# mmacklin/tinsel

Measured on AMD Instinct MI355X. Metric: Msamples/s (cornell.tin 1024x1024 maxDepth=4 spp=2126, wavefront path; Mrays/s alongside), higher is better.
Workload: dtype f32; 1 GPU; cornell.tin 1024x1024 maxDepth=4, 1 pass(es) per step, pipeline=auto; scene_pack=tests/golden/cornell.pack, parallelism=1 GPU

## Files before the change

### include/tinsel_hip.h

```cpp
#ifndef TINSEL_HIP_H
#define TINSEL_HIP_H

#include <stddef.h>
#include <stdint.h>

#ifdef __cplusplus
extern "C" {
#endif


typedef struct tinsel_vec3 { float x, y, z; } tinsel_vec3;
typedef struct tinsel_vec4 { float x, y, z, w; } tinsel_vec4;

typedef struct tinsel_transform {
    tinsel_vec3 p;
    tinsel_vec4 r;
    float s;
} tinsel_transform;

typedef struct tinsel_bvh_node {
    tinsel_vec3 lower;
    tinsel_vec3 upper;
    uint32_t left_index;
    uint32_t right_index_leaf;
// ... 295 lines not shown
typedef struct tinsel_ray     { float ox, oy, oz, time;  float dx, dy, dz, tmax; } tinsel_ray;
typedef struct tinsel_ray_hit { float t; int32_t primitive; float nx, ny, nz; uint32_t reserved[3]; } tinsel_ray_hit;

#define TINSEL_QUERY_CLOSEST  0
#define TINSEL_QUERY_OCCLUDED 1

int tinsel_hip_trace_rays(tinsel_hip* r, int mode, long long n, const tinsel_ray* rays_host, void* out_host);
int tinsel_hip_trace_rays_device(tinsel_hip* r, int mode, long long n, const tinsel_ray* rays_dev, void* out_dev, void* stream);
int tinsel_hip_trace_camera(tinsel_hip* r, const tinsel_camera* camera, int width, int height, float time, tinsel_ray_hit* out_host);

typedef struct tinsel_path_start { float ox, oy, oz, time;  float dx, dy, dz, reserved0;  uint32_t rng1, rng2, reserved1, reserved2; } tinsel_path_start;

int tinsel_hip_trace_radiance(tinsel_hip* r, long long n, const tinsel_path_start* starts_host, int max_depth, float* out_rgbx_host);
int tinsel_hip_trace_radiance_device(tinsel_hip* r, long long n, const tinsel_path_start* starts_dev, int max_depth, float* out_rgbx_dev, void* stream);

typedef struct tinsel_gather_point { float px, py, pz, time;  float nx, ny, nz;  uint32_t seed; } tinsel_gather_point;

#define TINSEL_GATHER_COSINE 0
#define TINSEL_GATHER_SPHERE 1

int tinsel_hip_gather_radiance(tinsel_hip* r, int mode, long long n, const tinsel_gather_point* points_host, int samples, int max_depth,
                               float* out_rgbx_host, tinsel_path_start* starts_out_host );
int tinsel_hip_gather_radiance_device(tinsel_hip* r, int mode, long long n, const tinsel_gather_point* points_dev, int samples, int max_depth,
                                      float* out_rgbx_dev, tinsel_path_start* starts_out_dev , void* stream);

#define TINSEL_GATHER_SH_MAX_ORDER 2

int tinsel_hip_gather_sh(tinsel_hip* r, int mode, int order, long long n, const tinsel_gather_point* points_host,
                         int samples, int max_depth, float* out_host, tinsel_path_start* starts_out_host );
int tinsel_hip_gather_sh_device(tinsel_hip* r, int mode, int order, long long n, const tinsel_gather_point* points_dev,
                                int samples, int max_depth, float* out_dev, tinsel_path_start* starts_out_dev , void* stream);

int tinsel_hip_reserve(tinsel_hip* r, int passes, int max_depth);

int tinsel_hip_set_batch_paths(tinsel_hip* r, unsigned long long max_paths);

long long tinsel_hip_read_batch_radiance(tinsel_hip* r, float* out_rgbx, unsigned long long max_paths);

int tinsel_hip_leaf(tinsel_hip* r, int op, int index, int n, const float* in, int in_stride, const uint32_t* seeds,
                    float* out, int out_stride, const tinsel_camera* camera, int width, int height);

int tinsel_hip_mesh_tree(tinsel_hip* r, int primitive, void* out_nodes, int capacity, int* out_meta);

int tinsel_hip_stack_entries(tinsel_hip* r);
int tinsel_hip_nee_per_path(tinsel_hip* r);
int tinsel_hip_walked_prims(tinsel_hip* r);
int tinsel_hip_walk_tops(tinsel_hip* r, int* out_counts, int capacity);
int tinsel_hip_queue_counts(tinsel_hip* r, uint32_t* out, int max_bounces);
int tinsel_hip_bounce_plan(tinsel_hip* r, uint32_t* out2);
unsigned int tinsel_hip_scene_features(const tinsel_scene_desc* scene);
int tinsel_hip_scene_plane_pairs(const tinsel_scene_desc* scene, int32_t* out_pairs, int capacity, int* out_singles);
int tinsel_hip_plane_table(tinsel_hip* r, int* out2);
int tinsel_hip_scene_slim(const tinsel_scene_desc* scene);
enum { TINSEL_BOUNCE_MEDIA = 1, TINSEL_BOUNCE_PROBE = 2, TINSEL_BOUNCE_MOTION = 4, TINSEL_BOUNCE_MESH_WALK = 8, TINSEL_BOUNCE_SPHERE = 16,
       TINSEL_BOUNCE_TRANSMISSION = 32, TINSEL_BOUNCE_POOLS = 64, TINSEL_BOUNCE_SHARE = 128, TINSEL_BOUNCE_SORT = 256, TINSEL_BOUNCE_ROULETTE = 512 };

const char* tinsel_hip_last_error(void);


typedef struct tinsel_hip_group tinsel_hip_group;

tinsel_hip_group* tinsel_hip_group_create(const tinsel_scene_desc* scene, int num_gpus, int tile);
tinsel_hip_group* tinsel_hip_group_create_tuned(const tinsel_scene_desc* scene, int num_gpus, int tile, const tinsel_hip_tuning* tuning);
void tinsel_hip_group_destroy(tinsel_hip_group* g);
int tinsel_hip_group_init(tinsel_hip_group* g, int width, int height);
int tinsel_hip_group_render(tinsel_hip_group* g, const tinsel_camera* camera, const tinsel_options* options, float* out_rgba, int passes);
int tinsel_hip_group_set_lookahead(tinsel_hip_group* g, int enable);
int tinsel_hip_group_present(tinsel_hip_group* g, const tinsel_options* options, int nlm_width, float nlm_falloff, float* out_rgba);
int tinsel_hip_group_size(tinsel_hip_group* g);
tinsel_hip* tinsel_hip_group_member(tinsel_hip_group* g, int rank);

#define TINSEL_HIP_COMM_ID_BYTES 128
int tinsel_hip_comm_unique_id(unsigned char* id_bytes, int capacity);
int tinsel_hip_comm_init(tinsel_hip* r, const unsigned char* id_bytes, int rank, int world);
int tinsel_hip_comm_size(tinsel_hip* r);
int tinsel_hip_comm_reduce_accum(tinsel_hip* r, float* out_device, int root, void* stream);

int tinsel_hip_plan_regions(unsigned long long slots, int num_cus, int nee_per_path, int fused, unsigned int* out);

int tinsel_hip_selftest_arith(int device_index, int op, int variant, unsigned long long* out_counts, unsigned int* out_first_bad);
int tinsel_hip_selftest_sort(int device_index, unsigned long long* keys, unsigned long long n, int begin_bit, int end_bit);
int tinsel_hip_selftest_scan(int device_index, const int* in, int* out, unsigned long long n);
int tinsel_hip_accumulate_support(int filter_type, float filter_width, float filter_falloff, float filter_offset, float* out_arg_zero);
int tinsel_hip_selftest_accumulate(int device_index, int width, int height, int filter_type, float filter_width, float filter_falloff, float filter_offset,
                                   float clamp, const unsigned int* pass_seeds, int passes, const float* radiance, float* accum, int choice, int form,
                                   int* out_form);

int tinsel_hip_ubench(int device_index, int kind, unsigned long long bytes, int steps, double* out_ms, double* out_units);


#define TINSEL_PACK_MAGIC "TINPACK1"

typedef struct tinsel_pack_header {
    char magic[8];
    uint32_t version;
    uint32_t num_primitives;
    uint32_t num_bvh_nodes;
    uint32_t num_meshes;
    uint64_t total_bytes;
    uint64_t off_primitives;
    uint64_t off_bvh_nodes;
    uint64_t off_probe_data;
    uint64_t off_probe_pdf_x;
    uint64_t off_probe_cdf_x;
    uint64_t off_probe_pdf_y;
    uint64_t off_probe_cdf_y;
// ... 47 lines not shown
```

### tinsel_amd/abi.py

```python
import ctypes as C


class Vec3(C.Structure):
    _fields_ = [("x", C.c_float), ("y", C.c_float), ("z", C.c_float)]

    def __iter__(self):
        return iter((self.x, self.y, self.z))


class Vec4(C.Structure):
    _fields_ = [("x", C.c_float), ("y", C.c_float), ("z", C.c_float), ("w", C.c_float)]

    def __iter__(self):
        return iter((self.x, self.y, self.z, self.w))


class Transform(C.Structure):
    _fields_ = [("p", Vec3), ("r", Vec4), ("s", C.c_float)]


class BVHNode(C.Structure):
    _fields_ = [("lower", Vec3), ("upper", Vec3), ("left_index", C.c_uint32), ("right_index_leaf", C.c_uint32)]


# ... 102 lines not shown
RAY_HIT_DTYPE = [("t", "<f4"), ("primitive", "<i4"), ("nx", "<f4"), ("ny", "<f4"), ("nz", "<f4"), ("reserved", "<u4", (3,))]
QUERY_CLOSEST, QUERY_OCCLUDED = 0, 1


class PathStart(C.Structure):
    _fields_ = [("ox", C.c_float), ("oy", C.c_float), ("oz", C.c_float), ("time", C.c_float),
                ("dx", C.c_float), ("dy", C.c_float), ("dz", C.c_float), ("reserved0", C.c_float),
                ("rng1", C.c_uint32), ("rng2", C.c_uint32), ("reserved1", C.c_uint32), ("reserved2", C.c_uint32)]


PATH_START_DTYPE = [("ox", "<f4"), ("oy", "<f4"), ("oz", "<f4"), ("time", "<f4"), ("dx", "<f4"), ("dy", "<f4"), ("dz", "<f4"), ("reserved0", "<f4"),
                    ("rng1", "<u4"), ("rng2", "<u4"), ("reserved1", "<u4"), ("reserved2", "<u4")]


class GatherPoint(C.Structure):
    _fields_ = [("px", C.c_float), ("py", C.c_float), ("pz", C.c_float), ("time", C.c_float),
                ("nx", C.c_float), ("ny", C.c_float), ("nz", C.c_float), ("seed", C.c_uint32)]


GATHER_POINT_DTYPE = [("px", "<f4"), ("py", "<f4"), ("pz", "<f4"), ("time", "<f4"), ("nx", "<f4"), ("ny", "<f4"), ("nz", "<f4"), ("seed", "<u4")]
GATHER_COSINE, GATHER_SPHERE = 0, 1
GATHER_SH_MAX_ORDER = 2
FEATURE_ALBEDO, FEATURE_NORMAL, FEATURE_DEPTH = 1, 2, 4
FEATURE_NAMES = ("albedo", "normal", "depth")
ID_MISS, ID_EMPTY, ID_MAX_SLOTS = -1, -2, 8
MAX_LIGHT_GROUPS = 8
MAX_VIEWS = 4096
VIEWS_ADD, VIEWS_ACCUMULATE_SINGLY = 1, 2
SAMPLE_MAP_MAX = 65535
SAMPLES_ADD = 1
RENDER_SAMPLE_MAP_ARGTYPES = [C.c_void_p, C.POINTER(Camera), C.POINTER(Options), C.c_uint32, C.c_void_p, C.c_uint, C.c_void_p]
RENDER_SAMPLE_MAP_DEVICE_ARGTYPES = RENDER_SAMPLE_MAP_ARGTYPES + [C.c_void_p]
PLAN_SAMPLE_MAP_ARGTYPES = [C.c_ulonglong, C.c_int, C.c_int, C.c_void_p, C.POINTER(C.c_ulonglong)]


class DenoiseParams(C.Structure):
    _fields_ = [("radius", C.c_int32), ("patch_radius", C.c_int32),
                ("k_color", C.c_float), ("k_albedo", C.c_float), ("k_normal", C.c_float), ("k_depth", C.c_float),
                ("demodulate", C.c_int32), ("albedo_floor", C.c_float)]

    def as_dict(self):
        return {k: getattr(self, k) for k, _ in self._fields_}


class KernelTimeV1(C.Structure):
    _fields_ = [("name", C.c_char * 32), ("launches", C.c_uint32), ("total_ms", C.c_float)]


BOUNCE_GENERAL, BOUNCE_COUNT, BOUNCE_FIT_CLOSED, BOUNCE_FIT_DEFERRED = 0, 1, 2, 3
BOUNCE_MEDIA, BOUNCE_PROBE, BOUNCE_MOTION, BOUNCE_MESH_WALK, BOUNCE_SPHERE = 1, 2, 4, 8, 16
BOUNCE_TRANSMISSION, BOUNCE_POOLS, BOUNCE_SHARE, BOUNCE_SORT, BOUNCE_ROULETTE = 32, 64, 128, 256, 512


class Tuning(C.Structure):
    _fields_ = [("struct_bytes", C.c_uint32),
                ("flat_scan", C.c_int32), ("lds_scene", C.c_int32), ("walk", C.c_int32), ("inline_max_tris", C.c_int32), ("walk_min_tris", C.c_int32),
                ("small_mesh_bytes", C.c_int64), ("arena_lds_limit", C.c_int64),
                ("batch_paths", C.c_int64), ("grid_mult", C.c_int32), ("bounce_share", C.c_int32), ("repack", C.c_int32),
                ("tail_split", C.c_int32), ("tail_share", C.c_float), ("tail_divide", C.c_int32),
                ("shade_sorted", C.c_int32), ("overlap", C.c_int32), ("scene_walk", C.c_int32), ("swalk_lds", C.c_int32), ("accumulate", C.c_int32),
                ("walk_block", C.c_int32), ("walk_single", C.c_int32), ("walk_lds_stack", C.c_int32), ("walk_refill_min", C.c_int32), ("walk_leaf_min", C.c_int32),
                ("walk_grid_mult", C.c_int32), ("quads_in_scan", C.c_int32), ("bounce_fit", C.c_int32), ("plane_pairs", C.c_int32)]
    CREATE_FIELDS = ("flat_scan", "lds_scene", "walk", "inline_max_tris", "walk_min_tris", "small_mesh_bytes", "arena_lds_limit")
    _DEFAULTS = dict(flat_scan=-1, lds_scene=-1, walk=-1, inline_max_tris=-1, walk_min_tris=-1, small_mesh_bytes=-1, arena_lds_limit=-1,
                     batch_paths=0, grid_mult=0, bounce_share=-1, repack=-1, tail_split=-1, tail_share=0.0, tail_divide=4,
                     shade_sorted=-1, overlap=-1, scene_walk=-1, swalk_lds=-1, accumulate=0,
                     walk_block=0, walk_single=-1, walk_lds_stack=-1, walk_refill_min=0, walk_leaf_min=0, walk_grid_mult=0, quads_in_scan=-1, bounce_fit=-1, plane_pairs=-1)

    def __init__(self, **over):
        super().__init__()
        self.struct_bytes = C.sizeof(Tuning)
        for k, v in self._DEFAULTS.items():
            setattr(self, k, v)
        for k, v in over.items():
            if k not in self._DEFAULTS:
                raise TypeError("tinsel_hip_tuning has no field %r" % k)
            setattr(self, k, v)

    def replace(self, **over):
        t = Tuning(**{k: getattr(self, k) for k in self._DEFAULTS})
        for k, v in over.items():
            if k not in self._DEFAULTS:
                raise TypeError("tinsel_hip_tuning has no field %r" % k)
            setattr(t, k, v)
        return t

    def as_dict(self):
        return {k: getattr(self, k) for k in self._DEFAULTS}


ACCUMULATE_AUTO, ACCUMULATE_TILED, ACCUMULATE_WIDE, ACCUMULATE_PIPED, ACCUMULATE_FULL_WINDOW = 0, 1, 2, 3, 4
ACCUMULATE_FORM_AUTO, ACCUMULATE_FORM_FULL_WINDOW, ACCUMULATE_FORM_SUPPORT = 0, 1, 2
ACCUMULATE_RAN_UNTILED, ACCUMULATE_RAN_TILED, ACCUMULATE_RAN_WIDE, ACCUMULATE_RAN_PIPED, ACCUMULATE_RAN_SUPPORT_TILED, ACCUMULATE_RAN_SUPPORT_WIDE = 0, 1, 2, 3, 4, 5
SELFTEST_ACCUMULATE_ARGTYPES = [C.c_int, C.c_int, C.c_int, C.c_int, C.c_float, C.c_float, C.c_float, C.c_float, C.c_void_p, C.c_int, C.c_void_p, C.c_void_p,
                                C.c_int, C.c_int, C.POINTER(C.c_int)]


def accumulate_arg_zero(offset):
    import math
    import numpy as np
    z = math.log(float(np.float32(offset))) - 1e-6
    f = np.float32(z)
    if float(f) > z:
        f = np.nextafter(f, np.float32(-np.inf))
    return f


def accumulate_takes_support_form(filter_type, width, falloff, offset):
    import numpy as np
    width, falloff, offset = np.float32(width), np.float32(falloff), np.float32(offset)
    if filter_type == FILTER_BOX or not (offset > 0 and np.isfinite(offset)) or not (falloff > 0 and np.isfinite(falloff)) or not (0 < width <= 1):
        return False
    return bool(-falloff <= accumulate_arg_zero(offset))
COMM_ID_BYTES = 128
MODE_NORMALS, MODE_COMPLEXITY, MODE_PATHTRACE = 0, 1, 2
BVH_REFERENCE, BVH_LBVH, BVH_PLOC = 0, 1, 2
SCENE_BVH_NODES, SCENE_BVH_DEVICE = 0, 1
ARITH_EXACT, ARITH_FAST = 0, 1
PROBE_CDF, PROBE_ALIAS = 0, 1
LOOKAHEAD_OFF, LOOKAHEAD_ON, LOOKAHEAD_PIN_OUTPUT = 0, 1, 2
# ... 10 lines not shown
```

### tinsel_amd/build.py

```python
import hashlib
import json
import os
import shutil
import subprocess
import sys
import tempfile
import time

HERE = os.path.dirname(os.path.abspath(__file__))
ROOT = os.path.dirname(HERE)
SRC = os.path.join(HERE, "csrc", "tinsel_hip.hip")
SRC_FAST = os.path.join(HERE, "csrc", "tinsel_fast.hip")
OUT = os.path.join(HERE, "libtinsel_hip.so")
OBJ_DIR = os.path.join(HERE, "csrc", "_obj")
DEPS = [os.path.join(HERE, "csrc", f) for f in sorted(os.listdir(os.path.join(HERE, "csrc"))) if not f.startswith("_")] + \
       [os.path.join(ROOT, "include", "tinsel_hip.h")]

COMMON_FLAGS = [
    "--offload-arch=gfx950", "-O3", "-std=c++17", "-fPIC", "-fno-slp-vectorize",
    "-Wall", "-Wno-unused-function", "-Wno-unused-variable",
]
HIPCC_FLAGS = COMMON_FLAGS + ["-ffp-contract=off", "-fno-fast-math"]
FAST_FLAGS = COMMON_FLAGS + ["-DTN_FAST=1", "-ffp-contract=fast", "-fno-hip-fp32-correctly-rounded-divide-sqrt", "-freciprocal-math",
                             "-fgpu-flush-denormals-to-zero"]


def hipcc():
    for cand in (os.environ.get("HIPCC"), shutil.which("hipcc"), "/opt/rocm/bin/hipcc"):
        if cand and os.path.exists(cand):
            return cand
    raise RuntimeError("hipcc not found: the HIP library cannot be built (there is no CPU fallback)")


def up_to_date():
    if not os.path.exists(OUT):
        return False
    t = os.path.getmtime(OUT)
    return all(os.path.getmtime(d) <= t for d in DEPS)


def _compile(obj_dir, extra=(), verbose=True):
    os.makedirs(obj_dir, exist_ok=True)
    cc = hipcc()
    jobs = [
        [cc] + HIPCC_FLAGS + list(extra) + ["-c", SRC, "-o", "tinsel_hip.o"],
        [cc] + FAST_FLAGS + list(extra) + ["-c", SRC_FAST, "-o", "tinsel_fast.o"],
    ]
    procs = []
    for cmd in jobs:
        if verbose:
            print("[tinsel_amd.build] (in %s)" % obj_dir, " ".join(cmd), flush=True)
        procs.append(subprocess.Popen(cmd, cwd=obj_dir))
    for p, cmd in zip(procs, jobs):
        if p.wait() != 0:
            raise subprocess.CalledProcessError(p.returncode, cmd)


def _resource_job(tmp):
    cmd = [hipcc()] + HIPCC_FLAGS + ["--cuda-device-only", "-Rpass-analysis=kernel-resource-usage", "-c", SRC, "-o", "resources_only.o"]
    return subprocess.Popen(cmd, cwd=tmp, stdout=subprocess.DEVNULL, stderr=subprocess.PIPE, text=True)


def _kernel_name(mangled):
    import re
    m = re.match(r"_ZN2tn(\d+)", mangled)
    if not m:
        return mangled
    n = int(m.group(1))
    name, rest = mangled[m.end():m.end() + n], mangled[m.end() + n:]
    if len(name) != n or not name.startswith("k_"):
        return mangled
    t = re.match(r"I((?:L[bij]n?\d+E)+)E", rest)
    args = re.findall(r"L[bij](n?\d+)E", t.group(1)) if t else []
    return name + ("<" + ",".join(a.replace("n", "-") for a in args) + ">" if args else "")


def _parse_resources(text):
    import re
    out, cur = {}, None
    for line in text.splitlines():
        m = re.search(r"remark:\s+(.*?)\s*\[-Rpass-analysis", line)
        if not m:
            continue
        body = m.group(1)
        if body.startswith("Function Name:"):
            cur = out.setdefault(_kernel_name(body.split(":", 1)[1].strip()), {})
        elif cur is not None and ":" in body:
            k, v = body.split(":", 1)
            key = {"VGPRs": "vgprs", "AGPRs": "agprs", "TotalSGPRs": "sgprs", "ScratchSize [bytes/lane]": "scratch_bytes",
                   "Occupancy [waves/SIMD]": "waves_per_simd", "LDS Size [bytes/block]": "static_lds_bytes",
                   "SGPRs Spill": "sgpr_spills", "VGPRs Spill": "vgpr_spills"}.get(k.strip())
            if key:
                cur[key] = int(v.strip())
    return out


def _code_bytes(device_obj):
    import struct
    with open(device_obj, "rb") as f:
        b = f.read()
    magic = b"__CLANG_OFFLOAD_BUNDLE__"
    if b.startswith(magic):
        count, = struct.unpack_from("<Q", b, len(magic))
        pos = len(magic) + 8
        for _ in range(count):
            off, size, tlen = struct.unpack_from("<QQQ", b, pos)
            triple = b[pos + 24:pos + 24 + tlen]
            pos += 24 + tlen
# ... 83 lines not shown
```

### tinsel_amd/csrc/tinsel_hip.hip

```cpp

#include "../../include/tinsel_hip.h"

#include "tn_launch.h"
#include "tn_denoise.h"
#include "tn_lbvh.h"
#include "tn_ubench.h"
#include "tn_selftest.h"

#include "tn_sort.h"

#include <hip/hip_runtime.h>
#include <rccl/rccl.h>

#include <dlfcn.h>

#include <cmath>
#include <condition_variable>
#include <deque>
#include <mutex>
#include <thread>
#include <cstdio>
#include <cstdlib>
#include <cstring>
#include <map>
#include <memory>
#include <string>
#include <vector>

using namespace tn;

namespace {

thread_local std::string g_error;

int fail(const std::string& msg)
{
    g_error = msg;
    fprintf(stderr, "tinsel_hip: %s\n", msg.c_str());
    return -1;
}

#define HIP_TRY(expr)                                                                                       \
    do {                                                                                                    \
        hipError_t _e = (expr);                                                                             \
        if (_e != hipSuccess)                                                                               \
            return fail(std::string(#expr) + ": " + hipGetErrorString(_e));                                 \
    } while (0)

#define HIP_TRY_NULL(expr)                                                                                  \
    do {                                                                                                    \
        hipError_t _e = (expr);                                                                             \
        if (_e != hipSuccess) {                                                                             \
            fail(std::string(#expr) + ": " + hipGetErrorString(_e));                                        \
            return nullptr;                                                                                 \
        }                                                                                                   \
    } while (0)

}

#include "tn_host_own.h"
#include "tn_host_layout.h"
#include "tn_host_state.h"
#include "tn_host_batch.h"
#include "tn_host_query.h"
#include "tn_host_radiance.h"
#include "tn_host_gather.h"
#include "tn_host_features.h"
#include "tn_host_ids.h"
#include "tn_host_light_groups.h"
#include "tn_host_views.h"
#include "tn_host_samples.h"
#include "tn_host_denoise.h"
#include "tn_host_lookahead.h"
#include "tn_host_bvh_build.h"
#include "tn_host_scene.h"

#include "tn_host_create.h"
#include "tn_host_api.h"
#include "tn_host_group.h"
```

### tinsel_amd/csrc/tn_fused.h

```cpp
#pragma once

#include "tn_path_state.h"

namespace tn {

constexpr int kPoolFields = 25;
constexpr int kPoolWordsPerWave = kPoolFields*kWave;
constexpr int kPoolWords = kPoolWordsPerWave*(kBlock/kWave);

constexpr int kPoolFieldsSlim = 21;

template <int FIELDS>
TN_D void pool_store(uint32_t* pool, uint32_t e, const PathRegs& p, uint32_t slot, int prim, float t, V3 n)
{
    static_assert(FIELDS == kPoolFields || FIELDS == kPoolFieldsSlim, "a pool entry is whole or slim");
    uint32_t* q = pool + e;
    q[0*kWave] = __float_as_uint(p.o.x); q[1*kWave] = __float_as_uint(p.o.y); q[2*kWave] = __float_as_uint(p.o.z);
    q[3*kWave] = __float_as_uint(p.d.x); q[4*kWave] = __float_as_uint(p.d.y); q[5*kWave] = __float_as_uint(p.d.z);
    if constexpr (FIELDS == kPoolFieldsSlim)
    {
        q[6*kWave] = __float_as_uint(p.thr.x); q[7*kWave] = __float_as_uint(p.thr.y); q[8*kWave] = __float_as_uint(p.thr.z);
        q[9*kWave] = __float_as_uint(p.rad.x); q[10*kWave] = __float_as_uint(p.rad.y); q[11*kWave] = __float_as_uint(p.rad.z);
        q[12*kWave] = p.rng.s1; q[13*kWave] = p.rng.s2;
        q[14*kWave] = __float_as_uint(p.bsdfPdf);
// ... 30 lines not shown
        p.rad = V3(__uint_as_float(q[9*kWave]), __uint_as_float(q[10*kWave]), __uint_as_float(q[11*kWave]));
        p.rng.s1 = q[12*kWave]; p.rng.s2 = q[13*kWave];
        p.bsdfPdf = __uint_as_float(q[14*kWave]);
        slot = q[15*kWave];
        prim = (int)q[16*kWave];
        t = __uint_as_float(q[17*kWave]);
        n = V3(__uint_as_float(q[18*kWave]), __uint_as_float(q[19*kWave]), __uint_as_float(q[20*kWave]));
        path_slim_constants(p);
        return;
    }
    p.time = __uint_as_float(q[6*kWave]);
    p.thr = V3(__uint_as_float(q[7*kWave]), __uint_as_float(q[8*kWave]), __uint_as_float(q[9*kWave]));
    p.rad = V3(__uint_as_float(q[10*kWave]), __uint_as_float(q[11*kWave]), __uint_as_float(q[12*kWave]));
    p.rng.s1 = q[13*kWave]; p.rng.s2 = q[14*kWave];
    p.eta = __uint_as_float(q[15*kWave]);
    p.bsdfPdf = __uint_as_float(q[16*kWave]);
    p.rayType = (int)q[17*kWave];
    slot = q[18*kWave];
    prim = (int)q[19*kWave];
    t = __uint_as_float(q[20*kWave]);
    n = V3(__uint_as_float(q[21*kWave]), __uint_as_float(q[22*kWave]), __uint_as_float(q[23*kWave]));
    p.medium = (int)q[24*kWave];
}


#ifdef TN_PROFILE_SECTIONS
#define TN_PROF_DECL uint32_t prof[6] = { 0, 0, 0, 0, 0, 0 }; long long tprev = clock64();
#define TN_TICK(k) { const long long _t = clock64(); prof[k] += (uint32_t)(_t - tprev); tprev = _t; }
#define TN_PROF_FLUSH if (lane_id() == 0) { for (int k = 0; k < 6; ++k) atomicAdd(q.stats + (size_t)(blockIdx.x % kStatShards)*kStatWords + 2 + k, (unsigned long long)prof[k]); } if (true) return;
#else
#define TN_TICK(k)
#define TN_PROF_DECL
#define TN_PROF_FLUSH
#endif

struct BounceKernargs { DevScene scIn; SplitState ss; QueueCtl q; int bounceBegin, bounceEnd, stackEntries; CameraParams cam; FrameParams fp; const uint32_t* passSeeds; };

enum BounceKind : int { kBounceGeneral = 0, kBounceCount = 1, kBounceFitClosed = 2, kBounceFitDeferred = 3 };
constexpr uint32_t bounce_kind_features(int kind)
{
    return kind == kBounceFitClosed ? (uint32_t)kFeatSphere :
           kind == kBounceFitDeferred ? (uint32_t)(kFeatSphere | kFeatPools | kFeatShare | kFeatSort) : (uint32_t)kFeatAll;
}

template <int KIND, bool LDS, bool DEFER>
__global__ __launch_bounds__(kBlock, kBounceWaves) void k_bounce(BounceKernargs ka)
{
    constexpr bool COUNT = KIND == kBounceCount;
    constexpr uint32_t FEAT = bounce_kind_features(KIND);
    constexpr bool SLIM = KIND >= kBounceFitClosed;
    constexpr int POOL = SLIM ? kPoolFieldsSlim : kPoolFields;
    static_assert(!SLIM || !(FEAT & (kFeatMedia | kFeatMotion | kFeatTransmission | kFeatProbe)), "the slim state has no word for these");
    typedef SceneT<LDS, false, DEFER ? 1 : 0, false, FEAT> SC;
    const DevScene& scIn = ka.scIn;
    const SplitState& ss = ka.ss;
    const QueueCtl& q = ka.q;
    const int bounceBegin = ka.bounceBegin, bounceEnd = ka.bounceEnd, stackEntries = ka.stackEntries;
    const CameraParams& cam = ka.cam;
    const FrameParams& fp = ka.fp;
    const uint32_t* __restrict__ const passSeeds = ka.passSeeds;
    extern __shared__ uint32_t s_stack[];
    LdsStack<kBlock> st = { s_stack + threadIdx.x };

    const bool repack = (FEAT & kFeatPools) && fp.repack != 0;
    const bool shareRegions = (FEAT & kFeatShare) && fp.share != 0;
    const uint32_t wave = wave_in_block();
    uint32_t* const pool = s_stack + stackEntries*kBlock + kScanWords + wave*kPoolWordsPerWave;
    SC sc;
    stage_scene_lds(sc, scIn, s_stack + stackEntries*kBlock + kScanWords + (repack ? kPoolWords : 0));
    if constexpr (!(FEAT & kFeatMedia)) sc.hasMedia = 0;
    if constexpr (!(FEAT & kFeatProbe)) sc.probe.valid = 0;
    if constexpr (!(FEAT & kFeatSort)) sc.sortQueues = 0;
    if constexpr (KIND >= kBounceFitClosed) sc.flatScan = 1;
    auto mat_at = [&](int prim) {
        Mat m = load_mat(sc.mats, prim);
        if constexpr (!(FEAT & kFeatTransmission)) m.transmission = 0.0f;
        if constexpr (SLIM) m.subsurface = 0.0f;
        return m;
    };
    typedef const __attribute__((address_space(4))) SplitState* StatePtr;
    auto state_args = [&]() {
        StatePtr sp = (StatePtr)((const __attribute__((address_space(4))) char*)__builtin_amdgcn_kernarg_segment_ptr() + offsetof(BounceKernargs, ss));
        asm volatile("" : "+s"(sp));
        return sp;
    };
    auto ssBuf = [&](int buf) {
        StatePtr sp = state_args();
        if constexpr (SLIM)
        {
            static_assert(offsetof(SplitState, rad) + sizeof(float4*[2]) - offsetof(SplitState, rayO) == 64, "rayO, rayD, thr, rad: contiguous");
            float4* const o0 = sp->rayO[0]; float4* const o1 = sp->rayO[1]; float4* const d0 = sp->rayD[0]; float4* const d1 = sp->rayD[1];
            float4* const t0 = sp->thr[0]; float4* const t1 = sp->thr[1]; float4* const r0 = sp->rad[0]; float4* const r1 = sp->rad[1];
            StateBuf b = { buf ? o1 : o0, buf ? d1 : d0, buf ? t1 : t0, buf ? r1 : r0, nullptr };
            return b;
        }
        StateBuf b = { sp->rayO[buf], sp->rayD[buf], sp->thr[buf], sp->rad[buf], sp->rngId[buf] };
        return b;
    };
    auto radOutNow = [&]() { return state_args()->radOut; };
#define TN_SS_BUF(buf) ssBuf(buf)
#define TN_RAD_OUT radOutNow()
    auto late_sky = [&]() {
        typedef const __attribute__((address_space(4))) DevScene* ScenePtr;
        ScenePtr sp = (ScenePtr)((const __attribute__((address_space(4))) char*)__builtin_amdgcn_kernarg_segment_ptr() + offsetof(BounceKernargs, scIn));
        asm volatile("" : "+s"(sp));
        DevScene s;
// ... 113 lines not shown
                        load_state(sc, TN_SS_BUF(cur), pos, p, slot, hasMedia);
                    have = true;
                }
            }

            if (have)
            {
                TN_TICK(0)
                prim = trace<SC, LdsStack<kBlock>, COUNT>(sc, st, p.o, p.d, p.time, t, n3, ctr);
                rays++;
                TN_TICK(1)
                if (prim < 0)
                {
                    on_miss(late_sky(), p, bounce);
                    TN_RAD_OUT[slot] = make_float4(p.rad.x, p.rad.y, p.rad.z, 0.0f);
                    have = false;
                }
            }

            if (repack)
            {
                const unsigned long long live = __ballot(have);
                const uint32_t nLive = (uint32_t)__popcll(live);
                if (flush || poolCount + nLive >= (uint32_t)kWave)
                {
                    const uint32_t take = (poolCount < (uint32_t)kWave - nLive) ? poolCount : (uint32_t)kWave - nLive;
                    const uint32_t rank = bits_below(~live);
                    if (!have && rank < take)
                    {
                        pool_load<POOL>(pool, poolCount - 1u - rank, p, slot, prim, t, n3);
                        if constexpr (!SLIM)
                            p.absorption = medium_absorption(sc, p.medium, hasMedia);
                        have = true;
                    }
                    poolCount -= take;
                }
                else
                {
                    if (have)
                        pool_store<POOL>(pool, poolCount + bits_below(live), p, slot, prim, t, n3);
                    poolCount += nLive;
                    have = false;
                }
            }

            if (have)
            {
                {
                    const V3 n = n3;
                    const Mat mat = mat_at(prim);
                    HitCtx h;
                    on_hit_begin<SLIM>(p, mat, t, n, bounce, h, prim);

                    if (sc.totalLightSamples > 0)
                    {
                        const V3 thrAtNee = p.thr;
                        LightCursor lights;
                        V3 sum = nee_sum(sc, [&](int k) -> V3 {
                            NeeGeo g;
                            V3 skyColor;
                            float skyPdf = 0.0f;
                            int light = -1;
                            if (sc.probe.valid && k == 0)
                                nee_sample_probe(late_sky(), h.p, h.n, p.rng, g, skyColor, skyPdf);
                            else
                            {
                                light = lights.next(sc);
                                nee_sample_light(sc, h.p, h.n, p.time, light, p.rng, g);
                            }
                            TN_TICK(2)
                            float ts;
                            V3 nn;
                            const int hp = trace<SC, LdsStack<kBlock>, COUNT>(sc, st, g.o, g.wi, p.time, ts, nn, ctr);
                            TN_TICK(3)
                            rays++;
                            shadowRays++;
                            if (light < 0)
                                return (hp < 0) ? nee_contrib_probe<SLIM>(mat_at(prim), h, g.wi, skyColor, skyPdf) : V3(0.0f);
                            if (!nee_light_reached(g, hp, ts))
                                return V3(0.0f);
                            return nee_contrib_light<SLIM>(sc, mat_at(prim), h, g.wi, g.nl, light, hp, ts);
                        });
                        p.rad = p.rad + thrAtNee*sum;
                    }

                    TN_TICK(2)
                    if (bounce + 1 < fp.maxDepth)
                    {
                        const Mat matAgain = mat_at(prim);
                        alive = (bsdf_step<SLIM>(p, matAgain, h) == kContinue);
                        if ((FEAT & kFeatRoulette) && alive && fp.rrStart > 0 && bounce + 1 >= fp.rrStart)
                            alive = roulette_survives(p);
                    }
                }

                TN_TICK(5)
                if (alive)
                    front = !sc.sortQueues || ray_meets_bounded_prim(sc, p.o, p.d);
                else
                    TN_RAD_OUT[slot] = make_float4(p.rad.x, p.rad.y, p.rad.z, 0.0f);
            }
            const uint32_t np = out.push(alive, front);
            if (alive)
            {
                if constexpr (SLIM)
                    store_state_slim(TN_SS_BUF(nxt), np, p, slot);
                else
                    store_state(TN_SS_BUF(nxt), np, p, slot);
            }
            if (flush)
                break;
        }
        if (lane == 0)
        {
            ss.segFront[(size_t)(bounce + 1)*ss.numRegions + r] = out.nFront;
            ss.segBack[(size_t)(bounce + 1)*ss.numRegions + r] = out.nBack;
        }
      }
    }

    wave_add_stat(q.stats, 0, rays);
    wave_add_stat(q.stats, 1, samples);
#ifndef TN_PROFILE_SECTIONS
    wave_add_stat(q.stats, 5, shadowRays);
#endif
    TN_PROF_FLUSH
    if (COUNT)
    {
        wave_add_stat(q.stats, 2, ctr.internal);
        wave_add_stat(q.stats, 3, ctr.tris);
        wave_add_stat(q.stats, 4, ctr.prims);
    }
}


// ... 5 lines not shown
```

### tinsel_amd/csrc/tn_host_api.h

```cpp
#pragma once

extern "C" {

int tinsel_hip_init(tinsel_hip* r, int width, int height)
{
    if (r)
        lookahead_release(r);
    if (!r || width <= 0 || height <= 0)
        return fail("init: bad arguments");
    HIP_TRY(hipSetDevice(r->device));
    HIP_TRY(hipDeviceSynchronize());
    r->accum = nullptr;
    if (r->accumOwn.alloc((size_t)width*height))
        return -1;
    r->accum = r->accumOwn.get();
    HIP_TRY(hipMemset(r->accum, 0, sizeof(float4)*(size_t)width*height));
    HIP_TRY(hipStreamSynchronize(nullptr));
    r->width = width;
    r->height = height;
    return 0;
}

int tinsel_hip_init_external(tinsel_hip* r, int width, int height, float* device_accum)
{
// ... 953 lines not shown
    std::vector<float> eqs;
    for (int n = 0; n < scene->num_bvh_nodes; ++n)
    {
        const tinsel_bvh_node& nd = scene->bvh_nodes[n];
        if (!ref_is_leaf(nd) || nd.left_index >= (uint32_t)scene->num_primitives || scene->primitives[nd.left_index].type != TINSEL_GEOM_PLANE)
            continue;
        if (make_prim_box(nd).alwaysHit && std::find(planes.begin(), planes.end(), (int32_t)nd.left_index) == planes.end())
            planes.push_back((int32_t)nd.left_index);
    }
    std::sort(planes.begin(), planes.end());
    for (const int32_t k : planes)
        eqs.insert(eqs.end(), scene->primitives[k].geo.plane.plane, scene->primitives[k].geo.plane.plane + 4);
    const std::vector<std::pair<int, int>> pairs = pair_planes(eqs);
    for (size_t q = 0; q < pairs.size() && out_pairs && (int)q < capacity; ++q)
    {
        out_pairs[2*q] = planes[(size_t)pairs[q].first];
        out_pairs[2*q + 1] = planes[(size_t)pairs[q].second];
    }
    if (out_singles)
        *out_singles = (int)planes.size() - 2*(int)pairs.size();
    return (int)pairs.size();
}

int tinsel_hip_plane_table(tinsel_hip* r, int* out2)
{
    if (!r || !out2)
        return fail("plane_table: bad arguments");
    out2[0] = r->planePairs;
    out2[1] = r->planeSingles;
    return 0;
}

int tinsel_hip_scene_slim(const tinsel_scene_desc* scene)
{
    if (!scene || !scene->primitives)
        return 0;
    bool anySubsurface = false;
    for (int i = 0; i < scene->num_primitives; ++i)
        anySubsurface = anySubsurface || !is_plus_zero(scene->primitives[i].material.subsurface);
    return scene_slim(tinsel_hip_scene_features(scene), anySubsurface) ? 1 : 0;
}

int tinsel_hip_bounce_plan(tinsel_hip* r, uint32_t* out2)
{
    if (!r || !out2)
        return fail("bounce_plan: bad arguments");
    if (r->lastBounceKind < 0)
        return fail("bounce_plan: the fused kernel has not run yet");
    out2[0] = (uint32_t)r->lastBounceKind;
    out2[1] = r->lastBounceFeatures;
    return 0;
}

int tinsel_hip_queue_counts(tinsel_hip* r, uint32_t* out, int max_bounces)
{
    if (!r || !out || max_bounces < 1)
        return fail("queue_counts: bad arguments");
    if (r->batchPipeline < 0 || r->batchDepth < 1)
        return fail("queue_counts: nothing rendered yet");
    HIP_TRY(hipSetDevice(r->device));
    HIP_TRY(hipDeviceSynchronize());
    const int n = std::min(max_bounces, std::min(r->batchDepth, r->lastFp.maxDepth));
    if (r->lastPipeline == TINSEL_PIPELINE_MEGAKERNEL || r->batchPipeline != r->lastPipeline)
        return fail("queue_counts: the last batch did not run a wavefront pipeline");
    const tinsel_hip::DenseLane& lane = r->lane[r->lastLane];
    const bool split = r->lastPipeline == TINSEL_PIPELINE_WAVEFRONT_SPLIT && r->neePerPath > 0;
    const size_t W = lane.regions;
    std::vector<uint32_t> seg(W*(size_t)n*4, 0u);
    uint32_t* const src[4] = { lane.ss.segFront, lane.ss.segBack, lane.ss.neeFront, lane.ss.neeBack };
    for (int a = 0; a < (split ? 4 : 2); ++a)
        HIP_TRY(hipMemcpy(seg.data() + (size_t)a*W*n, src[a], W*(size_t)n*sizeof(uint32_t), hipMemcpyDeviceToHost));
    for (int b = 0; b < n; ++b)
    {
        unsigned long long live = 0, nee = 0;
        for (size_t g = 0; g < W; ++g)
        {
            live += seg[(size_t)b*W + g] + seg[W*n + (size_t)b*W + g];
            nee += seg[2*W*n + (size_t)b*W + g] + seg[3*W*n + (size_t)b*W + g];
        }
        out[b] = (b == 0 && r->lastPipeline == TINSEL_PIPELINE_WAVEFRONT) ? lane.paths : (uint32_t)live;
        out[max_bounces + b] = (uint32_t)nee;
    }
    return n;
}


int tinsel_hip_plan_regions(unsigned long long slots, int num_cus, int nee_per_path, int fused, unsigned int* out)
{
    if (!out || slots == 0 || slots >= 0xffffffffull || num_cus < 1 || num_cus > 4096)
        return fail("plan_regions: bad arguments");
    RegionSpec s = region_spec(tuning_defaults(), num_cus, nee_per_path, fused != 0, kBounceWaves);
    s.capacity = (size_t)slots + s.maxRegions*kWave;
    RegionCut c;
    const int rc = cut_regions(s, (size_t)slots, streaming_grid(s, (size_t)slots), c) ? 0 : fail("render: path buffers too small for this batch");
    out[0] = c.numRegions; out[1] = c.regionLen; out[2] = c.bigRegions; out[3] = c.shortLen;
    out[4] = (unsigned int)c.grid(); out[5] = (unsigned int)s.maxRegions;
    return rc;
}

int tinsel_hip_selftest_arith(int device_index, int op, int variant, unsigned long long* out_counts, unsigned int* out_first_bad)
{
    if (!out_counts || !out_first_bad || op < 0 || op > 2)
        return fail("selftest_arith: bad arguments");
    if (variant < 0)
        variant = op == 0 ? kRcpVariant : op == 1 ? kSqrtVariant : kRsqrtVariant;
    HIP_TRY(hipSetDevice(device_index));
// ... 285 lines not shown
```

### tinsel_amd/csrc/tn_host_batch.h

```cpp
#pragma once

namespace {

void free_batch(tinsel_hip* r)
{
    r->batchMem.release();
    for (tinsel_hip::DenseLane& lane : r->lane)
        lane = tinsel_hip::DenseLane();
    r->batchPipeline = -1;
    r->batchSlots = 0;
    r->batchStateSlots = 0;
    r->batchLanes = 1;
    r->batchNee = -1;
    r->batchDepth = -1;
    r->lastBatchSlots = 0;
}

constexpr int kGridMultDefault = 32;
int grid_mult(const tinsel_hip* r) { return r->tune.grid_mult > 0 ? r->tune.grid_mult : kGridMultDefault; }

bool paired_can(const tinsel_hip* r) { return r->scene.flatScan != 0 && !r->countDetail; }

enum Residency { RES_HBM, RES_LDS, RES_MIXED };
Residency residency(const DevScene& sc, uint32_t staged) { return sc.allInArena ? RES_LDS : (staged != 0 && staged == sc.arenaBytes) ? RES_MIXED : RES_HBM; }
// ... 330 lines not shown
    if (share < 0.0)
    {
        const double sets = (double)grid/(double)(s.resident*s.numCUs);
        share = std::min(0.25, std::max(0.03, -share/std::max(1.0, sets)));
    }
    if (share > 0.0 && share < 0.9 && divide >= 2)
        split_tail_regions(s, c, slots, share, divide);
    return true;
}

bool plan_bounce(const tinsel_hip* r, int* resident)
{
    const size_t perCU = 160u*1024u;
    const size_t lds = stack_bytes(r), withPool = lds + kPoolWords*sizeof(uint32_t);
    const bool want = r->tune.repack >= 0 ? r->tune.repack != 0 : !r->sceneEnclosed;
    const bool pools = want && withPool*3 <= perCU && withPool <= (size_t)r->sharedMemLimit;
    const size_t ldsPerGroup = std::max<size_t>(1, pools ? withPool : lds);
    *resident = (int)std::max<size_t>(1, std::min<size_t>((size_t)kBounceWaves, perCU/ldsPerGroup));
    return pools;
}

uint32_t bounce_features(const tinsel_hip* r, bool pools)
{
    uint32_t f = 0;
    f |= r->scene.hasMedia ? kFeatMedia : 0u;
    f |= r->scene.probe.valid ? kFeatProbe : 0u;
    f |= r->anyTransmission ? kFeatTransmission : 0u;
    f |= r->scene.sortQueues ? kFeatSort : 0u;
    f |= pools ? kFeatPools : 0u;
    f |= r->rrStart > 0 ? kFeatRoulette : 0u;
    for (size_t i = 0; i < r->primsHost.size(); ++i)
    {
        const Prim64& p = r->primsHost[i];
        f |= (p.flags & kPrimMoving) ? kFeatMotion : 0u;
        f |= p.type == (uint32_t)kPrimSphere ? kFeatSphere : 0u;
        const int m = i < r->primMesh.size() ? r->primMesh[i] : -1;
        if (p.type == (uint32_t)kPrimMesh && !(p.flags & kPrimQuadArena) && !(m >= 0 && r->meshesNow[(size_t)m].twoLeaves))
            f |= kFeatMeshWalk;
    }
    return f;
}

bool scene_slim(uint32_t features, bool anySubsurface)
{
    return !(features & (kFeatMedia | kFeatProbe | kFeatMotion | kFeatMeshWalk | kFeatTransmission)) && !anySubsurface;
}

int fit_bounce(uint32_t need, bool deferMeshes)
{
    auto within = [&](int kind) { return (need & ~bounce_kind_features(kind)) == 0u; };
    if (deferMeshes)
        return within(kBounceFitDeferred) ? PK_BOUNCE_FIT_DEFERRED : PK_NONE;
    return within(kBounceFitClosed) ? PK_BOUNCE_FIT_CLOSED : PK_NONE;
}

struct WalkPlan
{
    int variant = PK_NONE, block = 256, perCU = 1;
    bool single = false;
    uint32_t ldsBytes = 0;
    WalkJob job = {};
};

struct SwalkPlan
{
    int extend = PK_NONE, shadow = PK_NONE, block = kBlock, perCU = 32;
    uint32_t ldsBytes = 0, arenaLds = 0;
    SwalkJob job = {};
};

WalkPlan plan_walk(const tinsel_hip* r)
{
    const tinsel_hip_tuning& t = r->tune;
    WalkPlan w;
    WalkJob& job = w.job;
    const int gridMult = t.walk_grid_mult > 0 ? t.walk_grid_mult : 1;
    job.refillMin = std::min(64, std::max(1, t.walk_refill_min > 0 ? t.walk_refill_min : 24));
    job.leafMin = std::min(64, std::max(1, t.walk_leaf_min > 0 ? t.walk_leaf_min : 8));
    job.numPrims = r->walkPrims.count;
    job.prof = r->walkProf.get();
    int entries = 1;
    for (int k = 0; k < kWalkMaxPrims && k < r->walkPrims.count; ++k)
    {
        job.prim[k] = r->walkPrims.prim[k];
        entries = std::max(entries, r->meshesNow[(size_t)r->walkPrimMesh[k]].stackNeed);
    }
    w.single = r->walkPrims.count == 1 && t.walk_single != 0;
    const size_t ctl = (kWalkCtlWords + (w.single ? 0 : kWalkMaxPrims*kWalkPrimWords))*sizeof(uint32_t);
    const int ldsStackEnv = t.walk_lds_stack >= 0 ? t.walk_lds_stack : 8;
    const bool twoPerCU = ldsStackEnv > 0 && !t.walk_block;
    const int ldsEntries = twoPerCU ? std::min(entries, std::max(1, ldsStackEnv)) : entries;
    const int rows = w.single ? kWalkLaneRows : kWalkRayRows;
    const size_t ldsBudget = twoPerCU ? (size_t)r->sharedMemLimit/2 : (size_t)r->sharedMemLimit;
    const bool big = t.walk_block ? t.walk_block == 1024 : (size_t)(ldsEntries + rows)*1024*sizeof(uint32_t) + ctl + 16384 <= ldsBudget;
    w.block = big ? 1024 : 256;
    size_t lds = (size_t)(ldsEntries + rows)*w.block*sizeof(uint32_t) + ctl;
    if (big)
    {
        size_t room = (ldsBudget - lds)/sizeof(Node64);
        for (int k = 0; k < r->walkPrims.count && room > 0; ++k)
        {
            const int n = (int)std::min<size_t>(room, (size_t)r->meshesNow[(size_t)r->walkPrimMesh[k]].topCount);
            job.topCount[k] = n;
            room -= (size_t)n;
            lds += (size_t)n*sizeof(Node64);
        }
// ... 477 lines not shown
{
    switch (generate)
    {
    case PK_GENERATE_RAYS: return KN_GENERATE_RAYS;
    case PK_GENERATE_GATHER: return KN_GENERATE_GATHER;
    default: return KN_GENERATE;
    }
}

int cut_and_generate(tinsel_hip* r, const BatchPlan& p, tinsel_hip::DenseLane& L, hipStream_t st, LaunchArgs& a, size_t slots, int* grid)
{
    *grid = streaming_grid(p.regions, slots);
    if (p.workList)
        *grid = std::max(1, std::min(*grid, (int)(seg_prefix_max_regions(r)/(kBlock/kWave))));
    if (cut_batch(p, L, a, slots, grid))
        return -1;
    ScopedTimer t(r, generate_timer(p.generate), st);
    a.grid = *grid;
    a.variant = p.generate;
    a.ldsBytes = 0;
    return launch_path(r, a, st);
}

void order_regions(tinsel_hip* r, hipStream_t st, const LaunchArgs& a, const uint32_t* front, const uint32_t* back, uint32_t* out)
{
    ScopedTimer t(r, KN_SEG, st);
    hipLaunchKernelGGL(k_region_order, dim3(1), dim3(kOrderBlock), 0, st, front, back, a.ss.numRegions, out);
}

int trace_fused(tinsel_hip* r, const BatchPlan& p, tinsel_hip::DenseLane& L, hipStream_t st, LaunchArgs& a, size_t slots)
{
    int grid = streaming_grid(p.regions, slots);
    if (cut_batch(p, L, a, slots, &grid))
        return -1;
    a.grid = grid;
    if (p.pools)
    {
        a.fp.repack = 1;
        a.ldsBytes += (uint32_t)(kPoolWords*sizeof(uint32_t));
    }
    {
        const int shareLen = 512;
        a.fp.share = r->tune.bounce_share >= 0 ? (r->tune.bounce_share != 0) : (r->neePerPath >= 3 || (int)a.ss.regionLen <= shareLen);
    }
    a.bounce = 0;
    a.bounceEnd = a.fp.maxDepth;
    a.order = nullptr;
    a.variant = a.fp.share ? p.bounceShared : p.bounce;
    r->lastBounceKind = a.variant == PK_BOUNCE_FIT_CLOSED ? kBounceFitClosed :
                        a.variant == PK_BOUNCE_FIT_DEFERRED ? kBounceFitDeferred :
                        (a.variant == PK_BOUNCE_COUNT_LDS || a.variant == PK_BOUNCE_COUNT) ? kBounceCount : kBounceGeneral;
    r->lastBounceFeatures = p.bounceFeatures | (a.fp.share ? kFeatShare : 0u);
    ScopedTimer t(r, KN_BOUNCE, st);
    return launch_path(r, a, st);
}

int trace_paired(tinsel_hip* r, const BatchPlan& p, tinsel_hip::DenseLane& L, hipStream_t st, LaunchArgs& a, size_t slots)
{
    int grid = 0;
    if (cut_and_generate(r, p, L, st, a, slots, &grid))
        return -1;
    const size_t W = a.ss.numRegions;
    const int K = r->neePerPath, maxDepth = a.fp.maxDepth;
    const int steps = maxDepth + (K > 0 ? 1 : 0);
    for (int bounce = 0; bounce < steps; ++bounce)
    {
        a.bounce = bounce;
        a.order = nullptr;
        if (p.walk)
        {
            a.grid = grid;
            const bool first = bounce == 0, last = bounce >= maxDepth;
            if (launch_walk(r, p, L, st, a, slots, L.ss.segFront + (size_t)bounce*W,  !first && K > 0,  !first && !last && K > 0))
                return -1;
        }
        if (bounce > 0 && maxDepth >= 6 && grid > r->numCUs*2)
        {
            order_regions(r, st, a, L.ss.segFront + (size_t)bounce*W, L.ss.segBack + (size_t)bounce*W, L.regionOrder);
            a.order = L.regionOrder;
        }
        ScopedTimer t(r, KN_STEP, st);
        a.grid = grid;
        a.variant = p.step;
        a.ldsBytes = p.ldsTrace;
        a.stackEntries = p.stackScan;
        if (launch_path(r, a, st))
            return -1;
    }
    return 0;
}

int trace_split(tinsel_hip* r, const BatchPlan& p, tinsel_hip::DenseLane& L, hipStream_t st, LaunchArgs& a, size_t slots)
{
    int grid = 0;
    if (cut_and_generate(r, p, L, st, a, slots, &grid))
        return -1;
    const size_t W = a.ss.numRegions;
    const bool ordered = !p.walk && grid > r->numCUs*2;
    for (int bounce = 0; bounce < a.fp.maxDepth; ++bounce)
    {
        a.bounce = bounce;
        a.order = nullptr;
        if (ordered && bounce > 0)
        {
            order_regions(r, st, a, L.ss.segFront + (size_t)bounce*W, L.ss.segBack + (size_t)bounce*W, L.regionOrder);
            a.order = L.regionOrder;
// ... 476 lines not shown
```

### tinsel_amd/csrc/tn_host_create.h

```cpp
#pragma once

namespace {

void comm_release(tinsel_hip* r);


struct SceneBuild
{
    tinsel_hip* r;
    DevScene& sc;
    const tinsel_scene_desc* desc;
    const tinsel_hip_tuning& tune;
    int P;
    std::vector<Prim64> prims;
    std::vector<Mat128> mats;
    std::vector<Moving64> moving;
    std::vector<DevMesh> meshes;
    std::vector<int32_t> lights;
    std::map<uint64_t, uint32_t> meshIndex;
    ArenaBuilder arena;
    int maxMeshNeed = 0;
    int totalLightSamples = 0;
    bool sceneHasBigMesh = false;
    SceneLevel lvl;
    bool flatScan = false;

    SceneBuild(tinsel_hip* r_, const tinsel_scene_desc* d)
        : r(r_), sc(r_->scene), desc(d), tune(r_->tune), P(d->num_primitives), prims((size_t)P), mats((size_t)P), moving((size_t)P)
    {
        for (int i = 0; i < P; ++i)
            if (desc->primitives[i].type == TINSEL_GEOM_MESH && mesh_bytes_estimate(desc->primitives[i].geo.mesh) > kSmallMeshBytes)
                sceneHasBigMesh = true;
    }

    static size_t mesh_bytes_estimate(const tinsel_mesh_geometry& g)
    {
        return (size_t)g.num_nodes*32 + (size_t)(g.num_indices/3)*52 + (size_t)g.num_vertices*12;
    }
    bool lives_in_arena(size_t meshBytes, int numTris) const
    {
        if (tune.small_mesh_bytes >= 0)
            return meshBytes <= (size_t)tune.small_mesh_bytes;
        const int inlineMaxTris = tune.inline_max_tris >= 0 ? tune.inline_max_tris : kInlineMaxTris;
        return sceneHasBigMesh ? numTris <= inlineMaxTris && meshBytes <= kSmallMeshBytes : meshBytes <= kSmallMeshBytes;
    }

    int add_primitives();
    int add_mesh(const tinsel_mesh_geometry& g, Prim64& o);
    int scene_level();
    void mark_walked_and_quads();
    int assemble_arena();
    void set_scene_flags();
    int upload_probe();
    int stats_and_fit();
};

void create_limits(tinsel_hip* r, int device_index, const tinsel_hip_tuning* tuning)
{
    r->device = device_index;
    r->tune = tuning_from_caller(tuning);
    hipDeviceProp_t prop;
    if (hipGetDeviceProperties(&prop, device_index) == hipSuccess)
    {
        r->numCUs = prop.multiProcessorCount;
        r->sharedMemLimit = (int)prop.sharedMemPerBlock;
    }
    prepare_kernels_once(r);
    if (!r->prepRefused.empty() && r->sharedMemLimit > 65536)
    {
        fprintf(stderr, "tinsel_hip: the runtime refused %d B of dynamic LDS for %s: planning within 65536 B per workgroup\n", r->sharedMemLimit, r->prepRefused.c_str());
        r->sharedMemLimit = 65536;
        r->segPrefixLds = std::min(r->segPrefixLds, 65536 - 1024);
    }

    if (r->tune.batch_paths >= 65536)
    {
        r->maxBatchSlots = (size_t)r->tune.batch_paths;
        r->batchSlotsExplicit = true;
    }
}

int SceneBuild::add_mesh(const tinsel_mesh_geometry& g, Prim64& o)
{
    const int numTris = g.num_indices/3;
    if (numTris <= 0 || !g.positions || !g.normals || !g.indices || !g.nodes || !g.cdf)
        return fail("create: mesh primitive with missing arrays");
    ConvertedBvh cb;
    if (!convert_bvh(g.nodes, g.num_nodes, numTris, lives_in_arena(mesh_bytes_estimate(g), numTris) ? 0 : kWalkTopNodes, cb))
        return fail("create: malformed mesh BVH");
    std::vector<Tri48> tris((size_t)numTris);
    for (int t = 0; t < numTris; ++t)
    {
        const int i0 = g.indices[t*3 + 0], i1 = g.indices[t*3 + 1], i2 = g.indices[t*3 + 2];
        if (i0 < 0 || i1 < 0 || i2 < 0 || i0 >= g.num_vertices || i1 >= g.num_vertices || i2 >= g.num_vertices)
            return fail("create: mesh index out of range");
        Tri48& T = tris[(size_t)t];
        T.ax = g.positions[i0].x; T.ay = g.positions[i0].y; T.az = g.positions[i0].z; T.i0 = i0;
        T.bx = g.positions[i1].x; T.by = g.positions[i1].y; T.bz = g.positions[i1].z; T.i1 = i1;
        T.cx = g.positions[i2].x; T.cy = g.positions[i2].y; T.cz = g.positions[i2].z; T.i2 = i2;
    }

    DevMesh dm;
    memset(&dm, 0, sizeof(dm));
    dm.root = cb.root;
    dm.numTris = numTris;
    dm.stackNeed = cb.maxLeafDepth + 1;
    dm.topCount = cb.topCount;
    dm.numInternal = (int32_t)cb.nodes.size();
    dm.twoLeaves = (cb.nodes.size() == 1 && !(cb.root & kLeafBit) && (cb.nodes[0].left & kLeafBit) && (cb.nodes[0].right & kLeafBit)) ? 1 : 0;
    const size_t meshBytes = cb.nodes.size()*sizeof(Node64) + tris.size()*sizeof(Tri48) + (size_t)g.num_vertices*12 + (size_t)numTris*4;
    if (lives_in_arena(meshBytes, numTris))
    {
        dm.inArena = 1;
        dm.offNodes = (uint32_t)arena.add(cb.nodes.data(), cb.nodes.size());
        dm.offTris = (uint32_t)arena.add(tris.data(), tris.size());
        dm.offNormals = (uint32_t)arena.add(&g.normals[0].x, (size_t)g.num_vertices*3);
        dm.offCdf = (uint32_t)arena.add(g.cdf, (size_t)numTris);
    }
    else
    {
        dm.nodes = r->sceneMem.upload(cb.nodes.data(), cb.nodes.size());
        dm.tris = r->sceneMem.upload(tris.data(), tris.size());
        dm.normals = r->sceneMem.upload(&g.normals[0].x, (size_t)g.num_vertices*3);
        dm.cdf = r->sceneMem.upload(g.cdf, (size_t)numTris);
        if ((!cb.nodes.empty() && !dm.nodes) || !dm.tris || !dm.normals || !dm.cdf)
            return fail("create: device allocation failed (mesh)");
    }
    if (dm.stackNeed > maxMeshNeed)
        maxMeshNeed = dm.stackNeed;
    r->meshNumVertices.push_back(g.num_vertices);
    r->meshIndices.emplace_back(g.indices, g.indices + (size_t)numTris*3);
    r->meshRootLo.push_back(V3(g.nodes[0].lower.x, g.nodes[0].lower.y, g.nodes[0].lower.z));
    r->meshRootHi.push_back(V3(g.nodes[0].upper.x, g.nodes[0].upper.y, g.nodes[0].upper.z));
    r->meshArea.push_back(g.area);
    o.mesh = (uint32_t)meshes.size();
    meshIndex[g.id] = o.mesh;
    meshes.push_back(dm);
    return 0;
}

int SceneBuild::add_primitives()
{
    for (int i = 0; i < P; ++i)
    {
        const tinsel_primitive& p = desc->primitives[i];
        Prim64& o = prims[(size_t)i];
        memset(&o, 0, sizeof(o));

        make_material(p, mats[(size_t)i]);
        r->primEndScale.push_back(p.end_transform.s);
        if (p.light_samples > 0)
        {
            if (p.type == TINSEL_GEOM_PLANE)
                return fail("create: a plane cannot be a light (PrimitiveSample asserts, intersection.h:871-875)");
            lights.push_back(i);
            totalLightSamples += p.light_samples;
        }

        const bool isStatic = memcmp(&p.start_transform, &p.end_transform, sizeof(tinsel_transform)) == 0;
        const Xform xs = to_xform(p.start_transform), xe = to_xform(p.end_transform);
        r->primStart.push_back(xs);
        r->primEnd.push_back(xe);
        set_prim_pose(o, xs, xe, isStatic);
        o.moving = (uint32_t)i;
        moving[(size_t)i] = make_moving(xs, xe);

        if (p.type == TINSEL_GEOM_SPHERE)
        {
            o.type = kPrimSphere;
            o.g0 = p.geo.sphere.radius;
// ... 34 lines not shown
    const int need = lvl.bvh.maxLeafDepth + 1 + maxMeshNeed;
    r->stackNeed = pick_stack(need);
    if (r->stackNeed < 0)
        return fail("create: BVH too deep for the 156-entry LDS traversal stack");
    flatScan = lvl.everyPrimHasALeaf && P <= 64 && tune.flat_scan != 0;
    return 0;
}

void SceneBuild::mark_walked_and_quads()
{
    const int walkMinTris = tune.walk_min_tris >= 0 ? tune.walk_min_tris : kInlineMaxTris + 1;
    r->binPrims.count = 0;
    r->walkPrims.count = 0;
    if (flatScan)
        for (int k = 0; k < P && r->binPrims.count < 7; ++k)
            if (prims[(size_t)k].type == kPrimMesh && !meshes[prims[(size_t)k].mesh].inArena)
            {
                r->binPrims.prim[r->binPrims.count++] = k;
                if (meshes[prims[(size_t)k].mesh].numTris >= walkMinTris)
                {
                    prims[(size_t)k].flags |= kPrimWalked | ((uint32_t)r->walkPrims.count << kPrimWalkLaneShift);
                    r->walkPrimMesh[r->walkPrims.count] = (int)prims[(size_t)k].mesh;
                    r->walkPrims.prim[r->walkPrims.count++] = k;
                }
            }
    for (int k = 0; k < P; ++k)
        if (prims[(size_t)k].type == kPrimMesh && meshes[prims[(size_t)k].mesh].twoLeaves && meshes[prims[(size_t)k].mesh].inArena)
        {
            const DevMesh& qm = meshes[prims[(size_t)k].mesh];
            if (((qm.offNodes | qm.offTris | qm.offNormals | qm.offCdf) & 127u) != 0u || ((qm.offNodes | qm.offTris | qm.offNormals | qm.offCdf) >> 7) > 0xffffu)
                continue;
            Prim64& qp = prims[(size_t)k];
            qp.flags |= kPrimQuadArena;
            const uint32_t w0 = (qm.offNodes >> 7) | ((qm.offTris >> 7) << 16), w1 = (qm.offNormals >> 7) | ((qm.offCdf >> 7) << 16);
            memcpy(&qp.g0, &w0, 4); memcpy(&qp.g1, &w1, 4);
        }
    r->walkEnabled = tune.walk != 0;
#ifdef TN_WALK_PROF
    if (r->walkProf.alloc(16) == 0)
        (void)hipMemset(r->walkProf.get(), 0, 16*sizeof(unsigned long long));
#endif
}

int SceneBuild::assemble_arena()
{
    const size_t offNodes = arena.add(lvl.bvh.nodes.data(), lvl.bvh.nodes.size());
    const size_t offPrims = arena.add(prims.data(), prims.size());
    const size_t offMats = arena.add(mats.data(), mats.size());
    const size_t offMoving = arena.add(moving.data(), moving.size());
    std::vector<LightRec> lightRecs(lights.size());
    for (size_t l = 0; l < lights.size(); ++l)
        lightRecs[l] = { lights[l], mats[(size_t)lights[l]].lightSamples, mats[(size_t)lights[l]].rcpLightSamples, 0 };
    const size_t offLights = arena.add(lightRecs.data(), lightRecs.size());
    const size_t offMeshes = arena.add(meshes.data(), meshes.size());

    int alwaysHitPlanes = 0;
    bool anyMeshInHbm = false;
    for (int k = 0; k < P; ++k)
    {
        alwaysHitPlanes += (prims[(size_t)k].type == kPrimPlane && lvl.boxes[(size_t)k].alwaysHit) ? 1 : 0;
        anyMeshInHbm = anyMeshInHbm || (prims[(size_t)k].type == kPrimMesh && !meshes[prims[(size_t)k].mesh].inArena);
    }
    if (flatScan && (alwaysHitPlanes >= 4 || anyMeshInHbm))
    {
        for (int k = 0; k < P; ++k)
            if (prims[(size_t)k].type == kPrimPlane && lvl.boxes[(size_t)k].alwaysHit)
                r->planeTablePrims.push_back(k);
        int meshPrimCount = 0;
        for (int k = 0; k < P; ++k)
            meshPrimCount += prims[(size_t)k].type == kPrimMesh ? 1 : 0;
        r->pairablePlanes = !(meshPrimCount >= 2 && !anyMeshInHbm);
        mark_plane_table(lvl, prims, r->planeTablePrims, pairs_planes(r, tune));
    }
    const std::vector<float>& planeEq = lvl.planeEq;
    const std::vector<int32_t>& planeIdx = lvl.planeIdx;
    const size_t offBoxes = arena.add(lvl.boxes.data(), lvl.boxes.size());
    const size_t offPlaneEq = arena.add(planeEq.data(), planeEq.size());
    const size_t offPlaneIdx = arena.add(planeIdx.data(), planeIdx.size());
    arena.bytes.resize((arena.bytes.size() + 127) & ~size_t(127), 0);

    unsigned char* arenaDev = r->sceneMem.upload(arena.bytes.data(), arena.bytes.size());
    if (!arenaDev)
        return fail("create: device allocation failed (scene arena)");
    DevMesh* hm = reinterpret_cast<DevMesh*>(&arena.bytes[offMeshes]);
    for (size_t m = 0; m < meshes.size(); ++m)
    {
        if (hm[m].inArena)
        {
            hm[m].nodes = reinterpret_cast<const Node64*>(arenaDev + hm[m].offNodes);
            hm[m].tris = reinterpret_cast<const Tri48*>(arenaDev + hm[m].offTris);
            hm[m].normals = reinterpret_cast<const float*>(arenaDev + hm[m].offNormals);
            hm[m].cdf = reinterpret_cast<const float*>(arenaDev + hm[m].offCdf);
        }
    }
    if (!meshes.empty() && hipMemcpy(arenaDev + offMeshes, hm, sizeof(DevMesh)*meshes.size(), hipMemcpyHostToDevice) != hipSuccess)
        return fail("create: device allocation failed (scene arena)");
    r->meshesRef.assign(hm, hm + meshes.size());
    r->meshesNow = r->meshesRef;

    sc.arena = arenaDev;
    sc.arenaBytes = (uint32_t)arena.bytes.size();
    const size_t ldsLimit = tune.arena_lds_limit >= 0 ? (size_t)tune.arena_lds_limit : kArenaLdsLimit;
    sc.arenaLdsBytes = (arena.bytes.size() <= ldsLimit && tune.lds_scene != 0) ? sc.arenaBytes : 0u;
    sc.nodes = reinterpret_cast<const Node64*>(arenaDev + offNodes);
    sc.prims = reinterpret_cast<const Prim64*>(arenaDev + offPrims);
    sc.mats = reinterpret_cast<const Mat128*>(arenaDev + offMats);
    sc.moving = reinterpret_cast<const Moving64*>(arenaDev + offMoving);
    sc.lights = reinterpret_cast<const LightRec*>(arenaDev + offLights);
    sc.meshes = reinterpret_cast<const DevMesh*>(arenaDev + offMeshes);
    sc.numMeshes = (int)meshes.size();
    sc.primBoxes = reinterpret_cast<const PrimBox*>(arenaDev + offBoxes);
    sc.planeEq = reinterpret_cast<const float4*>(arenaDev + offPlaneEq);
    sc.planeIdx = reinterpret_cast<const int32_t*>(arenaDev + offPlaneIdx);
    adopt_scene_level(r, lvl);
    r->arenaOffNodes = offNodes;
    r->arenaOffBoxes = offBoxes;
    r->arenaOffPrims = offPrims;
    r->arenaOffMoving = offMoving;
    r->arenaOffMats = offMats;
    r->primsHost = prims;
    return 0;
}

void SceneBuild::set_scene_flags()
{
    sc.hasMedia = 0;
    for (const Mat128& mm : mats)
        if (mm.absorption[0] != 0.0f || mm.absorption[1] != 0.0f || mm.absorption[2] != 0.0f)
            sc.hasMedia = 1;
    r->anyTransmission = std::any_of(mats.begin(), mats.end(), [](const Mat128& mm) { return mm.transmission != 0.0f; });
    r->anySubsurface = std::any_of(mats.begin(), mats.end(), [](const Mat128& mm) { return !is_plus_zero(mm.subsurface); });
    sc.flatScan = flatScan ? 1 : 0;
    {
        int meshPrimCount = 0;
        for (int k = 0; k < P; ++k)
            meshPrimCount += prims[(size_t)k].type == kPrimMesh ? 1 : 0;
        sc.deferMeshes = (meshPrimCount >= 2) ? 1 : 0;
    }
    {
        int planes = 0;
        for (int k = 0; k < P; ++k)
            planes += lvl.boxes[(size_t)k].alwaysHit ? 1 : 0;
        sc.sortQueues = (sc.flatScan && planes <= 2 && planes < P) ? 1 : 0;
    }
    for (int i = 0; i < P && !r->sceneEnclosed; ++i)
        for (int j = i + 1; j < P && !r->sceneEnclosed; ++j)
            if (prims[(size_t)i].type == kPrimPlane && prims[(size_t)j].type == kPrimPlane)
            {
                const Prim64 &a = prims[(size_t)i], &b = prims[(size_t)j];
                const float d = a.g0*b.g0 + a.g1*b.g1 + a.g2*b.g2;
                const float la = sqrtf(a.g0*a.g0 + a.g1*a.g1 + a.g2*a.g2), lb = sqrtf(b.g0*b.g0 + b.g1*b.g1 + b.g2*b.g2);
                r->sceneEnclosed = la > 0.0f && lb > 0.0f && d < -0.99f*la*lb;
            }
    bool all = sc.arenaLdsBytes != 0;
    for (const DevMesh& dmesh : meshes)
        all = all && dmesh.inArena;
    sc.allInArena = all ? 1 : 0;
    sc.numPrims = P;
    sc.numLights = (int)lights.size();
    sc.horizon[0] = desc->sky_horizon.x; sc.horizon[1] = desc->sky_horizon.y; sc.horizon[2] = desc->sky_horizon.z;
    sc.zenith[0] = desc->sky_zenith.x; sc.zenith[1] = desc->sky_zenith.y; sc.zenith[2] = desc->sky_zenith.z;
}

int SceneBuild::upload_probe()
{
    const size_t n = (size_t)desc->probe_width*desc->probe_height;
    if (!desc->probe_data || !desc->probe_pdf_x || !desc->probe_cdf_x || !desc->probe_pdf_y || !desc->probe_cdf_y || n == 0)
        return fail("create: probe marked valid but arrays missing");
    sc.probe.data = (const float4*)r->sceneMem.upload((const float*)desc->probe_data, n*4);
    sc.probe.pdfX = r->sceneMem.upload(desc->probe_pdf_x, n);
    sc.probe.cdfX = r->sceneMem.upload(desc->probe_cdf_x, n);
    sc.probe.pdfY = r->sceneMem.upload(desc->probe_pdf_y, (size_t)desc->probe_height);
    sc.probe.cdfY = r->sceneMem.upload(desc->probe_cdf_y, (size_t)desc->probe_height);
    sc.probe.width = desc->probe_width;
    sc.probe.height = desc->probe_height;
    sc.probe.valid = 1;
    if (!sc.probe.data || !sc.probe.pdfX || !sc.probe.cdfX || !sc.probe.pdfY || !sc.probe.cdfY)
        return fail("create: device allocation failed (probe)");
    return 0;
}

int SceneBuild::stats_and_fit()
{
    r->neePerPath = totalLightSamples + (r->scene.probe.valid ? 1 : 0);
    r->scene.totalLightSamples = r->neePerPath;
    if (r->statsDev.alloc((size_t)kStatShards*kStatWords) ||
        hipMemset(r->statsDev.get(), 0, sizeof(unsigned long long)*kStatShards*kStatWords) != hipSuccess)
        return fail("create: device allocation failed (stats)");
    if (stack_bytes(r) > (size_t)r->sharedMemLimit && r->scene.arenaLdsBytes)
    {
        r->scene.arenaLdsBytes = 0;
        r->scene.allInArena = 0;
    }
    if (stack_bytes(r) > (size_t)r->sharedMemLimit)
        return fail("create: the traversal stacks of this scene need " + std::to_string(stack_bytes(r)) + " B of LDS per workgroup, the device offers " + std::to_string(r->sharedMemLimit));
    return 0;
}

}

extern "C" {


const char* tinsel_hip_last_error(void) { return g_error.c_str(); }

void tinsel_hip_tuning_init(tinsel_hip_tuning* t)
{
    if (t)
        *t = tuning_defaults();
}

tinsel_hip* tinsel_hip_create(const tinsel_scene_desc* desc, int device_index) { return tinsel_hip_create_tuned(desc, device_index, nullptr); }

tinsel_hip* tinsel_hip_create_tuned(const tinsel_scene_desc* desc, int device_index, const tinsel_hip_tuning* tuning)
{
    if (!desc || !desc->primitives || desc->num_primitives <= 0 || !desc->bvh_nodes || desc->num_bvh_nodes <= 0)
    {
        fail("create: empty scene (Scene::Build must have run)");
        return nullptr;
    }

    int ndev = 0;
    if (hipGetDeviceCount(&ndev) != hipSuccess || ndev <= 0)
    {
        fail("create: no HIP device visible -- this library has no CPU fallback");
        return nullptr;
    }
    if (device_index < 0 || device_index >= ndev)
    {
        fail("create: bad device index");
        return nullptr;
    }
    HIP_TRY_NULL(hipSetDevice(device_index));

    std::unique_ptr<tinsel_hip> r(new tinsel_hip());
    create_limits(r.get(), device_index, tuning);
    memset(&r->scene, 0, sizeof(r->scene));
    SceneBuild b(r.get(), desc);
    if (b.add_primitives() || b.scene_level())
        return nullptr;
    b.mark_walked_and_quads();
    if (b.assemble_arena())
        return nullptr;
    b.set_scene_flags();
    if ((desc->probe_valid && b.upload_probe()) || b.stats_and_fit())
        return nullptr;
    return r.release();
}

void tinsel_hip_destroy(tinsel_hip* r)
{
    if (!r)
        return;
    (void)hipSetDevice(r->device);
    lookahead_release(r);
    (void)hipDeviceSynchronize();
    comm_release(r);
    if (r->walkProf)
    {
        unsigned long long wp[16] = { 0 };
        (void)hipMemcpy(wp, r->walkProf.get(), sizeof(wp), hipMemcpyDeviceToHost);
        const double tot = (double)(wp[0] + wp[1] + wp[2] + wp[3] + wp[4]);
        fprintf(stderr, "k_walk profile: cycles refill %.1f%% node %.1f%% tri %.1f%% pop %.1f%% loop %.1f%% | iterations %llu refills %llu node-phases %llu tri-phases %llu | "
                "lanes/node-phase %.1f lanes/tri-phase %.1f lanes/refill %.1f | waves %llu cycles/wave %.0f cycles/iteration %.0f cycles/refill %.0f cycles/node-phase %.0f cycles/tri-phase %.0f\n",
                100.0*wp[0]/tot, 100.0*wp[1]/tot, 100.0*wp[2]/tot, 100.0*wp[3]/tot, 100.0*wp[4]/tot, wp[5], wp[6], wp[7], wp[8],
                (double)wp[9]/std::max(1ull, wp[7]), (double)wp[10]/std::max(1ull, wp[8]), (double)wp[11]/std::max(1ull, wp[6]),
                wp[12], (double)wp[13]/std::max(1ull, wp[12]), tot/std::max(1ull, wp[5]), (double)wp[0]/std::max(1ull, wp[6]),
                (double)wp[1]/std::max(1ull, wp[7]), (double)wp[2]/std::max(1ull, wp[8]));
    }
    delete r;
}

}
```

### tinsel_amd/csrc/tn_host_own.h

```cpp
#pragma once

namespace {

template <class T>
struct DevBuf
{
    DevBuf() = default;
    DevBuf(DevBuf&& o) noexcept { swap(o); }
    DevBuf& operator=(DevBuf&& o) noexcept { DevBuf t(std::move(o)); swap(t); return *this; }
    ~DevBuf() { reset(); }

    int alloc(size_t count)
    {
        reset();
        void* d = nullptr;
        HIP_TRY(hipMalloc(&d, sizeof(T)*(count ? count : 1)));
        p = (T*)d;
        n = count;
        return 0;
    }
    int grow(size_t count) { return p && n >= count ? 0 : alloc(count); }
    int upload(const T* host, size_t count)
    {
        if (alloc(count))
// ... 31 lines not shown
    }
    template <class T>
    T* upload(const T* host, size_t count)
    {
        T* d = nullptr;
        if (count == 0 || alloc(&d, count) || hipMemcpy(d, host, sizeof(T)*count, hipMemcpyHostToDevice) != hipSuccess)
            return nullptr;
        return d;
    }
    void release()
    {
        for (void* p : allocs)
            (void)hipFree(p);
        allocs.clear();
    }

private:
    std::vector<void*> allocs;
};

template <class H, hipError_t (*Destroy)(H)>
struct DevHandle
{
    DevHandle() = default;
    DevHandle(DevHandle&& o) noexcept { std::swap(h, o.h); }
    DevHandle& operator=(DevHandle&& o) noexcept { DevHandle t(std::move(o)); std::swap(h, t.h); return *this; }
    ~DevHandle() { if (h) (void)Destroy(h); }
    operator H() const { return h; }

protected:
    H h = nullptr;
};

struct Stream : DevHandle<hipStream_t, hipStreamDestroy>
{
    int create()
    {
        if (!h)
            HIP_TRY(hipStreamCreateWithFlags(&h, hipStreamNonBlocking));
        return 0;
    }
};

struct Event : DevHandle<hipEvent_t, hipEventDestroy>
{
    int create(bool timing = false)
    {
        if (!h)
            HIP_TRY(hipEventCreateWithFlags(&h, timing ? hipEventDefault : hipEventDisableTiming));
        return 0;
    }
};

struct PinnedOutput
{
    PinnedOutput() = default;
    PinnedOutput(const PinnedOutput&) = delete;
    PinnedOutput& operator=(const PinnedOutput&) = delete;
    ~PinnedOutput() { release(nullptr); }

    bool want(void* p, size_t bytes, bool pin, hipStream_t copies)
    {
        if (ptr && (!pin || ptr != p || size != bytes))
            release(copies);
        if (pin && !ptr)
        {
            if (hipHostRegister(p, bytes, hipHostRegisterDefault) == hipSuccess)
            {
                ptr = p;
                size = bytes;
            }
            else
                (void)hipGetLastError();
        }
        return ptr != nullptr;
    }
    bool held() const { return ptr != nullptr; }
    void release(hipStream_t copies)
    {
        if (!ptr)
            return;
        if (copies)
            (void)hipStreamSynchronize(copies);
        (void)hipHostUnregister(ptr);
        ptr = nullptr;
        size = 0;
    }

private:
    void* ptr = nullptr;
    size_t size = 0;
};

}
```

### tinsel_amd/csrc/tn_host_scene.h

```cpp
#pragma once

namespace {

void primitive_bounds(const tinsel_hip* r, int i, V3& lower, V3& upper)
{
    const Prim64& p = r->primsHost[(size_t)i];
    V3 lo, hi;
    if (p.type == kPrimSphere)      { lo = V3(-p.g0); hi = V3(p.g0); }
    else if (p.type == kPrimPlane)  { lo = V3(-1.e+8f); hi = V3(1.e+8f); }
    else                            { lo = r->meshRootLo[(size_t)r->primMesh[(size_t)i]]; hi = r->meshRootHi[(size_t)r->primMesh[(size_t)i]]; }
    V3 sl, su, el, eu;
    transform_bounds(r->primStart[(size_t)i], lo, hi, sl, su);
    transform_bounds(r->primEnd[(size_t)i], lo, hi, el, eu);
    lower = V3(minT(sl.x, el.x), minT(sl.y, el.y), minT(sl.z, el.z));
    upper = V3(maxT(su.x, eu.x), maxT(su.y, eu.y), maxT(su.z, eu.z));
}

void node64_to_reference(const std::vector<Node64>& nodes, uint32_t ref, float lminx, float lminy, float lminz, float lmaxx, float lmaxy, float lmaxz,
                         std::vector<tinsel_bvh_node>& out, uint32_t at)
{
    tinsel_bvh_node& me = out[at];
    me.lower.x = lminx; me.lower.y = lminy; me.lower.z = lminz;
    me.upper.x = lmaxx; me.upper.y = lmaxy; me.upper.z = lmaxz;
    if (ref & kLeafBit)
// ... 126 lines not shown
    {
        put(slot, pairs[q].first); put(slot + 1, pairs[q].second);
        if (q + 1 < pairs.size())
        {
            put(slot + 2, pairs[q + 1].first); put(slot + 3, pairs[q + 1].second);
        }
        if (nextSingle < singles.size())
            put(slot + 4, singles[nextSingle++]);
        lvl.planeIdx[slot + 5] = lvl.planeIdx[slot] | (lvl.planeIdx[slot + 1] << 8) | (lvl.planeIdx[slot + 2] << 16) | (lvl.planeIdx[slot + 3] << 24);
    }
    lvl.planePairEnd = (int32_t)slot;
    while (nextSingle < singles.size())
        put(slot++, singles[nextSingle++]);
    lvl.numPlanes = (int32_t)slot;
    lvl.planePairs = (int)pairs.size();
    lvl.planeSingles = (int)singles.size();

    lvl.scanMask = 0;
    for (size_t k = 0; k < lvl.boxes.size() && k < 64; ++k)
        if (lvl.boxes[k].alwaysHit != 2u)
            lvl.scanMask |= 1ull << k;
}

bool pairs_planes(const tinsel_hip* r, const tinsel_hip_tuning& tune) { return tune.plane_pairs != 0 && r->pairablePlanes; }

bool build_scene_level(std::vector<tinsel_bvh_node> tree, const std::vector<Prim64>& prims, const std::vector<int32_t>& planeTable, bool pairPlanes, SceneLevel& out)
{
    const int P = (int)prims.size();
    if (!convert_bvh(tree.data(), (int)tree.size(), P, 0, out.bvh))
        return false;
    out.boxes.assign((size_t)P, PrimBox());
    std::vector<char> seen((size_t)P, 0);
    for (const tinsel_bvh_node& nd : tree)
        if (ref_is_leaf(nd) && nd.left_index < (uint32_t)P)
        {
            out.boxes[nd.left_index] = make_prim_box(nd);
            seen[nd.left_index] = 1;
        }
    out.everyPrimHasALeaf = std::find(seen.begin(), seen.end(), 0) == seen.end();
    mark_plane_table(out, prims, planeTable, pairPlanes);
    out.tree = std::move(tree);
    return true;
}

void adopt_scene_level(tinsel_hip* r, SceneLevel& lvl)
{
    r->scene.root = lvl.bvh.root;
    r->scene.scanMask = lvl.scanMask;
    r->scene.numPlanes = lvl.numPlanes;
    r->scene.planePairEnd = lvl.planePairEnd;
    r->planePairs = lvl.planePairs;
    r->planeSingles = lvl.planeSingles;
    r->sceneStackNeed = lvl.bvh.maxLeafDepth + 1;
    r->sceneBvhHost = std::move(lvl.tree);
}

int upload_scene_level(tinsel_hip* r, SceneLevel& lvl)
{
    unsigned char* arenaDev = const_cast<unsigned char*>(r->scene.arena);
    if (!lvl.bvh.nodes.empty())
        HIP_TRY(hipMemcpy(arenaDev + r->arenaOffNodes, lvl.bvh.nodes.data(), sizeof(Node64)*lvl.bvh.nodes.size(), hipMemcpyHostToDevice));
    HIP_TRY(hipMemcpy(arenaDev + r->arenaOffBoxes, lvl.boxes.data(), sizeof(PrimBox)*lvl.boxes.size(), hipMemcpyHostToDevice));
    if (!lvl.planeEq.empty())
    {
        HIP_TRY(hipMemcpy(const_cast<float4*>(r->scene.planeEq), lvl.planeEq.data(), sizeof(float)*lvl.planeEq.size(), hipMemcpyHostToDevice));
        HIP_TRY(hipMemcpy(const_cast<int32_t*>(r->scene.planeIdx), lvl.planeIdx.data(), sizeof(int32_t)*lvl.planeIdx.size(), hipMemcpyHostToDevice));
    }
    adopt_scene_level(r, lvl);
    return 0;
}

int fitting_stack(const tinsel_hip* r, int sceneNeed, const std::vector<DevMesh>& meshes)
{
    int maxMeshNeed = 0;
    for (const DevMesh& dm : meshes)
        maxMeshNeed = std::max(maxMeshNeed, dm.stackNeed);
    const int stack = pick_stack(sceneNeed + maxMeshNeed);
    return stack >= 0 && stack_bytes(r, stack) <= (size_t)r->sharedMemLimit ? stack : -1;
}

template <class Build>
int timed_build(double* ms, Build&& build)
{
    Event e0, e1;
    if (e0.create(true) || e1.create(true))
        return -1;
    (void)hipEventRecord(e0, nullptr);
    const int rc = build();
    (void)hipEventRecord(e1, nullptr);
    (void)hipEventSynchronize(e1);
    float t = 0.0f;
    (void)hipEventElapsedTime(&t, e0, e1);
    if (!rc && ms)
        *ms = t;
    return rc;
}

int write_mesh_prim_area(tinsel_hip* r, int p)
{
    const float area = r->meshArea[(size_t)r->primMesh[(size_t)p]]*r->primEndScale[(size_t)p];
    const float rcpArea = 1.0f/area;
    unsigned char* mat = const_cast<unsigned char*>(r->scene.arena) + r->arenaOffMats + sizeof(Mat128)*(size_t)p;
    HIP_TRY(hipMemcpy(mat + offsetof(Mat128, area), &area, sizeof(float), hipMemcpyHostToDevice));
    HIP_TRY(hipMemcpy(mat + offsetof(Mat128, rcpArea), &rcpArea, sizeof(float), hipMemcpyHostToDevice));
    return 0;
}

}

extern "C" {

int tinsel_hip_set_mesh_bvh(tinsel_hip* r, int mode, double* build_ms)
{
    lookahead_cancel(r);
    if (!r || (mode != TINSEL_BVH_REFERENCE && mode != TINSEL_BVH_LBVH && mode != TINSEL_BVH_PLOC))
        return fail("set_mesh_bvh: bad arguments");
    HIP_TRY(hipSetDevice(r->device));
    HIP_TRY(hipDeviceSynchronize());
    if (build_ms)
        *build_ms = 0.0;

    std::vector<DevMesh> next = r->meshesRef;
    DevPool built;
    const int rc = mode == TINSEL_BVH_REFERENCE ? 0 : timed_build(build_ms, [&] {
        int rc = 0;
        for (size_t m = 0; m < next.size() && !rc; ++m)
            if (!next[m].inArena && next[m].numTris >= 2)
                rc = build_device_bvh(built, r->meshesRef[m], next[m], mode);
        return rc;
    });
    const int stack = rc ? -1 : fitting_stack(r, r->sceneStackNeed, next);
    if (stack < 0)
        return rc ? rc : fail("set_mesh_bvh: tree too deep for the LDS traversal stack (previous trees kept)");
    if (!next.empty())
        HIP_TRY(hipMemcpy((void*)r->scene.meshes, next.data(), sizeof(DevMesh)*next.size(), hipMemcpyHostToDevice));
    r->meshesNow = next;
    r->stackNeed = stack;
    r->bvhMode = mode;
    r->lbvhTrees = std::move(built);
    return 0;
}

int tinsel_hip_refit_mesh(tinsel_hip* r, int primitive, const float* positions_xyz, int num_vertices, const float* normals_xyz)
{
    lookahead_cancel(r);
    if (!r || !positions_xyz || primitive < 0 || primitive >= r->scene.numPrims || r->primMesh[(size_t)primitive] < 0)
        return fail("refit_mesh: bad arguments (a mesh primitive and its new positions)");
    const int mi = r->primMesh[(size_t)primitive];
    DevMesh& dm = r->meshesNow[(size_t)mi];
    if (num_vertices != r->meshNumVertices[(size_t)mi])
        return fail("refit_mesh: the topology must not change (vertex count differs)");
    HIP_TRY(hipSetDevice(r->device));
    HIP_TRY(hipDeviceSynchronize());

    const int numTris = dm.numTris;
    const int numNodes = numTris - 1;
    {
// ... 165 lines not shown
```

### tinsel_amd/csrc/tn_host_state.h

```cpp
#pragma once

inline tinsel_hip_tuning tuning_defaults()
{
    tinsel_hip_tuning t;
    memset(&t, 0, sizeof(t));
    t.struct_bytes = (uint32_t)sizeof(t);
    t.flat_scan = t.lds_scene = t.walk = t.inline_max_tris = t.walk_min_tris = -1;
    t.small_mesh_bytes = t.arena_lds_limit = -1;
    t.batch_paths = 0;
    t.grid_mult = 0;
    t.bounce_share = t.repack = t.tail_split = t.shade_sorted = t.overlap = t.scene_walk = t.swalk_lds = -1;
    t.tail_share = 0.0f;
    t.tail_divide = 4;
    t.accumulate = TINSEL_ACCUMULATE_AUTO;
    t.walk_block = 0;
    t.walk_single = t.walk_lds_stack = t.quads_in_scan = t.bounce_fit = t.plane_pairs = -1;
    t.walk_refill_min = t.walk_leaf_min = t.walk_grid_mult = 0;
    return t;
}

inline tinsel_hip_tuning tuning_from_caller(const tinsel_hip_tuning* in)
{
    tinsel_hip_tuning t = tuning_defaults();
    if (in && in->struct_bytes >= sizeof(uint32_t))
        memcpy(&t, in, std::min<size_t>(in->struct_bytes, sizeof(t)));
    t.struct_bytes = (uint32_t)sizeof(t);
    return t;
}

struct tinsel_hip
{
    int device = 0;
    int numCUs = 256;
    tinsel_hip_tuning tune = tuning_defaults();

    DevPool sceneMem;
    DevScene scene;
    int stackNeed = 16;
    int neePerPath = 0;

    std::vector<DevMesh> meshesRef, meshesNow;
    std::vector<int> meshNumVertices;
    std::vector<std::vector<int32_t>> meshIndices;
    std::vector<int> primMesh;
    std::vector<int32_t> lightPrims;
    std::vector<float> primEndScale;
    std::vector<Prim64> primsHost;
    size_t arenaOffPrims = 0, arenaOffMoving = 0, arenaOffMats = 0;
    std::vector<V3> meshRootLo, meshRootHi;
    std::vector<float> meshArea;
    bool sceneDirty = false;
    std::vector<Xform> primStart, primEnd;
    std::vector<tinsel_bvh_node> sceneBvhHost;
    size_t arenaOffNodes = 0, arenaOffBoxes = 0;
    std::vector<int32_t> planeTablePrims;
    bool pairablePlanes = true;
    int planePairs = 0, planeSingles = 0;
    int sceneStackNeed = 1;
    std::string prepRefused;
    bool sceneEnclosed = false;
    int bvhMode = TINSEL_BVH_REFERENCE;
    int rrStart = 0;
    bool anyTransmission = false;
    bool anySubsurface = false;
    int lastBounceKind = -1;
    uint32_t lastBounceFeatures = 0;
    DevPool lbvhTrees;

    int width = 0, height = 0;
    float4* accum = nullptr;
    DevBuf<float4> accumOwn;

    DevBuf<int> accTilesDev;
    int accTilesCount = 0;
    int accTilesKey[6] = { 0, 0, 0, 0, 0, 0 };

    DevBuf<float4> display[3];
    const float4* presented = nullptr;

    size_t batchSlots = 0;
    int batchNee = -1;
    int batchDepth = -1;
    DevPool batchMem;
    PathState ps;
    QueueCtl ctl;
    int batchPipeline = -1;
    BinPrims binPrims = { 0, { 0, 0, 0, 0, 0, 0, 0 } };
    BinPrims walkPrims = { 0, { 0, 0, 0, 0, 0, 0, 0 } };
    int walkPrimMesh[7] = { 0, 0, 0, 0, 0, 0, 0 };
    struct DenseLane
    {
        SplitState ss;
        size_t splitCap = 0;
        uint32_t splitMaxRegions = 0;
        uint32_t* regionOrder = nullptr;
        uint32_t* regionOrderNee = nullptr;
        uint32_t* walkList = nullptr;
        uint32_t* segPrefix = nullptr;
        float4* walkRec = nullptr;
        uint32_t regions = 0, paths = 0;
    } lane[2];
    DevBuf<uint32_t> walkOverflow[2];
    int lastLane = 0;
    int batchLanes = 1;
    size_t batchStateSlots = 0;
    struct LaneSync
    {
        Stream stream;
        Event fork, join, accDone;
        int create() { return stream.create() || fork.create() || join.create() || accDone.create() ? -1 : 0; }
    } laneSync;
    bool walkEnabled = true;
    DevBuf<unsigned long long> walkProf;
    DevBuf<uint2> probeAlias;
    int sharedMemLimit = 65536;
    DevBuf<uint32_t> passSeedsDev;
    size_t passSeedsCount = 0;
    uint32_t passSeedsBase = 0;
    const uint32_t* passSeeds = nullptr;
    Event passSeedsReady;
// ... 99 lines not shown
```

### tinsel_amd/csrc/tn_integrator.h

```cpp
#pragma once

#include "tn_bsdf.h"
#include "tn_isect.h"
#include "tn_probe.h"

namespace tn {

constexpr float kRayEpsilon = 0.0001f;
constexpr float kBsdfSamples = 1.0f;
constexpr float kProbeSamples = 1.0f;

struct PathRegs
{
    V3 o, d;
    float time;
    V3 thr;
    V3 rad;
    Rng rng;
    float eta;
    V3 absorption;
    float bsdfPdf;
    int rayType;
    int medium;
};
// ... 35 lines not shown
    }
    else
    {
        h.etaO = 1.0f;
        h.outAbsorption = V3(0.0f);
        h.outMedium = -1;
    }
    h.etaI = SLIM ? 1.0f : p.eta;

    if (!SLIM && (p.absorption.x != 0.0f || p.absorption.y != 0.0f || p.absorption.z != 0.0f))
    {
        V3 a = (-p.absorption)*t;
        p.thr = p.thr*V3(m_expf(a.x), m_expf(a.y), m_expf(a.z));
    }

    h.p = p.o + p.d*t;
    h.n = n;
    h.wo = -p.d;

    if (bounce == 0)
    {
        p.rad = p.rad + mat.emission;
    }
    else
    {
        float lightArea = mat.area;
        if (lightArea > 0.0f)
        {
            float lightPdf = (mat.rcpArea*t*t)/clampT(dot(-p.d, n), 1.e-3f, 1.0f);

            float cbsdf = mat.cbsdf;
            float clight = mat.clight;
            float weight = cbsdf*p.bsdfPdf/(cbsdf*p.bsdfPdf + clight*lightPdf);

            if (!SLIM && p.rayType == kSpecular)
                weight = 1.0f;

            p.rad = p.rad + weight*p.thr*mat.emission;
        }
    }
}

struct NeeGeo
{
    V3 o;
    V3 wi;
    float dist;
    float nl;
};

template <class SC>
TN_D void primitive_sample(const SC& sc, int index, float time, V3& pos, V3& normal, Rng& rng)
{
    Prim64 p = load_prim(sc.prims, index);
    if constexpr (!(SC::kFeatures & kFeatMotion))
        p.flags &= ~(uint32_t)kPrimMoving;
    const Xform x = prim_pose(sc, p, time);

    if (p.type == kPrimSphere)
    {
        float u1 = rng.randf();
        float u2 = rng.randf();
        pos = pose_xform_point(p, x, uniform_sample_sphere(u1, u2)*p.g0);
        normal = normalize(pos - x.p);
    }
    else if (p.type == kPrimMesh)
    {
        const Tri48* mtris;
        const float* nr;
        int tri;
        float r = rng.randf();
        if (p.flags & kPrimQuadArena)
        {
            const unsigned char* base = (SC::kLds || sc.arenaLdsBytes != 0u) ? sc.ldsBase : sc.arena;
            const QuadOffsets q = quad_offsets(__float_as_uint(p.g0), __float_as_uint(p.g1));
            const float* mcdf = reinterpret_cast<const float*>(base + q.cdf);
            const float c0 = mcdf[0], c1 = mcdf[1];
            tri = (c1 < r) ? 1 : (c0 < r) ? 1 : 0;
            mtris = reinterpret_cast<const Tri48*>(base + q.tris);
            nr = reinterpret_cast<const float*>(base + q.normals);
        }
        else
        {
        const DevMesh m = sc.meshes[p.mesh];
        const float* mcdf = mesh_cdf(sc, m);

        int lo = 0, hi = m.numTris;
        while (lo < hi)
        {
            int mid = lo + (hi - lo)/2;
            if (mcdf[mid] < r)
                lo = mid + 1;
            else
                hi = mid;
        }
        tri = minI(lo, m.numTris - 1);
        mtris = mesh_tris(sc, m);
        nr = mesh_normals(sc, m);
        }

        float u, v;
        uniform_sample_triangle(rng, u, v);

        const float4* tp = reinterpret_cast<const float4*>(mtris + tri);
        float4 ta = tp[0], tb = tp[1], tc = tp[2];
        V3 a(ta.x, ta.y, ta.z), b(tb.x, tb.y, tb.z), c(tc.x, tc.y, tc.z);
        int i0 = __float_as_int(ta.w), i1 = __float_as_int(tb.w), i2 = __float_as_int(tc.w);
// ... 1 lines not shown
        V3 n2(nr[i1*3 + 0], nr[i1*3 + 1], nr[i1*3 + 2]);
        V3 n3(nr[i2*3 + 0], nr[i2*3 + 1], nr[i2*3 + 2]);

        pos = pose_xform_point(p, x, u*a + v*b + (1.0f - u - v)*c);
        normal = safe_normalize(pose_xform_vector(p, x, u*n1 + v*n2 + (1.0f - u - v)*n3), V3(0.0f));
    }
}

template <class SC>
TN_D void nee_sample_light(const SC& sc, V3 hitP, V3 hitN, float time, int light, Rng& rng, NeeGeo& g)
{
    V3 lightPos, lightNormal;
    primitive_sample(sc, light, time, lightPos, lightNormal, rng);

    V3 wi = lightPos - hitP;
    float dSq = length_sq(wi);
    wi = divs(wi, sqrtf_cr(dSq));

    g.o = hitP + face_forward(hitN, wi)*kRayEpsilon;
    g.wi = wi;
    g.dist = sqrtf_cr(dSq);
    g.nl = absf(dot(lightNormal, wi));
}

TN_D bool nee_light_reached(const NeeGeo& g, int hitPrim, float t)
{
    const float kTolerance = 1.e-2f;
    return hitPrim >= 0 && fabsf(t - g.dist) <= kTolerance && !(absf(g.nl) < 1.e-6f);
}

struct NeeTerms
{
    V3 f;
    float bsdfPdf;
    float absDot;
};

template <bool SLIM = false>
TN_D NeeTerms nee_bsdf_terms(const Mat& surf, const HitCtx& h, V3 wi)
{
    NeeTerms e;
    e.f = V3(0.0f);
    e.absDot = 0.0f;
    const float etaI = hit_eta_i<SLIM>(h), etaO = hit_eta_o<SLIM>(h, surf);
    e.bsdfPdf = bsdf_pdf(surf, etaI, etaO, h.n, h.wo, wi);
    if (e.bsdfPdf > 0.0f)
    {
        e.f = bsdf_eval(surf, etaI, etaO, h.n, h.wo, wi);
        e.absDot = absf(dot(wi, h.n));
    }
    return e;
}

TN_D V3 nee_combine_light(const DevScene& sc, const NeeTerms& e, float nl, int light, int hitPrim, float t)
{
    V3 L(0.0f);
    const Mat128* lm = sc.mats + light;
    float tSq = t*t;
    float lightPdf = (lm->rcpArea*tSq)/nl;
    if (e.bsdfPdf > 0.0f)
    {
        float cbsdf = lm->cbsdf;
        float clight = lm->clight;
        float weight = clight*lightPdf/(cbsdf*e.bsdfPdf + clight*lightPdf);
        const Mat128* hm = sc.mats + hitPrim;
        V3 em(hm->emission[0], hm->emission[1], hm->emission[2]);
        L = weight*e.f*em*(e.absDot/maxT(1.e-3f, lightPdf));
    }
    return L;
}

template <bool SLIM = false>
TN_D V3 nee_contrib_light(const DevScene& sc, const Mat& surf, const HitCtx& h, V3 wi, float nl, int light, int hitPrim, float t)
{
    return nee_combine_light(sc, nee_bsdf_terms<SLIM>(surf, h, wi), nl, light, hitPrim, t);
}

TN_D void nee_sample_probe(const DevScene& sc, V3 hitP, V3 hitN, Rng& rng, NeeGeo& g, V3& skyColor, float& skyPdf)
{
    V3 wi;
    probe_sample(sc.probe, wi, skyColor, skyPdf, rng);

    g.o = hitP + face_forward(hitN, wi)*kRayEpsilon;
    g.wi = wi;
    g.dist = -1.0f;
    g.nl = 0.0f;
}

template <bool SLIM = false>
TN_D V3 nee_contrib_probe(const Mat& surf, const HitCtx& h, V3 wi, V3 skyColor, float skyPdf)
{
    V3 L(0.0f);
    const float etaI = hit_eta_i<SLIM>(h), etaO = hit_eta_o<SLIM>(h, surf);
    float bsdfPdf = bsdf_pdf(surf, etaI, etaO, h.n, h.wo, wi);
    if (bsdfPdf > 0.0f)
    {
        V3 f = bsdf_eval(surf, etaI, etaO, h.n, h.wo, wi);
        int N = int(kProbeSamples + kBsdfSamples);
        float cbsdf = kBsdfSamples/N;
        float csky = float(kProbeSamples)/N;
        float weight = csky*skyPdf/(cbsdf*bsdfPdf + csky*skyPdf);
        if (weight > 0.0f)
            L = divs(weight*skyColor*f*absf(dot(wi, h.n)), skyPdf);
    }
    return L;
}

struct LightCursor
{
    int li = 0, sInLight = 0;
    TN_D int next(const DevScene& sc)
    {
        while (sInLight >= sc.mats[sc.lights[li].prim].lightSamples) { ++li; sInLight = 0; }
        ++sInLight;
        return sc.lights[li].prim;
    }
};

template <class Contrib>
TN_D V3 nee_sum(const DevScene& sc, Contrib contrib)
{
    V3 sum(0.0f);
    int k = 0;
    if (sc.probe.valid)
    {
        sum = sum + contrib(k++);
        sum = divs(sum, float(kProbeSamples));
    }
    for (int li = 0; li < sc.numLights; ++li)
// ... 113 lines not shown
```

### tinsel_amd/csrc/tn_isect.h

```cpp
#pragma once

#include "tn_scene.h"
#include "tn_plane.h"

namespace tn {

template <int STRIDE>
struct LdsStack
{
    uint32_t* base;
    TN_D void set(int i, uint32_t v) { base[i*STRIDE] = v; }
    TN_D uint32_t get(int i) const { return base[i*STRIDE]; }
};

struct TraceCounters
{
    uint32_t internal;
    uint32_t tris;
    uint32_t prims;
};

#if TN_FAST
TN_D float minf_ref(float a, float b) { return fminf(a, b); }
TN_D float maxf_ref(float a, float b) { return fmaxf(a, b); }
// ... 508 lines not shown
            if (ray_plane(o, d, e0.x, e0.y, e0.z, e0.w, t0))
                accept(__float_as_int(left == 1 ? id.x : id.z), t0, V3(e0.x, e0.y, e0.z));
        }
    }
    for (unsigned long long todo = wave_uniform64(sc.scanMask); todo != 0ull; todo &= todo - 1ull)
    {
        const int i = (int)__builtin_ctzll(todo);
        ConstF4V b0 = sc.kBoxes[i*2], b1 = sc.kBoxes[i*2 + 1];
        ConstF4V ra = sc.kPrims[i*4], rb = sc.kPrims[i*4 + 1], rc = sc.kPrims[i*4 + 2], rd = sc.kPrims[i*4 + 3];
        asm volatile("" : "+s"(b0), "+s"(b1), "+s"(ra), "+s"(rb), "+s"(rc), "+s"(rd));
        Prim64 rec = unpack_prim(ra, rb, rc, rd);
        if (__float_as_uint(b1.z) == 0u)
        {
            float tb;
            if (!(finiteAll ? ray_aabb_minmax(o, rcp, b0.x, b0.y, b0.z, b0.w, b1.x, b1.y, tb) : ray_aabb(o, rcp, b0.x, b0.y, b0.z, b0.w, b1.x, b1.y, tb)))
                continue;
        }
        if (SC::kDefer != 0 && (SC::kDefer == 1 || sc.deferMeshes) && rec.type == (uint32_t)kPrimMesh)
        {
            meshes |= 1ull << i;
            continue;
        }
        float t;
        V3 n;
        const bool primHit = prim_intersect<SC, Stack, COUNT, ANYHIT, true>(sc, i, st, 0, o, d, time, t, n, ctr, tStop, rcp, true, &rec);
        if (primHit)
            accept(i, t, n);
        if (ANYHIT && minT < tStop)
        {
            meshes = 0;
            break;
        }
    }
    if (SC::kDefer != 0)
    {
        while (meshes)
        {
            const int i = (int)__builtin_ctzll(meshes);
            meshes &= meshes - 1ull;
            float t;
            V3 n;
            if (prim_intersect<SC, Stack, COUNT, ANYHIT>(sc, i, st, 0, o, d, time, t, n, ctr, tStop, rcp, true))
                accept(i, t, n);
            if (ANYHIT && minT < tStop)
                break;
        }
    }

    outT = minT;
    outN = face_forward(cn, -d);
    return closest;
}

template <class SC>
TN_D bool ray_meets_bounded_prim(const SC& sc, V3 o, V3 d)
{
    const V3 rcp = rcp3_cr(d);
    bool any = false;
    for (int i = 0; i < sc.numPrims; ++i)
    {
        const float4* bp = reinterpret_cast<const float4*>(sc.primBoxes + i);
        const float4 b0 = bp[0], b1 = bp[1];
        if (__float_as_uint(b1.z) != 0u)
            continue;
        float tb;
        any = any || ray_aabb(o, rcp, b0.x, b0.y, b0.z, b0.w, b1.x, b1.y, tb);
    }
    return any;
}

TN_D bool ray_sane(V3 o) { return fabsf(o.x) < 1e6f && fabsf(o.y) < 1e6f && fabsf(o.z) < 1e6f; }

TN_D float shadow_stop(float dist)
{
    return dist < 0.0f ? kFltMax : dist - 0.02f - 1e-5f*dist;
}

template <class SC, class Stack, bool COUNT, bool ANYHIT = false>
TN_D int trace(const SC& sc, Stack& st, V3 o, V3 d, float time, float& outT, V3& outN, TraceCounters& ctr, float tStop = 0.0f)
{
    float minT = kFltMax;
    int closest = -1;
    V3 cn;

    V3 rcp = rcp3_cr(d);

    if (!COUNT && sc.flatScan)
    {
        const bool sane = ray_sane(o);
        bool tie = false;
        int prim = -1;
        if (sane)
            prim = trace_flat<SC, Stack, COUNT, false>(sc, st, o, d, rcp, time, outT, outN, tie, ctr, 0.0f);
        if (sane && !tie)
            return prim;
    }

    int sp = 0;
    st.set(sp++, sc.root);

    while (sp)
    {
        uint32_t ref = st.get(--sp);

        if (ref & kLeafBit)
        {
            float t;
            V3 n;
            const int index = (int)(ref & ~kLeafBit);
            if (prim_intersect<SC, Stack, COUNT, ANYHIT>(sc, index, st, sp, o, d, time, t, n, ctr, tStop, rcp, true))
            {
                if (t < minT && t > 0.0f)
                {
                    minT = t;
                    closest = index;
                    cn = n;
                    if (ANYHIT && t < tStop)
                        break;
                }
            }
        }
        else
        {
            Node64 nd = load_node(sc.nodes, ref);
            if (COUNT) ctr.internal++;

            float tL, tR;
            bool hL = ray_aabb(o, rcp, nd.lminx, nd.lminy, nd.lminz, nd.lmaxx, nd.lmaxy, nd.lmaxz, tL);
            bool hR = ray_aabb(o, rcp, nd.rminx, nd.rminy, nd.rminz, nd.rmaxx, nd.rmaxy, nd.rmaxz, tR);

            uint32_t first = nd.left, second = nd.right;
            if (hL && hR && (tL < tR))
            {
                first = nd.right;
                second = nd.left;
            }
            if (hL)
                st.set(sp++, first);
            if (hR)
                st.set(sp++, second);
        }
    }

    outT = minT;
// ... 6 lines not shown
```

### tinsel_amd/csrc/tn_scene.h

```cpp
#pragma once

#include "tn_math.h"

namespace tn {

constexpr uint32_t kLeafBit = 0x80000000u;
constexpr uint32_t kNoNode = 0xffffffffu;
struct alignas(64) Node64
{
    float lminx, lminy, lminz, lmaxx;
    float lmaxy, lmaxz, rminx, rminy;
    float rminz, rmaxx, rmaxy, rmaxz;
    uint32_t left, right;
    uint32_t pad0, pad1;
};
static_assert(sizeof(Node64) == 64, "Node64");

struct alignas(16) Tri48
{
    float ax, ay, az; int32_t i0;
    float bx, by, bz; int32_t i1;
    float cx, cy, cz; int32_t i2;
};
static_assert(sizeof(Tri48) == 48, "Tri48");

enum : uint32_t
{
    kPrimSphere = 0,
    kPrimPlane = 1,
    kPrimMesh = 2,
};

enum : uint32_t
{
    kPrimMoving = 1u,
    kPrimWalked = 2u,
    kPrimQuadArena = 8u,
    kPrimNoRot = 4u,
    kPrimWalkLaneShift = 8,
};

struct alignas(64) Prim64
{
    float px, py, pz, s;
    float rx, ry, rz, rw;
    float g0, g1, g2, g3;
    uint32_t type;
    uint32_t flags;
    uint32_t mesh;
    uint32_t moving;
};
static_assert(sizeof(Prim64) == 64, "Prim64");

struct QuadOffsets { uint32_t nodes, tris, normals, cdf; };
TN_HD QuadOffsets quad_offsets(uint32_t w0, uint32_t w1)
// ... 83 lines not shown
    const DevMesh* meshes;
    const LightRec* lights;
    uint32_t root;
    int32_t numPrims;
    int32_t numLights;
    int32_t totalLightSamples;
    float horizon[3];
    float zenith[3];
    DevProbe probe;
    const unsigned char* arena;
    uint32_t arenaBytes;
    uint32_t arenaLdsBytes;
    int32_t numMeshes;
    int32_t allInArena;
    const PrimBox* primBoxes;
    int32_t flatScan;
    int32_t hasMedia;
    int32_t sortQueues;
    int32_t deferMeshes;
    const float4* planeEq;
    const int32_t* planeIdx;
    int32_t numPlanes;
    int32_t planePairEnd;
    unsigned long long scanMask;
};

typedef float ConstF4V __attribute__((ext_vector_type(4)));
typedef const __attribute__((address_space(4))) ConstF4V* ConstF4;

enum BounceFeature : uint32_t
{
    kFeatMedia = 1u,
    kFeatProbe = 2u,
    kFeatMotion = 4u,
    kFeatMeshWalk = 8u,
    kFeatSphere = 16u,
    kFeatTransmission = 32u,
    kFeatPools = 64u,
    kFeatShare = 128u,
    kFeatSort = 256u,
    kFeatRoulette = 512u,
    kFeatAll = 1023u
};

template <bool LDS, int WALKED_ONLY = 0, int DEFER = 2, bool MIXED = false, uint32_t FEATURES = kFeatAll>
struct SceneT : DevScene
{
    static constexpr uint32_t kFeatures = FEATURES;
    static constexpr bool kLds = LDS;
    static constexpr bool kMixed = MIXED;
    static constexpr bool kWalkedOnly = WALKED_ONLY != 0;
    static constexpr bool kQuadsInline = WALKED_ONLY == 2;
    static constexpr int kDefer = DEFER;
    const unsigned char* ldsBase;
    ConstF4 kPrims, kBoxes, kPlaneEq, kPlaneIdx;
    const float4* walkRec;
    uint32_t walkItem;
};

template <class SC> TN_D const Node64* mesh_nodes(const SC& sc, const DevMesh& m)
{
    if constexpr (SC::kLds && SC::kMixed) return m.inArena ? reinterpret_cast<const Node64*>(sc.ldsBase + m.offNodes) : m.nodes;
    else if constexpr (SC::kLds) return reinterpret_cast<const Node64*>(sc.ldsBase + m.offNodes); else return m.nodes;
}
template <class SC> TN_D const Tri48* mesh_tris(const SC& sc, const DevMesh& m)
{
    if constexpr (SC::kLds && SC::kMixed) return m.inArena ? reinterpret_cast<const Tri48*>(sc.ldsBase + m.offTris) : m.tris;
    else if constexpr (SC::kLds) return reinterpret_cast<const Tri48*>(sc.ldsBase + m.offTris); else return m.tris;
}
template <class SC> TN_D const float* mesh_normals(const SC& sc, const DevMesh& m)
{
    if constexpr (SC::kLds && SC::kMixed) return m.inArena ? reinterpret_cast<const float*>(sc.ldsBase + m.offNormals) : m.normals;
    else if constexpr (SC::kLds) return reinterpret_cast<const float*>(sc.ldsBase + m.offNormals); else return m.normals;
}
template <class SC> TN_D const float* mesh_cdf(const SC& sc, const DevMesh& m)
{
    if constexpr (SC::kLds && SC::kMixed) return m.inArena ? reinterpret_cast<const float*>(sc.ldsBase + m.offCdf) : m.cdf;
    else if constexpr (SC::kLds) return reinterpret_cast<const float*>(sc.ldsBase + m.offCdf); else return m.cdf;
}

}
```

### tinsel_amd/renderer.py

```python
import ctypes as C
import os

import numpy as np

from . import abi

_HERE = os.path.dirname(os.path.abspath(__file__))
LIB_PATH = os.environ.get("TINSEL_HIP_LIB", os.path.join(_HERE, "libtinsel_hip.so"))

_lib = None
DEFAULT_TUNING = None


class TinselHipError(RuntimeError):
    pass


def load_library():
    global _lib
    if _lib is not None:
        return _lib
    if not os.path.exists(LIB_PATH):
        raise TinselHipError(
            "%s is missing: build it with `python -m tinsel_amd.build` (hipcc, gfx950). "
# ... 56 lines not shown
        L.tinsel_hip_render_features.argtypes = [vp, C.POINTER(abi.Camera), C.POINTER(abi.Options), C.c_uint32, ci, C.c_uint, vp]
        L.tinsel_hip_render_features_device.argtypes = [vp, C.POINTER(abi.Camera), C.POINTER(abi.Options), C.c_uint32, ci, C.c_uint, vp, vp]
    if hasattr(L, "tinsel_hip_render_id_mattes"):
        L.tinsel_hip_render_id_mattes.argtypes = [vp, C.POINTER(abi.Camera), C.POINTER(abi.Options), C.c_uint32, ci, ci, vp, vp]
        L.tinsel_hip_render_id_mattes_device.argtypes = [vp, C.POINTER(abi.Camera), C.POINTER(abi.Options), C.c_uint32, ci, ci, vp, vp, vp]
    if hasattr(L, "tinsel_hip_render_light_groups"):
        L.tinsel_hip_render_light_groups.argtypes = [vp, C.POINTER(abi.Camera), C.POINTER(abi.Options), C.c_uint32, ci, ci, vp, ci, vp]
        L.tinsel_hip_render_light_groups_device.argtypes = [vp, C.POINTER(abi.Camera), C.POINTER(abi.Options), C.c_uint32, ci, ci, vp, ci, vp, vp]
    if hasattr(L, "tinsel_hip_render_views"):
        L.tinsel_hip_render_views.argtypes = [vp, C.POINTER(abi.Camera), ci, C.POINTER(abi.Options), C.c_uint32, ci, C.c_uint, vp]
        L.tinsel_hip_render_views_device.argtypes = [vp, C.POINTER(abi.Camera), ci, C.POINTER(abi.Options), C.c_uint32, ci, C.c_uint, vp, vp]
        L.tinsel_hip_plan_views.argtypes = [C.c_ulonglong, ci, ci, ci, ci, C.POINTER(C.c_int)]
    if hasattr(L, "tinsel_hip_render_sample_map"):
        L.tinsel_hip_render_sample_map.argtypes = abi.RENDER_SAMPLE_MAP_ARGTYPES
        L.tinsel_hip_render_sample_map_device.argtypes = abi.RENDER_SAMPLE_MAP_DEVICE_ARGTYPES
        L.tinsel_hip_plan_sample_map.argtypes = abi.PLAN_SAMPLE_MAP_ARGTYPES
    if hasattr(L, "tinsel_hip_denoise"):
        L.tinsel_hip_denoise_params_init.restype = None
        L.tinsel_hip_denoise_params_init.argtypes = [C.POINTER(abi.DenoiseParams)]
        L.tinsel_hip_denoise.argtypes = [vp, vp, vp, C.c_uint, ci, ci, C.POINTER(abi.DenoiseParams), vp]
        L.tinsel_hip_denoise_device.argtypes = [vp, vp, vp, C.c_uint, ci, ci, C.POINTER(abi.DenoiseParams), vp, vp]
        L.tinsel_hip_present_image_device.argtypes = [vp, vp, C.POINTER(abi.Options), ci, C.c_float, vp]
    L.tinsel_hip_kernel_times.argtypes = [vp, C.POINTER(abi.KernelTime), ci]
    L.tinsel_hip_enable_kernel_timing.argtypes = [vp, ci]
    L.tinsel_hip_set_batch_paths.argtypes = [vp, C.c_ulonglong]
    L.tinsel_hip_read_batch_radiance.restype = C.c_longlong
    L.tinsel_hip_read_batch_radiance.argtypes = [vp, vp, C.c_ulonglong]
    L.tinsel_hip_leaf.argtypes = [vp, ci, ci, ci, vp, ci, vp, vp, ci, C.POINTER(abi.Camera), ci, ci]
    L.tinsel_hip_write_accum.argtypes = [vp, vp, C.c_uint32]
    L.tinsel_hip_reserve.argtypes = [vp, ci, ci]
    L.tinsel_hip_set_russian_roulette.argtypes = [vp, ci]
    L.tinsel_hip_set_mesh_bvh.argtypes = [vp, ci, C.POINTER(C.c_double)]
    L.tinsel_hip_present.argtypes = [vp, C.POINTER(abi.Options), ci, C.c_float, vp]
    L.tinsel_hip_present_async.argtypes = [vp, C.POINTER(abi.Options), ci, C.c_float, vp]
    L.tinsel_hip_present_device_ptr.restype = vp
    L.tinsel_hip_present_device_ptr.argtypes = [vp]
    L.tinsel_image_quantize_rgb8.argtypes = [vp, ci, ci, vp]
    L.tinsel_hip_stack_entries.argtypes = [vp]
    if hasattr(L, "tinsel_hip_mesh_tree"):
        L.tinsel_hip_mesh_tree.argtypes = [vp, ci, vp, ci, C.POINTER(C.c_int)]
    L.tinsel_hip_nee_per_path.argtypes = [vp]
    L.tinsel_hip_walked_prims.argtypes = [vp]
    if hasattr(L, "tinsel_hip_walk_tops"):
        L.tinsel_hip_walk_tops.argtypes = [vp, C.POINTER(C.c_int), ci]
    if hasattr(L, "tinsel_hip_bounce_plan"):
        L.tinsel_hip_bounce_plan.argtypes = [vp, C.POINTER(C.c_uint32)]
        L.tinsel_hip_scene_features.restype = C.c_uint
        L.tinsel_hip_scene_features.argtypes = [C.POINTER(abi.SceneDesc)]
    if hasattr(L, "tinsel_hip_scene_slim"):
        L.tinsel_hip_scene_slim.argtypes = [C.POINTER(abi.SceneDesc)]
    if hasattr(L, "tinsel_hip_scene_plane_pairs"):
        L.tinsel_hip_scene_plane_pairs.argtypes = [C.POINTER(abi.SceneDesc), C.POINTER(C.c_int32), C.c_int, C.POINTER(C.c_int)]
        L.tinsel_hip_plane_table.argtypes = [vp, C.POINTER(C.c_int)]
    if hasattr(L, "tinsel_hip_queue_counts"):
        L.tinsel_hip_queue_counts.argtypes = [vp, C.POINTER(C.c_uint32), C.c_int]
    L.tinsel_hip_set_lookahead.argtypes = [vp, ci]
    L.tinsel_hip_refit_mesh.argtypes = [vp, ci, vp, ci, vp]
    if hasattr(L, "tinsel_hip_rebuild_scene"):
        L.tinsel_hip_set_primitive_transform.argtypes = [vp, ci, C.POINTER(abi.Transform), C.POINTER(abi.Transform)]
        L.tinsel_hip_rebuild_scene.argtypes = [vp, ci, vp, ci, C.POINTER(C.c_double)]
    L.tinsel_hip_set_probe_sampling.argtypes = [vp, ci]
    L.tinsel_hip_set_arithmetic.argtypes = [vp, ci]
    L.tinsel_hip_get_arithmetic.argtypes = [vp]
    L.tinsel_hip_group_create.restype = vp
    L.tinsel_hip_group_create.argtypes = [C.POINTER(abi.SceneDesc), ci, ci]
    L.tinsel_hip_group_destroy.restype = None
    L.tinsel_hip_group_destroy.argtypes = [vp]
    L.tinsel_hip_group_init.argtypes = [vp, ci, ci]
    L.tinsel_hip_group_render.argtypes = [vp, C.POINTER(abi.Camera), C.POINTER(abi.Options), vp, ci]
    L.tinsel_hip_group_present.argtypes = [vp, C.POINTER(abi.Options), ci, C.c_float, vp]
    L.tinsel_hip_group_size.argtypes = [vp]
    L.tinsel_hip_group_member.restype = vp
    L.tinsel_hip_group_member.argtypes = [vp, ci]
    L.tinsel_hip_group_set_lookahead.argtypes = [vp, ci]
    L.tinsel_hip_ubench.argtypes = [ci, ci, C.c_ulonglong, ci, C.POINTER(C.c_double), C.POINTER(C.c_double)]
    L.tinsel_hip_selftest_arith.argtypes = [ci, ci, ci, C.POINTER(C.c_ulonglong), C.POINTER(C.c_uint)]
    if hasattr(L, "tinsel_hip_selftest_sort"):
        L.tinsel_hip_selftest_sort.argtypes = [ci, vp, C.c_ulonglong, ci, ci]
        L.tinsel_hip_selftest_scan.argtypes = [ci, vp, vp, C.c_ulonglong]
    if hasattr(L, "tinsel_hip_selftest_accumulate"):
        L.tinsel_hip_selftest_accumulate.argtypes = abi.SELFTEST_ACCUMULATE_ARGTYPES
        L.tinsel_hip_accumulate_support.argtypes = [ci, C.c_float, C.c_float, C.c_float, C.POINTER(C.c_float)]
    L.tinsel_hip_plan_regions.argtypes = [C.c_ulonglong, ci, ci, ci, C.POINTER(C.c_uint)]
    L.tinsel_hip_last_error.restype = C.c_char_p
    L.tinsel_pack_open.argtypes = [vp, C.c_size_t, C.POINTER(abi.SceneDesc), C.POINTER(abi.Camera), C.POINTER(abi.Options)]
    _lib = L
    return L


EXPORTED_SYMBOLS = [
    "tinsel_hip_bounce_plan", "tinsel_hip_scene_features", "tinsel_hip_scene_slim", "tinsel_hip_scene_plane_pairs", "tinsel_hip_plane_table", "tinsel_hip_create", "tinsel_hip_destroy", "tinsel_hip_init", "tinsel_hip_init_external", "tinsel_hip_render",
    "tinsel_hip_render_async", "tinsel_hip_accum_device_ptr", "tinsel_hip_read_accum", "tinsel_hip_set_shard",
    "tinsel_hip_set_pipeline", "tinsel_hip_set_pass_index", "tinsel_hip_get_pass_index", "tinsel_hip_stats",
    "tinsel_hip_reset_stats", "tinsel_hip_stats_detail", "tinsel_hip_set_detail_counters", "tinsel_hip_render_cost", "tinsel_hip_kernel_times", "tinsel_hip_kernel_time_bytes",
    "tinsel_hip_enable_kernel_timing", "tinsel_hip_set_batch_paths", "tinsel_hip_stack_entries", "tinsel_hip_mesh_tree",
    "tinsel_hip_nee_per_path", "tinsel_hip_last_error", "tinsel_pack_open", "tinsel_hip_read_batch_radiance", "tinsel_hip_leaf",
    "tinsel_hip_write_accum", "tinsel_hip_reserve", "tinsel_hip_set_russian_roulette", "tinsel_hip_set_mesh_bvh", "tinsel_hip_present", "tinsel_hip_present_async", "tinsel_hip_present_device_ptr", "tinsel_image_quantize_rgb8",
    "tinsel_hip_walked_prims", "tinsel_hip_walk_tops", "tinsel_hip_queue_counts", "tinsel_hip_set_lookahead", "tinsel_hip_set_arithmetic", "tinsel_hip_get_arithmetic", "tinsel_hip_refit_mesh", "tinsel_hip_set_probe_sampling",
    "tinsel_hip_set_primitive_transform", "tinsel_hip_rebuild_scene",
    "tinsel_hip_group_create", "tinsel_hip_group_destroy", "tinsel_hip_group_init", "tinsel_hip_group_render", "tinsel_hip_group_present",
    "tinsel_hip_group_size", "tinsel_hip_group_member", "tinsel_hip_group_set_lookahead", "tinsel_hip_ubench",
    "tinsel_hip_selftest_arith", "tinsel_hip_selftest_sort", "tinsel_hip_selftest_scan", "tinsel_hip_selftest_accumulate", "tinsel_hip_accumulate_support", "tinsel_hip_plan_regions",
    "tinsel_hip_tuning_init", "tinsel_hip_create_tuned", "tinsel_hip_set_tuning", "tinsel_hip_get_tuning", "tinsel_hip_group_create_tuned",
    "tinsel_hip_comm_unique_id", "tinsel_hip_comm_init", "tinsel_hip_comm_size", "tinsel_hip_comm_reduce_accum",
    "tinsel_hip_trace_rays", "tinsel_hip_trace_rays_device", "tinsel_hip_trace_camera",
    "tinsel_hip_trace_radiance", "tinsel_hip_trace_radiance_device",
    "tinsel_hip_gather_radiance", "tinsel_hip_gather_radiance_device",
    "tinsel_hip_gather_sh", "tinsel_hip_gather_sh_device",
    "tinsel_hip_render_features", "tinsel_hip_render_features_device",
    "tinsel_hip_render_id_mattes", "tinsel_hip_render_id_mattes_device",
    "tinsel_hip_render_light_groups", "tinsel_hip_render_light_groups_device",
    "tinsel_hip_render_views", "tinsel_hip_render_views_device", "tinsel_hip_plan_views",
    "tinsel_hip_render_sample_map", "tinsel_hip_render_sample_map_device", "tinsel_hip_plan_sample_map",
    "tinsel_hip_denoise_params_init", "tinsel_hip_denoise", "tinsel_hip_denoise_device", "tinsel_hip_present_image_device",
]


def rank_id_lists(ids, weights):
    ids, weights = np.asarray(ids, np.int32), np.asarray(weights, np.float32)
    empty = ids == abi.ID_EMPTY
    order = np.lexsort((ids, -weights.astype(np.float64), empty), axis=0)
    return np.take_along_axis(ids, order, 0), np.take_along_axis(weights, order, 0)


def matte(result, ids):
    wanted = np.isin(np.asarray(result["ids"]), np.atleast_1d(np.asarray(ids, np.int64)))
    wanted &= np.asarray(result["ids"]) != abi.ID_EMPTY
    total = np.asarray(result["total"], np.float32)
    s = np.where(wanted, np.asarray(result["weights"], np.float32), np.float32(0)).sum(axis=0, dtype=np.float32)
    out = np.zeros(total.shape, np.float32)
    np.divide(s, total, out=out, where=total != 0)
    return out


def merge_id_mattes(results, slots):
    results = list(results)
    slots = int(slots)
    if not results or not 1 <= slots:
        raise ValueError("merge_id_mattes: at least one result and one slot")
    H, W = np.asarray(results[0]["total"]).shape
    cap = sum(np.asarray(r["ids"]).shape[0] for r in results)
    ids = np.full((cap, H, W), abi.ID_EMPTY, np.int32)
    weights = np.zeros((cap, H, W), np.float32)
# ... 274 lines not shown
    for k, v in fields.items():
        if k not in names:
            raise TypeError("tinsel_hip_denoise_params has no field %r" % k)
        setattr(p, k, v)
    return p


def _is_tensor(a):
    return a is not None and not isinstance(a, np.ndarray) and hasattr(a, "data_ptr")


def _check(rc, what):
    if rc != 0:
        msg = load_library().tinsel_hip_last_error()
        raise TinselHipError("%s failed: %s" % (what, msg.decode() if msg else "?"))


def _host_ptr(a):
    return (a if a.size else np.zeros(1, a.dtype)).ctypes.data_as(C.c_void_p)


class Scene:

    def __init__(self, blob: bytes):
        L = load_library()
        self._buf = C.create_string_buffer(blob, len(blob))
        self.desc = abi.SceneDesc()
        self.camera = abi.Camera()
        self.options = abi.Options()
        _check(L.tinsel_pack_open(self._buf, len(blob), C.byref(self.desc), C.byref(self.camera), C.byref(self.options)),
               "tinsel_pack_open")

    @classmethod
    def load_pack(cls, path):
        with open(path, "rb") as fh:
            return cls(fh.read())

    @property
    def num_primitives(self):
        return self.desc.num_primitives

    def bounce_features(self):
        return int(load_library().tinsel_hip_scene_features(C.byref(self.desc)))

    def bounce_slim(self):
        return bool(load_library().tinsel_hip_scene_slim(C.byref(self.desc)))

    def plane_pairs(self):
        n = max(1, self.num_primitives//2)
        out = (C.c_int32*(2*n))()
        singles = C.c_int(0)
        k = load_library().tinsel_hip_scene_plane_pairs(C.byref(self.desc), out, n, C.byref(singles))
        return [(out[2*q], out[2*q + 1]) for q in range(k)], singles.value


def _bytes_at(ptr, n):
    return C.string_at(ptr, n) if (ptr and n > 0) else b""


_libc = C.CDLL(None)
_libc.memcmp.argtypes = [C.c_void_p, C.c_void_p, C.c_size_t]


def _same_bytes(pa, pb, n):
    if n <= 0 or pa == pb:
        return True
    return bool(pa) and bool(pb) and _libc.memcmp(pa, pb, n) == 0


def _same_nodes(pa, pb, n):
    if n <= 0 or _same_bytes(pa, pb, n*32):
        return True
    a = np.ctypeslib.as_array((C.c_uint32*(n*8)).from_address(pa)).reshape(n, 8)
    b = np.ctypeslib.as_array((C.c_uint32*(n*8)).from_address(pb)).reshape(n, 8)
    if not np.array_equal(a[:, :7], b[:, :7]):
        return False
    leaf_a, leaf_b = a[:, 7] >> 31, b[:, 7] >> 31
    if not np.array_equal(leaf_a, leaf_b):
        return False
    inner = leaf_a == 0
    return bool(np.array_equal(a[inner, 7], b[inner, 7]))


def scene_delta(old: Scene, new: Scene):
    a, b = old.desc, new.desc
    if a.num_primitives != b.num_primitives or bytes(a.sky_horizon) != bytes(b.sky_horizon) or bytes(a.sky_zenith) != bytes(b.sky_zenith):
        return None
    if (a.probe_valid, a.probe_width, a.probe_height) != (b.probe_valid, b.probe_width, b.probe_height):
        return None
    if a.probe_valid and not _same_bytes(a.probe_data, b.probe_data, a.probe_width*a.probe_height*16):
        return None
    P = a.num_primitives
    pa, pb = (abi.Primitive*P).from_address(a.primitives), (abi.Primitive*P).from_address(b.primitives)
    moves = []
    for i in range(P):
        x, y = pa[i], pb[i]
        mx, my = bytes(x.material), bytes(y.material)
        if x.type != y.type or x.light_samples != y.light_samples or mx[:84] != my[:84] or mx[112:] != my[112:]:
            return None
        if x.type == abi.GEOM_SPHERE and x.geo.sphere.radius != y.geo.sphere.radius:
            return None
        if x.type == abi.GEOM_PLANE and bytes(x.geo.plane) != bytes(y.geo.plane):
            return None
        if x.type == abi.GEOM_MESH:
            g, h = x.geo.mesh, y.geo.mesh
            if (g.num_vertices, g.num_indices, g.num_nodes, g.area) != (h.num_vertices, h.num_indices, h.num_nodes, h.area):
                return None
            for f, n in (("positions", g.num_vertices*12), ("normals", g.num_vertices*12), ("indices", g.num_indices*4), ("cdf", (g.num_indices//3)*4)):
                if not _same_bytes(getattr(g, f), getattr(h, f), n):
                    return None
            if not _same_nodes(g.nodes, h.nodes, g.num_nodes):
                return None
        if bytes(x.start_transform) != bytes(y.start_transform) or bytes(x.end_transform) != bytes(y.end_transform):
            moves.append((i, abi.Transform.from_buffer_copy(bytes(y.start_transform)), abi.Transform.from_buffer_copy(bytes(y.end_transform))))
    nodes = (abi.BVHNode*b.num_bvh_nodes).from_buffer_copy(_bytes_at(b.bvh_nodes, b.num_bvh_nodes*C.sizeof(abi.BVHNode)))
    return moves, nodes


class HipRenderer:

    def __init__(self, scene: Scene, device: int = 0, tuning: "abi.Tuning | None" = None):
        L = load_library()
        self._L = L
        tuning = tuning if tuning is not None else DEFAULT_TUNING
        if tuning is None:
            self._h = L.tinsel_hip_create(C.byref(scene.desc), device)
        else:
            self._h = L.tinsel_hip_create_tuned(C.byref(scene.desc), device, C.byref(tuning))
        if not self._h:
            msg = L.tinsel_hip_last_error()
            raise TinselHipError("tinsel_hip_create failed: %s" % (msg.decode() if msg else "?"))
        self.device = device
        self.num_primitives = int(scene.desc.num_primitives)
        self.width = self.height = 0
        self._accum_tensor = None

    def init(self, width, height, accum_tensor=None):
        if accum_tensor is not None:
            assert tuple(accum_tensor.shape) == (height, width, 4) and accum_tensor.is_contiguous()
            self._accum_tensor = accum_tensor
            _check(self._L.tinsel_hip_init_external(self._h, width, height, accum_tensor.data_ptr()), "tinsel_hip_init_external")
        else:
            self._accum_tensor = None
            _check(self._L.tinsel_hip_init(self._h, width, height), "tinsel_hip_init")
        self.width, self.height = width, height

    def render(self, camera, options, output=None, passes=1, readback=True):
        if output is None and readback:
            output = np.empty((options.height, options.width, 4), np.float32)
        ptr = output.ctypes.data_as(C.c_void_p) if (readback and output is not None) else None
        _check(self._L.tinsel_hip_render(self._h, C.byref(camera), C.byref(options), ptr, passes), "tinsel_hip_render")
        return output

    Init = init
    Render = render

    def render_async(self, camera, options, passes=1, stream=None):
        _check(self._L.tinsel_hip_render_async(self._h, C.byref(camera), C.byref(options), passes, stream), "tinsel_hip_render_async")

    def read_accum(self):
        out = np.empty((self.height, self.width, 4), np.float32)
        _check(self._L.tinsel_hip_read_accum(self._h, out.ctypes.data_as(C.c_void_p)), "tinsel_hip_read_accum")
        return out

    def set_mesh_bvh(self, mode):
        ms = C.c_double(0.0)
        _check(self._L.tinsel_hip_set_mesh_bvh(self._h, int(mode), C.byref(ms)), "tinsel_hip_set_mesh_bvh")
        return ms.value

    def write_accum(self, accum, next_pass_index):
        accum = np.ascontiguousarray(accum, np.float32)
        assert accum.shape == (self.height, self.width, 4)
        _check(self._L.tinsel_hip_write_accum(self._h, accum.ctypes.data_as(C.c_void_p), int(next_pass_index)), "tinsel_hip_write_accum")

    def present(self, options, nlm_width=0, nlm_falloff=200.0, readback=True):
        out = np.empty((self.height, self.width, 4), np.float32) if readback else None
        ptr = out.ctypes.data_as(C.c_void_p) if readback else None
        _check(self._L.tinsel_hip_present(self._h, C.byref(options), int(nlm_width), float(nlm_falloff), ptr), "tinsel_hip_present")
        return out

    @property
    def accum_tensor(self):
        return self._accum_tensor

    def accum_device_ptr(self):
        return self._L.tinsel_hip_accum_device_ptr(self._h)

    def set_shard(self, rank, world, tile=32):
        _check(self._L.tinsel_hip_set_shard(self._h, rank, world, tile), "tinsel_hip_set_shard")

    def set_pipeline(self, pipeline):
        _check(self._L.tinsel_hip_set_pipeline(self._h, pipeline), "tinsel_hip_set_pipeline")

    @staticmethod
    def comm_unique_id():
        buf = (C.c_ubyte*abi.COMM_ID_BYTES)()
        _check(load_library().tinsel_hip_comm_unique_id(buf, abi.COMM_ID_BYTES), "tinsel_hip_comm_unique_id")
        return bytes(buf)

    def comm_init(self, id_bytes, rank, world):
        buf = (C.c_ubyte*abi.COMM_ID_BYTES).from_buffer_copy(bytes(id_bytes))
        _check(self._L.tinsel_hip_comm_init(self._h, buf, int(rank), int(world)), "tinsel_hip_comm_init")

    def comm_size(self):
        return int(self._L.tinsel_hip_comm_size(self._h)) if hasattr(self._L, "tinsel_hip_comm_size") else 0

    def comm_reduce_accum(self, out_ptr, root=0, stream=None):
        _check(self._L.tinsel_hip_comm_reduce_accum(self._h, out_ptr, int(root), stream), "tinsel_hip_comm_reduce_accum")

    def set_tuning(self, tuning=None, **fields):
        t = (tuning if tuning is not None else self.get_tuning()).replace(**fields)
        _check(self._L.tinsel_hip_set_tuning(self._h, C.byref(t)), "tinsel_hip_set_tuning")

    def plane_table(self):
        out = (C.c_int*2)()
        _check(self._L.tinsel_hip_plane_table(self._h, out), "tinsel_hip_plane_table")
        return out[0], out[1]

    def get_tuning(self):
        t = abi.Tuning()
        _check(self._L.tinsel_hip_get_tuning(self._h, C.byref(t)), "tinsel_hip_get_tuning")
        return t

    def set_arithmetic(self, mode):
        _check(self._L.tinsel_hip_set_arithmetic(self._h, int(mode)), "tinsel_hip_set_arithmetic")

    def refit_mesh(self, primitive, positions, normals=None):
        positions = np.ascontiguousarray(positions, np.float32)
        nptr = None
        if normals is not None:
            normals = np.ascontiguousarray(normals, np.float32)
            nptr = normals.ctypes.data_as(C.c_void_p)
        _check(self._L.tinsel_hip_refit_mesh(self._h, int(primitive), positions.ctypes.data_as(C.c_void_p), int(positions.shape[0]), nptr),
               "tinsel_hip_refit_mesh")

    def set_primitive_transform(self, index, start, end=None):
        end = start if end is None else end
        _check(self._L.tinsel_hip_set_primitive_transform(self._h, int(index), C.byref(start), C.byref(end)), "tinsel_hip_set_primitive_transform")

    def rebuild_scene(self, nodes=None):
        ms = C.c_double(0.0)
        if nodes is None:
            rc = self._L.tinsel_hip_rebuild_scene(self._h, abi.SCENE_BVH_DEVICE, None, 0, C.byref(ms))
        else:
            rc = self._L.tinsel_hip_rebuild_scene(self._h, abi.SCENE_BVH_NODES, C.cast(nodes, C.c_void_p), len(nodes), C.byref(ms))
        _check(rc, "tinsel_hip_rebuild_scene")
        return ms.value

    def update_scene(self, old: Scene, new: Scene):
        d = scene_delta(old, new)
        if d is None:
            return False
        moves, nodes = d
        for i, s, e in moves:
            self.set_primitive_transform(i, s, e)
        self.rebuild_scene(nodes)
        return True

    def set_probe_sampling(self, mode):
        _check(self._L.tinsel_hip_set_probe_sampling(self._h, int(mode)), "tinsel_hip_set_probe_sampling")

    def set_lookahead(self, on):
        _check(self._L.tinsel_hip_set_lookahead(self._h, int(on)), "tinsel_hip_set_lookahead")

    def set_russian_roulette(self, start_bounce):
        _check(self._L.tinsel_hip_set_russian_roulette(self._h, int(start_bounce)), "tinsel_hip_set_russian_roulette")

    def reserve(self, passes, max_depth):
        _check(self._L.tinsel_hip_reserve(self._h, int(passes), int(max_depth)), "tinsel_hip_reserve")

    def get_pass_index(self):
        return int(self._L.tinsel_hip_get_pass_index(self._h))

    def set_pass_index(self, i):
        _check(self._L.tinsel_hip_set_pass_index(self._h, i), "tinsel_hip_set_pass_index")

    def set_batch_paths(self, n):
        _check(self._L.tinsel_hip_set_batch_paths(self._h, n), "tinsel_hip_set_batch_paths")

    def set_detail_counters(self, on):
        _check(self._L.tinsel_hip_set_detail_counters(self._h, int(on)), "tinsel_hip_set_detail_counters")

    def render_cost(self, camera, options, pass_begin=0, passes=1):
        out = np.zeros((options.height, options.width, 4), np.uint32)
        _check(self._L.tinsel_hip_render_cost(self._h, C.byref(camera), C.byref(options), int(pass_begin), int(passes),
                                              out.ctypes.data_as(C.c_void_p)), "tinsel_hip_render_cost")
        return out

    def features(self, camera, options, pass_begin=0, passes=1, which=abi.FEATURE_NAMES, out=None):
        mask, names = feature_mask(which)
        H, W = int(options.height), int(options.width)
        shape = (max(len(names), 1), H, W, 4)
        if out is not None and not isinstance(out, np.ndarray) and hasattr(out, "data_ptr"):
            import torch
            if out.dtype != torch.float32 or tuple(out.shape) != shape or not out.is_contiguous() or not out.is_cuda:
                raise ValueError("features: a contiguous float32 tensor %s on the GPU is expected" % (shape,))
            if out.device.index != self.device:
                raise ValueError("features: the tensor is on %s, the renderer on device %d" % (out.device, self.device))
            _check(self._L.tinsel_hip_render_features_device(self._h, C.byref(camera), C.byref(options), int(pass_begin), int(passes), mask,
                                                             out.data_ptr(), torch.cuda.current_stream(out.device).cuda_stream),
                   "tinsel_hip_render_features_device")
        else:
            if out is None:
                out = np.zeros(shape, np.float32)
            elif out.dtype != np.float32 or out.shape != shape or not out.flags.c_contiguous:
                raise ValueError("features: a C-contiguous float32 array %s is expected" % (shape,))
            _check(self._L.tinsel_hip_render_features(self._h, C.byref(camera), C.byref(options), int(pass_begin), int(passes), mask,
                                                      out.ctypes.data_as(C.c_void_p)), "tinsel_hip_render_features")
        return {n: out[k] for k, n in enumerate(names)}

    def light_groups(self, camera, options, pass_begin, passes, groups, env_group=None, out=None):
        table = np.ascontiguousarray(np.asarray(groups).reshape(-1), np.int32)
        env = -1 if env_group is None else int(env_group)
        if out is not None:
            G = int(out.shape[0])
        else:
            G = max(int(table.max()) if table.size else -1, env) + 1
        if table.size != self.num_primitives:
            raise ValueError("light_groups: groups has %d entries, the scene %d primitives" % (table.size, self.num_primitives))
        H, W = int(options.height), int(options.width)
        shape = (max(G, 1), H, W, 4)
        if _is_tensor(out):
# ... 520 lines not shown
```

Before: 6902 Msamples/s.

## Bake scene constants into a JIT-compiled specialized bounce kernel

Generates a per-scene header containing primitives, plane equations, boxes and light tables as constexpr data. It compiles a specialized closed-FIT k_bounce instance through hipcc at runtime, caches the code object and installs it when the workload is large enough. This is meant to remove scene loads from LDS and memory and let the compiler unroll and constant-fold intersection and light selection. The cost is runtime compile latency, register-pressure checks that can refuse the bake, and a dependency on a compiler being available.

```diff
diff --git a/include/tinsel_hip.h b/include/tinsel_hip.h
--- a/include/tinsel_hip.h
+++ b/include/tinsel_hip.h
@@ -371,6 +371,15 @@
 int tinsel_hip_scene_plane_pairs(const tinsel_scene_desc* scene, int32_t* out_pairs, int capacity, int* out_singles);
 int tinsel_hip_plane_table(tinsel_hip* r, int* out2);
 int tinsel_hip_scene_slim(const tinsel_scene_desc* scene);
+long long tinsel_hip_bake_source(tinsel_hip* r, char* out_text, unsigned long long capacity, char* out_key65, int* out_bakeable);
+long long tinsel_hip_bake_source_desc(const tinsel_scene_desc* scene, const tinsel_hip_tuning* tuning, char* out_text, unsigned long long capacity,
+                                      char* out_key65, int* out_bakeable);
+int tinsel_hip_install_baked(tinsel_hip* r, const void* image, unsigned long long bytes, const char* key, int how);
+int tinsel_hip_bake_status(tinsel_hip* r, uint32_t* out3, char* out_key65);
+int tinsel_hip_set_bounce_bake(tinsel_hip* r, int mode);
+int tinsel_hip_get_bounce_bake(tinsel_hip* r);
+enum { TINSEL_BAKE_OFF = 0, TINSEL_BAKE_NOT_BAKEABLE = 1, TINSEL_BAKE_NO_COMPILER = 2, TINSEL_BAKE_COMPILED = 3, TINSEL_BAKE_FROM_CACHE = 4,
+       TINSEL_BAKE_STALE = 5, TINSEL_BAKE_NONE = 6, TINSEL_BAKE_LDS_REFUSED = 7 };
 enum { TINSEL_BOUNCE_MEDIA = 1, TINSEL_BOUNCE_PROBE = 2, TINSEL_BOUNCE_MOTION = 4, TINSEL_BOUNCE_MESH_WALK = 8, TINSEL_BOUNCE_SPHERE = 16,
        TINSEL_BOUNCE_TRANSMISSION = 32, TINSEL_BOUNCE_POOLS = 64, TINSEL_BOUNCE_SHARE = 128, TINSEL_BOUNCE_SORT = 256, TINSEL_BOUNCE_ROULETTE = 512 };
 
diff --git a/tinsel_amd/abi.py b/tinsel_amd/abi.py
--- a/tinsel_amd/abi.py
+++ b/tinsel_amd/abi.py
@@ -178,6 +178,10 @@
 BOUNCE_TRANSMISSION, BOUNCE_POOLS, BOUNCE_SHARE, BOUNCE_SORT, BOUNCE_ROULETTE = 32, 64, 128, 256, 512
 
 
+BAKE_OFF, BAKE_NOT_BAKEABLE, BAKE_NO_COMPILER, BAKE_COMPILED, BAKE_FROM_CACHE, BAKE_STALE, BAKE_NONE, BAKE_LDS_REFUSED = 0, 1, 2, 3, 4, 5, 6, 7
+BAKE_AUTO_MIN_PATHS = 64 << 20
+
+
 class Tuning(C.Structure):
     _fields_ = [("struct_bytes", C.c_uint32),
                 ("flat_scan", C.c_int32), ("lds_scene", C.c_int32), ("walk", C.c_int32), ("inline_max_tris", C.c_int32), ("walk_min_tris", C.c_int32),
@@ -187,11 +191,13 @@
                 ("shade_sorted", C.c_int32), ("overlap", C.c_int32), ("scene_walk", C.c_int32), ("swalk_lds", C.c_int32), ("accumulate", C.c_int32),
                 ("walk_block", C.c_int32), ("walk_single", C.c_int32), ("walk_lds_stack", C.c_int32), ("walk_refill_min", C.c_int32), ("walk_leaf_min", C.c_int32),
                 ("walk_grid_mult", C.c_int32), ("quads_in_scan", C.c_int32), ("bounce_fit", C.c_int32), ("plane_pairs", C.c_int32)]
+    BINDING_FIELDS = ("bounce_bake",)
+    bounce_bake = -1
     CREATE_FIELDS = ("flat_scan", "lds_scene", "walk", "inline_max_tris", "walk_min_tris", "small_mesh_bytes", "arena_lds_limit")
     _DEFAULTS = dict(flat_scan=-1, lds_scene=-1, walk=-1, inline_max_tris=-1, walk_min_tris=-1, small_mesh_bytes=-1, arena_lds_limit=-1,
                      batch_paths=0, grid_mult=0, bounce_share=-1, repack=-1, tail_split=-1, tail_share=0.0, tail_divide=4,
                      shade_sorted=-1, overlap=-1, scene_walk=-1, swalk_lds=-1, accumulate=0,
-                     walk_block=0, walk_single=-1, walk_lds_stack=-1, walk_refill_min=0, walk_leaf_min=0, walk_grid_mult=0, quads_in_scan=-1, bounce_fit=-1, plane_pairs=-1)
+                     walk_block=0, walk_single=-1, walk_lds_stack=-1, walk_refill_min=0, walk_leaf_min=0, walk_grid_mult=0, quads_in_scan=-1, bounce_fit=-1, plane_pairs=-1, bounce_bake=-1)
 
     def __init__(self, **over):
         super().__init__()
diff --git a/tinsel_amd/build.py b/tinsel_amd/build.py
--- a/tinsel_amd/build.py
+++ b/tinsel_amd/build.py
@@ -54,6 +54,83 @@
     for p, cmd in zip(procs, jobs):
         if p.wait() != 0:
             raise subprocess.CalledProcessError(p.returncode, cmd)
+
+
+SRC_BAKED = os.path.join(HERE, "csrc", "tinsel_baked.hip")
+BAKE_CACHE_ENV = "TINSEL_BAKE_CACHE"
+
+
+def bake_cache_dir():
+    return os.environ.get(BAKE_CACHE_ENV) or os.path.join(OBJ_DIR, "baked")
+
+
+def _bake_cache_name(key, cc):
+    h = hashlib.sha256()
+    h.update(key.encode())
+    csrc = os.path.join(HERE, "csrc")
+    for f in sorted(os.listdir(csrc)):
+        if f.endswith(".h") or f == os.path.basename(SRC_BAKED):
+            h.update(f.encode())
+            h.update(_sha(os.path.join(csrc, f)).encode())
+    h.update(" ".join(HIPCC_FLAGS).encode())
+    h.update(subprocess.run([cc, "--version"], capture_output=True, text=True).stdout.encode())
+    return "k_bounce_baked_%s.co" % h.hexdigest()[:32]
+
+
+def bake_command(cc, header, out, extra=()):
+    return [cc] + HIPCC_FLAGS + list(extra) + ["--cuda-device-only", "-DTN_BAKED_HEADER=\"%s\"" % header, "-c", SRC_BAKED, "-o", out]
+
+
+BAKED_KERNEL = "k_bounce<2,1,0>"
+
+
+def baked_refusal(res):
+    if not res:
+        return "the compiler reported no resources for %s" % BAKED_KERNEL
+    if res.get("waves_per_simd") != 4 or res.get("scratch_bytes") != 0 or res.get("vgprs", 0) > 128:
+        return "%s at %s waves per SIMD, %s VGPRs, %s B of scratch (wanted: 4, <= 128, 0)" % (
+            BAKED_KERNEL, res.get("waves_per_simd"), res.get("vgprs"), res.get("scratch_bytes"))
+    return None
+
+
+def bake(text, key, verbose=False):
+    if hashlib.sha256(text.encode()).hexdigest() != key:
+        return None, "the key is not the sha256 of the text"
+    try:
+        cc = hipcc()
+    except RuntimeError:
+        return None, "no compiler"
+    try:
+        path = os.path.join(bake_cache_dir(), _bake_cache_name(key, cc))
+        if os.path.exists(path):
+            with open(path, "rb") as f:
+                return f.read(), "cache"
+        with tempfile.TemporaryDirectory(prefix="tinsel_bake_") as tmp:
+            header = os.path.join(tmp, "scene_%s.h" % key[:16])
+            with open(header, "w") as f:
+                f.write(text)
+            cmd = bake_command(cc, header, "baked.co", extra=["-Rpass-analysis=kernel-resource-usage"])
+            if verbose:
+                print("[tinsel_amd.build] (in %s)" % tmp, " ".join(cmd), flush=True)
+            p = subprocess.run(cmd, cwd=tmp, capture_output=True, text=True)
+            if p.returncode != 0:
+                return None, "compile failed: " + p.stderr[-2000:]
+            why = baked_refusal(_parse_resources(p.stderr).get(BAKED_KERNEL))
+            if why:
+                return None, "refused: " + why
+            with open(os.path.join(tmp, "baked.co"), "rb") as f:
+                image = f.read()
+    except OSError as e:
+        return None, "compiler unavailable: %s" % e
+    try:
+        os.makedirs(os.path.dirname(path), exist_ok=True)
+        fd, part = tempfile.mkstemp(prefix=".part_", dir=os.path.dirname(path))
+        with os.fdopen(fd, "wb") as f:
+            f.write(image)
+        os.replace(part, path)
+    except OSError:
+        pass
+    return image, "compiled"
 
 
 def _resource_job(tmp):
diff --git a/tinsel_amd/csrc/tinsel_baked.hip b/tinsel_amd/csrc/tinsel_baked.hip
--- /dev/null
+++ b/tinsel_amd/csrc/tinsel_baked.hip
@@ -0,0 +1,7 @@
+#ifndef TN_BAKED_HEADER
+#error "tinsel_baked.hip is compiled with -DTN_BAKED_HEADER=\"<generated header>\" (tinsel_amd/build.py bake())"
+#endif
+
+#include "tn_fused.h"
+
+template __global__ void tn::k_bounce<tn::kBounceFitClosed, true, false>(tn::BounceKernargs);
diff --git a/tinsel_amd/csrc/tinsel_hip.hip b/tinsel_amd/csrc/tinsel_hip.hip
--- a/tinsel_amd/csrc/tinsel_hip.hip
+++ b/tinsel_amd/csrc/tinsel_hip.hip
@@ -61,6 +61,7 @@
 #include "tn_host_own.h"
 #include "tn_host_layout.h"
 #include "tn_host_state.h"
+#include "tn_host_bake.h"
 #include "tn_host_batch.h"
 #include "tn_host_query.h"
 #include "tn_host_radiance.h"
diff --git a/tinsel_amd/csrc/tn_baked.h b/tinsel_amd/csrc/tn_baked.h
--- /dev/null
+++ b/tinsel_amd/csrc/tn_baked.h
@@ -0,0 +1,213 @@
+#pragma once
+
+#if TN_BAKED_SCENE
+
+namespace tn {
+namespace baked {
+
+TN_D constexpr float word_f(uint32_t bits) { return __builtin_bit_cast(float, bits); }
+
+template <int K> struct Slot { static constexpr int v = K; };
+template <int B, int E, class F>
+TN_D void static_for(F&& fn)
+{
+    if constexpr (B < E)
+    {
+        fn(Slot<B>());
+        static_for<B + 1, E>(fn);
+    }
+}
+
+template <int S> TN_D ConstF4V plane_eq()
+{
+    static_assert(S >= 0 && S < kPlaneSlots, "a slot of the plane table");
+    return ConstF4V{ word_f(kPlaneEq[S*4]), word_f(kPlaneEq[S*4 + 1]), word_f(kPlaneEq[S*4 + 2]), word_f(kPlaneEq[S*4 + 3]) };
+}
+
+template <int I> TN_D Prim64 prim()
+{
+    static_assert(I >= 0 && I < kNumPrims, "a primitive of the scene");
+    constexpr int w = I*16;
+    Prim64 p;
+    p.px = word_f(kPrims[w]); p.py = word_f(kPrims[w + 1]); p.pz = word_f(kPrims[w + 2]); p.s = word_f(kPrims[w + 3]);
+    p.rx = word_f(kPrims[w + 4]); p.ry = word_f(kPrims[w + 5]); p.rz = word_f(kPrims[w + 6]); p.rw = word_f(kPrims[w + 7]);
+    p.g0 = word_f(kPrims[w + 8]); p.g1 = word_f(kPrims[w + 9]); p.g2 = word_f(kPrims[w + 10]); p.g3 = word_f(kPrims[w + 11]);
+    p.type = kPrims[w + 12]; p.flags = kPrims[w + 13]; p.mesh = kPrims[w + 14]; p.moving = kPrims[w + 15];
+    return p;
+}
+
+constexpr int kLightSelectMax = 4;
+template <class SC> TN_D Prim64 light_prim(const SC& sc, int index)
+{
+    if constexpr (kNumLights >= 1 && kNumLights <= kLightSelectMax)
+    {
+        Prim64 p = prim<(int)kLights[0]>();
+        static_for<1, kNumLights>([&](auto l) {
+            constexpr int k = (int)kLights[decltype(l)::v*4];
+            if (index == k)
+                p = prim<k>();
+        });
+        return p;
+    }
+    else
+        return load_prim(sc.prims, index);
+}
+
+struct LightMat
+{
+    int light;
+    const Mat128* mats;
+    template <int W> TN_D float word(float loaded) const
+    {
+        if constexpr (kNumLights >= 1 && kNumLights <= kLightSelectMax)
+        {
+            float x = word_f(kLightMat[W]);
+            static_for<1, kNumLights>([&](auto l) {
+                if (light == (int)kLights[decltype(l)::v*4])
+                    x = word_f(kLightMat[decltype(l)::v*4 + W]);
+            });
+            return x;
+        }
+        else
+            return loaded;
+    }
+    TN_D float rcpArea() const { return word<0>(mats[light].rcpArea); }
+    TN_D float cbsdf() const { return word<1>(mats[light].cbsdf); }
+    TN_D float clight() const { return word<2>(mats[light].clight); }
+};
+
+struct LightCursor
+{
+    int li = 0, sInLight = 0;
+    TN_D int next()
+    {
+        while (sInLight >= (int)kLights[li*4 + 1]) { ++li; sInLight = 0; }
+        ++sInLight;
+        return (int)kLights[li*4];
+    }
+};
+
+template <int FROM, class Accept>
+TN_D void single_planes(V3 o, V3 d, Accept& accept)
+{
+    constexpr int blocks = kNumPlanes > FROM ? (kNumPlanes - FROM)/4 : 0;
+    static_for<0, blocks>([&](auto b) {
+        constexpr int pk = FROM + 4*decltype(b)::v;
+        const ConstF4V e0 = plane_eq<pk>(), e1 = plane_eq<pk + 1>(), e2 = plane_eq<pk + 2>(), e3 = plane_eq<pk + 3>();
+        float t0, t1, t2, t3;
+        const bool h0 = ray_plane(o, d, e0.x, e0.y, e0.z, e0.w, t0);
+        const bool h1 = ray_plane(o, d, e1.x, e1.y, e1.z, e1.w, t1);
+        const bool h2 = ray_plane(o, d, e2.x, e2.y, e2.z, e2.w, t2);
+        const bool h3 = ray_plane(o, d, e3.x, e3.y, e3.z, e3.w, t3);
+        if (h0) accept((int)kPlaneIdx[pk], t0, V3(e0.x, e0.y, e0.z));
+        if (h1) accept((int)kPlaneIdx[pk + 1], t1, V3(e1.x, e1.y, e1.z));
+        if (h2) accept((int)kPlaneIdx[pk + 2], t2, V3(e2.x, e2.y, e2.z));
+        if (h3) accept((int)kPlaneIdx[pk + 3], t3, V3(e3.x, e3.y, e3.z));
+    });
+    static_for<FROM + 4*blocks, kNumPlanes>([&](auto s) {
+        constexpr int pk = decltype(s)::v;
+        const ConstF4V e0 = plane_eq<pk>();
+        float t0;
+        if (ray_plane(o, d, e0.x, e0.y, e0.z, e0.w, t0))
+            accept((int)kPlaneIdx[pk], t0, V3(e0.x, e0.y, e0.z));
+    });
+}
+
+}
+
+template <class SC, class Stack, bool COUNT>
+TN_D int trace_flat_baked(const SC& sc, Stack& st, V3 o, V3 d, V3 rcp, float time, float& outT, V3& outN, bool& tie, TraceCounters& ctr)
+{
+    static_assert(SC::kBaked && SC::kDefer == 0 && SC::kFeatures != kFeatAll, "the closed FIT instance");
+    float minT = kFltMax;
+    int closest = -1;
+    V3 cn;
+    tie = false;
+
+    auto accept = [&](int i, float t, V3 n) {
+        if (t > 0.0f)
+        {
+            if (fabsf(t - minT) <= 1e-5f*fabsf(t))
+                tie = true;
+            if (t < minT)
+            {
+                minT = t;
+                closest = i;
+                cn = n;
+            }
+        }
+    };
+    const bool finiteAll = __all(finite_bits(rcp.x) && finite_bits(rcp.y) && finite_bits(rcp.z) &&
+                                 finite_bits(o.x) && finite_bits(o.y) && finite_bits(o.z));
+
+    constexpr bool kPairBlock = baked::kPlanePairEnd >= 8;
+    bool paired = false;
+    if constexpr (kPairBlock)
+    {
+        const ConstF4V e0 = baked::plane_eq<0>(), e1 = baked::plane_eq<1>(), e2 = baked::plane_eq<2>(), e3 = baked::plane_eq<3>(), e4 = baked::plane_eq<4>();
+        constexpr uint32_t idr = baked::kPlaneIdx[4], ids = baked::kPlaneIdx[5];
+        const PlanePair p0 = plane_pair_pick(o.x, o.y, o.z, d.x, d.y, d.z, e0.x, e0.y, e0.z, e0.w, e1.w);
+        const PlanePair p1 = plane_pair_pick(o.x, o.y, o.z, d.x, d.y, d.z, e2.x, e2.y, e2.z, e2.w, e3.w);
+        if (!__any(p0.both || p1.both))
+        {
+            paired = true;
+            auto accept_of_pair = [&](const PlanePair& pp, const ConstF4V& ea, const ConstF4V& eb, int ia, int ib) {
+                float t;
+                if (plane_pair_hit(pp, t))
+                {
+                    if (fabsf(t - minT) <= 1e-5f*fabsf(t))
+                        tie = true;
+                    if (t < minT)
+                    {
+                        minT = t;
+                        if (pp.b) { closest = ib; cn = V3(eb.x, eb.y, eb.z); }
+                        else      { closest = ia; cn = V3(ea.x, ea.y, ea.z); }
+                    }
+                }
+            };
+            float t4;
+            const bool h4 = ray_plane(o, d, e4.x, e4.y, e4.z, e4.w, t4);
+            accept_of_pair(p0, e0, e1, (int)(ids & 255u), (int)((ids >> 8) & 255u));
+            accept_of_pair(p1, e2, e3, (int)((ids >> 16) & 255u), (int)(ids >> 24));
+            if (h4) accept((int)idr, t4, V3(e4.x, e4.y, e4.z));
+        }
+    }
+    if constexpr (kPairBlock)
+    {
+        if (paired)
+            baked::single_planes<8>(o, d, accept);
+        else
+            baked::single_planes<0>(o, d, accept);
+    }
+    else
+        baked::single_planes<0>(o, d, accept);
+
+    baked::static_for<0, baked::kNumPrims>([&](auto ic) {
+        constexpr int i = decltype(ic)::v;
+        if constexpr (((baked::kScanMask >> i) & 1ull) != 0ull)
+        {
+            if constexpr (baked::kBoxes[i*8 + 6] == 0u)
+            {
+                constexpr int w = i*8;
+                const float minx = baked::word_f(baked::kBoxes[w]), miny = baked::word_f(baked::kBoxes[w + 1]), minz = baked::word_f(baked::kBoxes[w + 2]),
+                            maxx = baked::word_f(baked::kBoxes[w + 3]), maxy = baked::word_f(baked::kBoxes[w + 4]), maxz = baked::word_f(baked::kBoxes[w + 5]);
+                float tb;
+                if (!(finiteAll ? ray_aabb_minmax(o, rcp, minx, miny, minz, maxx, maxy, maxz, tb) : ray_aabb(o, rcp, minx, miny, minz, maxx, maxy, maxz, tb)))
+                    return;
+            }
+            const Prim64 rec = baked::prim<i>();
+            float t;
+            V3 n;
+            if (prim_intersect<SC, Stack, COUNT, false, true>(sc, i, st, 0, o, d, time, t, n, ctr, 0.0f, rcp, true, &rec))
+                accept(i, t, n);
+        }
+    });
+
+    outT = minT;
+    outN = face_forward(cn, -d);
+    return closest;
+}
+
+}
+
+#endif
diff --git a/tinsel_amd/csrc/tn_fused.h b/tinsel_amd/csrc/tn_fused.h
--- a/tinsel_amd/csrc/tn_fused.h
+++ b/tinsel_amd/csrc/tn_fused.h
@@ -106,6 +106,13 @@
     constexpr int POOL = SLIM ? kPoolFieldsSlim : kPoolFields;
     static_assert(!SLIM || !(FEAT & (kFeatMedia | kFeatMotion | kFeatTransmission | kFeatProbe)), "the slim state has no word for these");
     typedef SceneT<LDS, false, DEFER ? 1 : 0, false, FEAT> SC;
+#if TN_BAKED_SCENE
+    if constexpr (SC::kBaked)
+    {
+        static_assert(kBounceWaves == 4, "v103 is four waves' threshold");
+        asm volatile("" ::: "v103");
+    }
+#endif
     const DevScene& scIn = ka.scIn;
     const SplitState& ss = ka.ss;
     const QueueCtl& q = ka.q;
@@ -325,11 +332,19 @@
                     HitCtx h;
                     on_hit_begin<SLIM>(p, mat, t, n, bounce, h, prim);
 
-                    if (sc.totalLightSamples > 0)
+#if TN_BAKED_SCENE
+                    constexpr bool BAKED = SC::kBaked;
+                    const bool anyLightSamples = BAKED ? baked::kTotalLightSamples > 0 : sc.totalLightSamples > 0;
+                    baked::LightCursor bakedLights;
+#else
+                    constexpr bool BAKED = false;
+                    const bool anyLightSamples = sc.totalLightSamples > 0;
+#endif
+                    if (anyLightSamples)
                     {
                         const V3 thrAtNee = p.thr;
                         LightCursor lights;
-                        V3 sum = nee_sum(sc, [&](int k) -> V3 {
+                        auto contrib = [&](int k) -> V3 {
                             NeeGeo g;
                             V3 skyColor;
                             float skyPdf = 0.0f;
@@ -338,6 +353,9 @@
                                 nee_sample_probe(late_sky(), h.p, h.n, p.rng, g, skyColor, skyPdf);
                             else
                             {
+#if TN_BAKED_SCENE
+                                if constexpr (BAKED) light = bakedLights.next(); else
+#endif
                                 light = lights.next(sc);
                                 nee_sample_light(sc, h.p, h.n, p.time, light, p.rng, g);
                             }
@@ -352,8 +370,16 @@
                                 return (hp < 0) ? nee_contrib_probe<SLIM>(mat_at(prim), h, g.wi, skyColor, skyPdf) : V3(0.0f);
                             if (!nee_light_reached(g, hp, ts))
                                 return V3(0.0f);
+#if TN_BAKED_SCENE
+                            if constexpr (BAKED) return nee_contrib_light_baked<SLIM>(sc, mat_at(prim), h, g.wi, g.nl, light, hp, ts);
+#endif
                             return nee_contrib_light<SLIM>(sc, mat_at(prim), h, g.wi, g.nl, light, hp, ts);
-                        });
+                        };
+#if TN_BAKED_SCENE
+                        const V3 sum = BAKED ? nee_sum_baked(contrib) : nee_sum(sc, contrib);
+#else
+                        const V3 sum = nee_sum(sc, contrib);
+#endif
                         p.rad = p.rad + thrAtNee*sum;
                     }
 
diff --git a/tinsel_amd/csrc/tn_host_api.h b/tinsel_amd/csrc/tn_host_api.h
--- a/tinsel_amd/csrc/tn_host_api.h
+++ b/tinsel_amd/csrc/tn_host_api.h
@@ -1029,6 +1029,78 @@
     return 0;
 }
 
+long long tinsel_hip_bake_source(tinsel_hip* r, char* out_text, unsigned long long capacity, char* out_key65, int* out_bakeable)
+{
+    if (!r)
+        return fail("bake_source: null renderer");
+    return bake_source_of(r, out_text, capacity, out_key65, out_bakeable);
+}
+
+int tinsel_hip_install_baked(tinsel_hip* r, const void* image, unsigned long long bytes, const char* key, int how)
+{
+    if (!r)
+        return fail("install_baked: null renderer");
+    if (!image && how == TINSEL_BAKE_NO_COMPILER)
+    {
+        if (!r->baked.fn)
+            r->baked.how = how;
+        return 0;
+    }
+    if (!image || bytes < 64 || !key || strlen(key) != 64 || (how != TINSEL_BAKE_COMPILED && how != TINSEL_BAKE_FROM_CACHE))
+        return fail("install_baked: bad arguments (a code object, its 64-digit key, TINSEL_BAKE_COMPILED or _FROM_CACHE)");
+    lookahead_cancel(r);
+    HIP_TRY(hipSetDevice(r->device));
+    HIP_TRY(hipDeviceSynchronize());
+    Module fresh;
+    if (fresh.load(image))
+        return -1;
+    hipFunction_t fn = nullptr;
+    HIP_TRY(hipModuleGetFunction(&fn, fresh, kBakedKernelName));
+    uint32_t ldsLimit = 65536;
+    if (hipFuncSetAttribute((const void*)fn, hipFuncAttributeMaxDynamicSharedMemorySize, r->sharedMemLimit) == hipSuccess)
+        ldsLimit = (uint32_t)r->sharedMemLimit;
+    else
+        (void)hipGetLastError();
+    r->baked.module = std::move(fresh);
+    r->baked.fn = fn;
+    r->baked.key = key;
+    r->baked.how = how;
+    r->baked.ldsLimit = ldsLimit;
+    r->baked.launches = 0;
+    return 0;
+}
+
+int tinsel_hip_set_bounce_bake(tinsel_hip* r, int mode)
+{
+    if (!r || mode < -1 || mode > 1)
+        return fail("set_bounce_bake: bad arguments (-1 auto, 0 never, 1 always)");
+    lookahead_cancel(r);
+    r->baked.mode = mode;
+    return 0;
+}
+
+int tinsel_hip_get_bounce_bake(tinsel_hip* r) { return r ? r->baked.mode : -1; }
+
+int tinsel_hip_bake_status(tinsel_hip* r, uint32_t* out3, char* out_key65)
+{
+    if (!r || !out3)
+        return fail("bake_status: bad arguments");
+    if (out_key65)
+        memcpy(out_key65, r->baked.fn ? r->baked.key.c_str() : "", r->baked.fn ? 65 : 1);
+    out3[1] = (uint32_t)(r->baked.launches & 0xffffffffull);
+    out3[2] = (uint32_t)(r->baked.launches >> 32);
+    if (r->baked.mode == 0)
+        out3[0] = TINSEL_BAKE_OFF;
+    else if (!plans_fit_closed(r, nullptr))
+        out3[0] = TINSEL_BAKE_NOT_BAKEABLE;
+    else if (!r->baked.fn)
+        out3[0] = r->baked.how == TINSEL_BAKE_NO_COMPILER ? TINSEL_BAKE_NO_COMPILER : TINSEL_BAKE_NONE;
+    else
+        out3[0] = r->baked.key != bake_live_key(r) ? (uint32_t)TINSEL_BAKE_STALE :
+                  stack_bytes(r) > (size_t)r->baked.ldsLimit ? (uint32_t)TINSEL_BAKE_LDS_REFUSED : (uint32_t)r->baked.how;
+    return 0;
+}
+
 int tinsel_hip_queue_counts(tinsel_hip* r, uint32_t* out, int max_bounces)
 {
     if (!r || !out || max_bounces < 1)
diff --git a/tinsel_amd/csrc/tn_host_bake.h b/tinsel_amd/csrc/tn_host_bake.h
--- /dev/null
+++ b/tinsel_amd/csrc/tn_host_bake.h
@@ -0,0 +1,147 @@
+#pragma once
+
+namespace {
+
+std::string sha256_hex(const std::string& msg)
+{
+    static const uint32_t K[64] = {
+        0x428a2f98u, 0x71374491u, 0xb5c0fbcfu, 0xe9b5dba5u, 0x3956c25bu, 0x59f111f1u, 0x923f82a4u, 0xab1c5ed5u, 0xd807aa98u, 0x12835b01u, 0x243185beu, 0x550c7dc3u,
+        0x72be5d74u, 0x80deb1feu, 0x9bdc06a7u, 0xc19bf174u, 0xe49b69c1u, 0xefbe4786u, 0x0fc19dc6u, 0x240ca1ccu, 0x2de92c6fu, 0x4a7484aau, 0x5cb0a9dcu, 0x76f988dau,
+        0x983e5152u, 0xa831c66du, 0xb00327c8u, 0xbf597fc7u, 0xc6e00bf3u, 0xd5a79147u, 0x06ca6351u, 0x14292967u, 0x27b70a85u, 0x2e1b2138u, 0x4d2c6dfcu, 0x53380d13u,
+        0x650a7354u, 0x766a0abbu, 0x81c2c92eu, 0x92722c85u, 0xa2bfe8a1u, 0xa81a664bu, 0xc24b8b70u, 0xc76c51a3u, 0xd192e819u, 0xd6990624u, 0xf40e3585u, 0x106aa070u,
+        0x19a4c116u, 0x1e376c08u, 0x2748774cu, 0x34b0bcb5u, 0x391c0cb3u, 0x4ed8aa4au, 0x5b9cca4fu, 0x682e6ff3u, 0x748f82eeu, 0x78a5636fu, 0x84c87814u, 0x8cc70208u,
+        0x90befffau, 0xa4506cebu, 0xbef9a3f7u, 0xc67178f2u };
+    uint32_t h[8] = { 0x6a09e667u, 0xbb67ae85u, 0x3c6ef372u, 0xa54ff53au, 0x510e527fu, 0x9b05688cu, 0x1f83d9abu, 0x5be0cd19u };
+    std::string m = msg;
+    const unsigned long long bits = (unsigned long long)msg.size()*8ull;
+    m.push_back((char)0x80);
+    while (m.size() % 64 != 56)
+        m.push_back((char)0);
+    for (int k = 7; k >= 0; --k)
+        m.push_back((char)((bits >> (8*k)) & 255ull));
+    auto rotr = [](uint32_t x, int n) { return (x >> n) | (x << (32 - n)); };
+    for (size_t off = 0; off < m.size(); off += 64)
+    {
+        uint32_t w[64];
+        for (int t = 0; t < 16; ++t)
+            w[t] = ((uint32_t)(unsigned char)m[off + 4*t] << 24) | ((uint32_t)(unsigned char)m[off + 4*t + 1] << 16) |
+                   ((uint32_t)(unsigned char)m[off + 4*t + 2] << 8) | (uint32_t)(unsigned char)m[off + 4*t + 3];
+        for (int t = 16; t < 64; ++t)
+        {
+            const uint32_t s0 = rotr(w[t - 15], 7) ^ rotr(w[t - 15], 18) ^ (w[t - 15] >> 3), s1 = rotr(w[t - 2], 17) ^ rotr(w[t - 2], 19) ^ (w[t - 2] >> 10);
+            w[t] = w[t - 16] + s0 + w[t - 7] + s1;
+        }
+        uint32_t a = h[0], b = h[1], c = h[2], d = h[3], e = h[4], f = h[5], g = h[6], hh = h[7];
+        for (int t = 0; t < 64; ++t)
+        {
+            const uint32_t S1 = rotr(e, 6) ^ rotr(e, 11) ^ rotr(e, 25), ch = (e & f) ^ (~e & g), t1 = hh + S1 + ch + K[t] + w[t];
+            const uint32_t S0 = rotr(a, 2) ^ rotr(a, 13) ^ rotr(a, 22), maj = (a & b) ^ (a & c) ^ (b & c), t2 = S0 + maj;
+            hh = g; g = f; f = e; e = d + t1; d = c; c = b; b = a; a = t1 + t2;
+        }
+        h[0] += a; h[1] += b; h[2] += c; h[3] += d; h[4] += e; h[5] += f; h[6] += g; h[7] += hh;
+    }
+    char out[65];
+    for (int k = 0; k < 8; ++k)
+        snprintf(out + 8*k, 9, "%08x", h[k]);
+    return std::string(out, 64);
+}
+
+struct BakeTables
+{
+    int numPrims = 0, numPlanes = 0, planePairEnd = 0, totalLightSamples = 0;
+    unsigned long long scanMask = 0;
+    std::vector<uint32_t> planeEq, planeIdx, boxes, prims, lights, lightMat;
+};
+
+inline uint32_t word_of(float f) { uint32_t u; memcpy(&u, &f, 4); return u; }
+
+std::string bake_text(const BakeTables& t)
+{
+    std::string s;
+    s += "// tinsel_hip baked scene level: generated by tinsel_hip_bake_source, read by tn_baked.h (which says what each table holds)\n";
+    s += "#pragma once\n#include <stdint.h>\nnamespace tn { namespace baked {\n";
+    char buf[96];
+    auto scalar = [&](const char* name, long long v) { snprintf(buf, sizeof(buf), "constexpr int %s = %lld;\n", name, v); s += buf; };
+    std::vector<uint32_t> planeEq = t.planeEq, planeIdx = t.planeIdx, lights = t.lights, lightMat = t.lightMat;
+    planeIdx.resize(std::max<size_t>(planeIdx.size(), 8), 0u);
+    planeEq.resize(planeIdx.size()*4, 0u);
+    lights.resize(std::max<size_t>(lights.size(), 4), 0u);
+    lightMat.resize(std::max<size_t>(lightMat.size(), 4), 0u);
+    scalar("kNumPrims", t.numPrims);
+    scalar("kNumPlanes", t.numPlanes);
+    scalar("kPlanePairEnd", t.planePairEnd);
+    scalar("kPlaneSlots", (long long)planeIdx.size());
+    scalar("kNumLights", (long long)(t.lights.size()/4));
+    scalar("kTotalLightSamples", t.totalLightSamples);
+    snprintf(buf, sizeof(buf), "constexpr unsigned long long kScanMask = 0x%016llxull;\n", t.scanMask);
+    s += buf;
+    auto table = [&](const char* name, const std::vector<uint32_t>& w) {
+        snprintf(buf, sizeof(buf), "constexpr uint32_t %s[%zu] = {", name, std::max<size_t>(w.size(), 1));
+        s += buf;
+        for (size_t k = 0; k < w.size(); ++k)
+        {
+            snprintf(buf, sizeof(buf), "%s0x%08xu,", k % 8 == 0 ? "\n    " : " ", w[k]);
+            s += buf;
+        }
+        if (w.empty())
+            s += " 0u";
+        s += "\n};\n";
+    };
+    table("kPlaneEq", planeEq);
+    table("kPlaneIdx", planeIdx);
+    table("kBoxes", t.boxes);
+    table("kPrims", t.prims);
+    table("kLights", lights);
+    table("kLightMat", lightMat);
+    s += "} }\n";
+    return s;
+}
+
+BakeTables bake_tables(const tinsel_hip* r)
+{
+    BakeTables t;
+    t.numPrims = r->scene.numPrims;
+    t.numPlanes = r->scene.numPlanes;
+    t.planePairEnd = r->scene.planePairEnd;
+    t.totalLightSamples = r->scene.totalLightSamples;
+    t.scanMask = r->scene.scanMask;
+    for (const float f : r->levelPlaneEq)
+        t.planeEq.push_back(word_of(f));
+    for (const int32_t k : r->levelPlaneIdx)
+        t.planeIdx.push_back((uint32_t)k);
+    for (const PrimBox& b : r->levelBoxes)
+    {
+        const uint32_t w[8] = { word_of(b.minx), word_of(b.miny), word_of(b.minz), word_of(b.maxx), word_of(b.maxy), word_of(b.maxz), b.alwaysHit, 0u };
+        t.boxes.insert(t.boxes.end(), w, w + 8);
+    }
+    for (const Prim64& p : r->primsHost)
+    {
+        const uint32_t w[16] = { word_of(p.px), word_of(p.py), word_of(p.pz), word_of(p.s), word_of(p.rx), word_of(p.ry), word_of(p.rz), word_of(p.rw),
+                                 word_of(p.g0), word_of(p.g1), word_of(p.g2), word_of(p.g3), p.type, p.flags, p.mesh, p.moving };
+        t.prims.insert(t.prims.end(), w, w + 16);
+    }
+    for (size_t l = 0; l < r->lightPrims.size() && l < r->lightMats.size(); ++l)
+    {
+        const Mat128& m = r->lightMats[l];
+        const uint32_t rec[4] = { (uint32_t)r->lightPrims[l], (uint32_t)m.lightSamples, word_of(m.rcpLightSamples), 0u };
+        const uint32_t mat[4] = { word_of(m.rcpArea), word_of(m.cbsdf), word_of(m.clight), word_of(m.rcpLightSamples) };
+        t.lights.insert(t.lights.end(), rec, rec + 4);
+        t.lightMat.insert(t.lightMat.end(), mat, mat + 4);
+    }
+    return t;
+}
+
+std::string bake_live_key(const tinsel_hip* r) { return sha256_hex(bake_text(bake_tables(r))); }
+
+constexpr const char* kBakedKernelName = "_ZN2tn8k_bounceILi2ELb1ELb0EEEvNS_14BounceKernargsE";
+
+int launch_baked(tinsel_hip* r, const LaunchArgs& a, hipStream_t st)
+{
+    BounceKernargs ka{ a.scene, a.ss, a.ctl, a.bounce, a.bounceEnd, a.stackEntries, a.cam, a.fp, a.passSeeds };
+    void* params[] = { &ka };
+    HIP_TRY(hipModuleLaunchKernel(r->baked.fn, (unsigned)a.grid, 1, 1, (unsigned)kBlock, 1, 1, a.ldsBytes, st, params, nullptr));
+    ++r->baked.launches;
+    return 0;
+}
+
+}
diff --git a/tinsel_amd/csrc/tn_host_batch.h b/tinsel_amd/csrc/tn_host_batch.h
--- a/tinsel_amd/csrc/tn_host_batch.h
+++ b/tinsel_amd/csrc/tn_host_batch.h
@@ -406,6 +406,34 @@
     if (deferMeshes)
         return within(kBounceFitDeferred) ? PK_BOUNCE_FIT_DEFERRED : PK_NONE;
     return within(kBounceFitClosed) ? PK_BOUNCE_FIT_CLOSED : PK_NONE;
+}
+
+bool plans_fit_closed(const tinsel_hip* r, std::string* why)
+{
+    auto no = [&](const char* w) { if (why) *why = w; return false; };
+    if (resolve_pipeline(r) != TINSEL_PIPELINE_WAVEFRONT)
+        return no("the scene does not run the fused pipeline");
+    if (residency(r->scene, r->scene.arenaLdsBytes) != RES_LDS)
+        return no("the scene is not staged whole into LDS");
+    if (r->countDetail)
+        return no("detail counters are on");
+    if (!r->scene.flatScan)
+        return no("the scene level is not a flat scan");
+    if (r->tune.bounce_fit == 0)
+        return no("tinsel_hip_tuning::bounce_fit is 0");
+    int resident = 0;
+    const uint32_t need = bounce_features(r, plan_bounce(r, &resident));
+    if (!scene_slim(need, r->anySubsurface))
+        return no("the scene is not slim (a medium, a probe, motion, a walked mesh, transmission or subsurface)");
+    if (fit_bounce(need, r->scene.deferMeshes != 0) != PK_BOUNCE_FIT_CLOSED)
+        return no(r->scene.deferMeshes ? "the scene defers its mesh walks (the deferred FIT instance is not baked)" : "the scene's features lie outside the closed FIT set");
+    return true;
+}
+
+bool baked_serves(const tinsel_hip* r, const LaunchArgs& a)
+{
+    return r->baked.fn != nullptr && r->baked.mode != 0 && r->arith == TINSEL_ARITH_EXACT && a.ldsBytes <= r->baked.ldsLimit &&
+           r->baked.key == bake_live_key(r);
 }
 
 struct WalkPlan
@@ -989,6 +1017,8 @@
                         (a.variant == PK_BOUNCE_COUNT_LDS || a.variant == PK_BOUNCE_COUNT) ? kBounceCount : kBounceGeneral;
     r->lastBounceFeatures = p.bounceFeatures | (a.fp.share ? kFeatShare : 0u);
     ScopedTimer t(r, KN_BOUNCE, st);
+    if (a.variant == PK_BOUNCE_FIT_CLOSED && baked_serves(r, a))
+        return launch_baked(r, a, st);
     return launch_path(r, a, st);
 }
 
diff --git a/tinsel_amd/csrc/tn_host_create.h b/tinsel_amd/csrc/tn_host_create.h
--- a/tinsel_amd/csrc/tn_host_create.h
+++ b/tinsel_amd/csrc/tn_host_create.h
@@ -24,9 +24,11 @@
     bool sceneHasBigMesh = false;
     SceneLevel lvl;
     bool flatScan = false;
-
-    SceneBuild(tinsel_hip* r_, const tinsel_scene_desc* d)
-        : r(r_), sc(r_->scene), desc(d), tune(r_->tune), P(d->num_primitives), prims((size_t)P), mats((size_t)P), moving((size_t)P)
+    bool dry = false;
+    template <class T> T* dry_address() const { return reinterpret_cast<T*>(uintptr_t(128)); }
+
+    SceneBuild(tinsel_hip* r_, const tinsel_scene_desc* d, bool dry_ = false)
+        : r(r_), sc(r_->scene), desc(d), tune(r_->tune), P(d->num_primitives), prims((size_t)P), mats((size_t)P), moving((size_t)P), dry(dry_)
     {
         for (int i = 0; i < P; ++i)
             if (desc->primitives[i].type == TINSEL_GEOM_MESH && mesh_bytes_estimate(desc->primitives[i].geo.mesh) > kSmallMeshBytes)
@@ -116,6 +118,10 @@
         dm.offTris = (uint32_t)arena.add(tris.data(), tris.size());
         dm.offNormals = (uint32_t)arena.add(&g.normals[0].x, (size_t)g.num_vertices*3);
         dm.offCdf = (uint32_t)arena.add(g.cdf, (size_t)numTris);
+    }
+    else if (dry)
+    {
+        dm.nodes = dry_address<const Node64>(); dm.tris = dry_address<const Tri48>(); dm.normals = dry_address<const float>(); dm.cdf = dry_address<const float>();
     }
     else
     {
@@ -256,6 +262,9 @@
     for (size_t l = 0; l < lights.size(); ++l)
         lightRecs[l] = { lights[l], mats[(size_t)lights[l]].lightSamples, mats[(size_t)lights[l]].rcpLightSamples, 0 };
     const size_t offLights = arena.add(lightRecs.data(), lightRecs.size());
+    r->lightMats.clear();
+    for (const int32_t l : lights)
+        r->lightMats.push_back(mats[(size_t)l]);
     const size_t offMeshes = arena.add(meshes.data(), meshes.size());
 
     int alwaysHitPlanes = 0;
@@ -283,7 +292,7 @@
     const size_t offPlaneIdx = arena.add(planeIdx.data(), planeIdx.size());
     arena.bytes.resize((arena.bytes.size() + 127) & ~size_t(127), 0);
 
-    unsigned char* arenaDev = r->sceneMem.upload(arena.bytes.data(), arena.bytes.size());
+    unsigned char* arenaDev = dry ? dry_address<unsigned char>() : r->sceneMem.upload(arena.bytes.data(), arena.bytes.size());
     if (!arenaDev)
         return fail("create: device allocation failed (scene arena)");
     DevMesh* hm = reinterpret_cast<DevMesh*>(&arena.bytes[offMeshes]);
@@ -297,7 +306,7 @@
             hm[m].cdf = reinterpret_cast<const float*>(arenaDev + hm[m].offCdf);
         }
     }
-    if (!meshes.empty() && hipMemcpy(arenaDev + offMeshes, hm, sizeof(DevMesh)*meshes.size(), hipMemcpyHostToDevice) != hipSuccess)
+    if (!dry && !meshes.empty() && hipMemcpy(arenaDev + offMeshes, hm, sizeof(DevMesh)*meshes.size(), hipMemcpyHostToDevice) != hipSuccess)
         return fail("create: device allocation failed (scene arena)");
     r->meshesRef.assign(hm, hm + meshes.size());
     r->meshesNow = r->meshesRef;
@@ -371,6 +380,11 @@
     const size_t n = (size_t)desc->probe_width*desc->probe_height;
     if (!desc->probe_data || !desc->probe_pdf_x || !desc->probe_cdf_x || !desc->probe_pdf_y || !desc->probe_cdf_y || n == 0)
         return fail("create: probe marked valid but arrays missing");
+    if (dry)
+    {
+        sc.probe.valid = 1;
+        return 0;
+    }
     sc.probe.data = (const float4*)r->sceneMem.upload((const float*)desc->probe_data, n*4);
     sc.probe.pdfX = r->sceneMem.upload(desc->probe_pdf_x, n);
     sc.probe.cdfX = r->sceneMem.upload(desc->probe_cdf_x, n);
@@ -388,8 +402,8 @@
 {
     r->neePerPath = totalLightSamples + (r->scene.probe.valid ? 1 : 0);
     r->scene.totalLightSamples = r->neePerPath;
-    if (r->statsDev.alloc((size_t)kStatShards*kStatWords) ||
-        hipMemset(r->statsDev.get(), 0, sizeof(unsigned long long)*kStatShards*kStatWords) != hipSuccess)
+    if (!dry && (r->statsDev.alloc((size_t)kStatShards*kStatWords) ||
+        hipMemset(r->statsDev.get(), 0, sizeof(unsigned long long)*kStatShards*kStatWords) != hipSuccess))
         return fail("create: device allocation failed (stats)");
     if (stack_bytes(r) > (size_t)r->sharedMemLimit && r->scene.arenaLdsBytes)
     {
@@ -401,6 +415,44 @@
     return 0;
 }
 
+int build_scene(tinsel_hip* r, const tinsel_scene_desc* desc, bool dry)
+{
+    memset(&r->scene, 0, sizeof(r->scene));
+    SceneBuild b(r, desc, dry);
+    if (b.add_primitives() || b.scene_level())
+        return -1;
+    b.mark_walked_and_quads();
+    if (b.assemble_arena())
+        return -1;
+    b.set_scene_flags();
+    if ((desc->probe_valid && b.upload_probe()) || b.stats_and_fit())
+        return -1;
+    return 0;
+}
+
+constexpr int kDescSharedMemLimit = 160*1024;
+
+long long bake_source_of(const tinsel_hip* r, char* out_text, unsigned long long capacity, char* out_key65, int* out_bakeable)
+{
+    const std::string text = bake_text(bake_tables(r));
+    if (out_text && capacity > 0)
+    {
+        const size_t n = std::min<size_t>(text.size(), (size_t)capacity - 1);
+        memcpy(out_text, text.data(), n);
+        out_text[n] = 0;
+    }
+    if (out_key65)
+        memcpy(out_key65, sha256_hex(text).c_str(), 65);
+    if (out_bakeable)
+    {
+        std::string why;
+        *out_bakeable = plans_fit_closed(r, &why) ? 1 : 0;
+        if (!*out_bakeable)
+            g_error = "bake_source: not bakeable: " + why;
+    }
+    return (long long)text.size();
+}
+
 }
 
 extern "C" {
@@ -439,17 +491,22 @@
 
     std::unique_ptr<tinsel_hip> r(new tinsel_hip());
     create_limits(r.get(), device_index, tuning);
-    memset(&r->scene, 0, sizeof(r->scene));
-    SceneBuild b(r.get(), desc);
-    if (b.add_primitives() || b.scene_level())
-        return nullptr;
-    b.mark_walked_and_quads();
-    if (b.assemble_arena())
-        return nullptr;
-    b.set_scene_flags();
-    if ((desc->probe_valid && b.upload_probe()) || b.stats_and_fit())
+    if (build_scene(r.get(), desc, false))
         return nullptr;
     return r.release();
+}
+
+long long tinsel_hip_bake_source_desc(const tinsel_scene_desc* desc, const tinsel_hip_tuning* tuning, char* out_text, unsigned long long capacity,
+                                      char* out_key65, int* out_bakeable)
+{
+    if (!desc || !desc->primitives || desc->num_primitives <= 0 || !desc->bvh_nodes || desc->num_bvh_nodes <= 0)
+        return fail("bake_source_desc: empty scene (Scene::Build must have run)");
+    std::unique_ptr<tinsel_hip> r(new tinsel_hip());
+    r->tune = tuning_from_caller(tuning);
+    r->sharedMemLimit = kDescSharedMemLimit;
+    if (build_scene(r.get(), desc, true))
+        return -1;
+    return bake_source_of(r.get(), out_text, capacity, out_key65, out_bakeable);
 }
 
 void tinsel_hip_destroy(tinsel_hip* r)
diff --git a/tinsel_amd/csrc/tn_host_own.h b/tinsel_amd/csrc/tn_host_own.h
--- a/tinsel_amd/csrc/tn_host_own.h
+++ b/tinsel_amd/csrc/tn_host_own.h
@@ -107,6 +107,17 @@
     }
 };
 
+struct Module : DevHandle<hipModule_t, hipModuleUnload>
+{
+    int load(const void* image)
+    {
+        Module fresh;
+        HIP_TRY(hipModuleLoadData(&fresh.h, image));
+        std::swap(h, fresh.h);
+        return 0;
+    }
+};
+
 struct PinnedOutput
 {
     PinnedOutput() = default;
diff --git a/tinsel_amd/csrc/tn_host_scene.h b/tinsel_amd/csrc/tn_host_scene.h
--- a/tinsel_amd/csrc/tn_host_scene.h
+++ b/tinsel_amd/csrc/tn_host_scene.h
@@ -202,6 +202,9 @@
     r->planePairs = lvl.planePairs;
     r->planeSingles = lvl.planeSingles;
     r->sceneStackNeed = lvl.bvh.maxLeafDepth + 1;
+    r->levelPlaneEq = lvl.planeEq;
+    r->levelPlaneIdx = lvl.planeIdx;
+    r->levelBoxes = lvl.boxes;
     r->sceneBvhHost = std::move(lvl.tree);
 }
 
@@ -253,6 +256,12 @@
     unsigned char* mat = const_cast<unsigned char*>(r->scene.arena) + r->arenaOffMats + sizeof(Mat128)*(size_t)p;
     HIP_TRY(hipMemcpy(mat + offsetof(Mat128, area), &area, sizeof(float), hipMemcpyHostToDevice));
     HIP_TRY(hipMemcpy(mat + offsetof(Mat128, rcpArea), &rcpArea, sizeof(float), hipMemcpyHostToDevice));
+    for (size_t l = 0; l < r->lightPrims.size() && l < r->lightMats.size(); ++l)
+        if (r->lightPrims[l] == p)
+        {
+            r->lightMats[l].area = area;
+            r->lightMats[l].rcpArea = rcpArea;
+        }
     return 0;
 }
 
diff --git a/tinsel_amd/csrc/tn_host_state.h b/tinsel_amd/csrc/tn_host_state.h
--- a/tinsel_amd/csrc/tn_host_state.h
+++ b/tinsel_amd/csrc/tn_host_state.h
@@ -66,6 +66,20 @@
     int lastBounceKind = -1;
     uint32_t lastBounceFeatures = 0;
     DevPool lbvhTrees;
+    std::vector<float> levelPlaneEq;
+    std::vector<int32_t> levelPlaneIdx;
+    std::vector<PrimBox> levelBoxes;
+    std::vector<Mat128> lightMats;
+    struct Baked
+    {
+        Module module;
+        hipFunction_t fn = nullptr;
+        std::string key;
+        int mode = -1;
+        int how = 0;
+        uint32_t ldsLimit = 65536;
+        unsigned long long launches = 0;
+    } baked;
 
     int width = 0, height = 0;
     float4* accum = nullptr;
diff --git a/tinsel_amd/csrc/tn_integrator.h b/tinsel_amd/csrc/tn_integrator.h
--- a/tinsel_amd/csrc/tn_integrator.h
+++ b/tinsel_amd/csrc/tn_integrator.h
@@ -111,7 +111,11 @@
 template <class SC>
 TN_D void primitive_sample(const SC& sc, int index, float time, V3& pos, V3& normal, Rng& rng)
 {
+#if TN_BAKED_SCENE
+    Prim64 p = [&] { if constexpr (SC::kBaked) return baked::light_prim(sc, index); else return load_prim(sc.prims, index); }();
+#else
     Prim64 p = load_prim(sc.prims, index);
+#endif
     if constexpr (!(SC::kFeatures & kFeatMotion))
         p.flags &= ~(uint32_t)kPrimMoving;
     const Xform x = prim_pose(sc, p, time);
@@ -219,16 +223,24 @@
     return e;
 }
 
-TN_D V3 nee_combine_light(const DevScene& sc, const NeeTerms& e, float nl, int light, int hitPrim, float t)
+struct LightMatLoaded
+{
+    const Mat128* m;
+    TN_D float rcpArea() const { return m->rcpArea; }
+    TN_D float cbsdf() const { return m->cbsdf; }
+    TN_D float clight() const { return m->clight; }
+};
+
+template <class LM>
+TN_D V3 nee_combine_light_of(const DevScene& sc, const NeeTerms& e, float nl, const LM& lm, int hitPrim, float t)
 {
     V3 L(0.0f);
-    const Mat128* lm = sc.mats + light;
     float tSq = t*t;
-    float lightPdf = (lm->rcpArea*tSq)/nl;
+    float lightPdf = (lm.rcpArea()*tSq)/nl;
     if (e.bsdfPdf > 0.0f)
     {
-        float cbsdf = lm->cbsdf;
-        float clight = lm->clight;
+        float cbsdf = lm.cbsdf();
+        float clight = lm.clight();
         float weight = clight*lightPdf/(cbsdf*e.bsdfPdf + clight*lightPdf);
         const Mat128* hm = sc.mats + hitPrim;
         V3 em(hm->emission[0], hm->emission[1], hm->emission[2]);
@@ -237,11 +249,40 @@
     return L;
 }
 
+TN_D V3 nee_combine_light(const DevScene& sc, const NeeTerms& e, float nl, int light, int hitPrim, float t)
+{
+    return nee_combine_light_of(sc, e, nl, LightMatLoaded{ sc.mats + light }, hitPrim, t);
+}
+
 template <bool SLIM = false>
 TN_D V3 nee_contrib_light(const DevScene& sc, const Mat& surf, const HitCtx& h, V3 wi, float nl, int light, int hitPrim, float t)
 {
     return nee_combine_light(sc, nee_bsdf_terms<SLIM>(surf, h, wi), nl, light, hitPrim, t);
 }
+
+#if TN_BAKED_SCENE
+template <bool SLIM = false>
+TN_D V3 nee_contrib_light_baked(const DevScene& sc, const Mat& surf, const HitCtx& h, V3 wi, float nl, int light, int hitPrim, float t)
+{
+    return nee_combine_light_of(sc, nee_bsdf_terms<SLIM>(surf, h, wi), nl, baked::LightMat{ light, sc.mats }, hitPrim, t);
+}
+
+template <class Contrib>
+TN_D V3 nee_sum_baked(Contrib contrib)
+{
+    V3 sum(0.0f);
+    int k = 0;
+    for (int li = 0; li < baked::kNumLights; ++li)
+    {
+        const int numSamples = (int)baked::kLights[li*4 + 1];
+        V3 L(0.0f);
+        for (int s = 0; s < numSamples; ++s)
+            L = L + contrib(k++);
+        sum = sum + L*baked::word_f(baked::kLights[li*4 + 2]);
+    }
+    return sum;
+}
+#endif
 
 TN_D void nee_sample_probe(const DevScene& sc, V3 hitP, V3 hitN, Rng& rng, NeeGeo& g, V3& skyColor, float& skyPdf)
 {
diff --git a/tinsel_amd/csrc/tn_isect.h b/tinsel_amd/csrc/tn_isect.h
--- a/tinsel_amd/csrc/tn_isect.h
+++ b/tinsel_amd/csrc/tn_isect.h
@@ -584,6 +584,12 @@
     return closest;
 }
 
+}
+
+#include "tn_baked.h"
+
+namespace tn {
+
 template <class SC>
 TN_D bool ray_meets_bounded_prim(const SC& sc, V3 o, V3 d)
 {
@@ -622,6 +628,14 @@
         const bool sane = ray_sane(o);
         bool tie = false;
         int prim = -1;
+#if TN_BAKED_SCENE
+        if constexpr (SC::kBaked)
+        {
+            if (sane)
+                prim = trace_flat_baked<SC, Stack, COUNT>(sc, st, o, d, rcp, time, outT, outN, tie, ctr);
+        }
+        else
+#endif
         if (sane)
             prim = trace_flat<SC, Stack, COUNT, false>(sc, st, o, d, rcp, time, outT, outN, tie, ctr, 0.0f);
         if (sane && !tie)
diff --git a/tinsel_amd/csrc/tn_scene.h b/tinsel_amd/csrc/tn_scene.h
--- a/tinsel_amd/csrc/tn_scene.h
+++ b/tinsel_amd/csrc/tn_scene.h
@@ -1,6 +1,13 @@
 #pragma once
 
 #include "tn_math.h"
+
+#ifdef TN_BAKED_HEADER
+#include TN_BAKED_HEADER
+#define TN_BAKED_SCENE 1
+#else
+#define TN_BAKED_SCENE 0
+#endif
 
 namespace tn {
 
@@ -190,6 +197,7 @@
     static constexpr bool kWalkedOnly = WALKED_ONLY != 0;
     static constexpr bool kQuadsInline = WALKED_ONLY == 2;
     static constexpr int kDefer = DEFER;
+    static constexpr bool kBaked = TN_BAKED_SCENE != 0 && LDS && WALKED_ONLY == 0 && DEFER == 0 && !MIXED && FEATURES == (uint32_t)kFeatSphere;
     const unsigned char* ldsBase;
     ConstF4 kPrims, kBoxes, kPlaneEq, kPlaneIdx;
     const float4* walkRec;
diff --git a/tinsel_amd/renderer.py b/tinsel_amd/renderer.py
--- a/tinsel_amd/renderer.py
+++ b/tinsel_amd/renderer.py
@@ -132,6 +132,15 @@
     if hasattr(L, "tinsel_hip_scene_plane_pairs"):
         L.tinsel_hip_scene_plane_pairs.argtypes = [C.POINTER(abi.SceneDesc), C.POINTER(C.c_int32), C.c_int, C.POINTER(C.c_int)]
         L.tinsel_hip_plane_table.argtypes = [vp, C.POINTER(C.c_int)]
+    if hasattr(L, "tinsel_hip_bake_source"):
+        L.tinsel_hip_bake_source.restype = C.c_longlong
+        L.tinsel_hip_bake_source.argtypes = [vp, C.c_char_p, C.c_ulonglong, C.c_char_p, C.POINTER(C.c_int)]
+        L.tinsel_hip_bake_source_desc.restype = C.c_longlong
+        L.tinsel_hip_bake_source_desc.argtypes = [C.POINTER(abi.SceneDesc), C.POINTER(abi.Tuning), C.c_char_p, C.c_ulonglong, C.c_char_p, C.POINTER(C.c_int)]
+        L.tinsel_hip_install_baked.argtypes = [vp, C.c_char_p, C.c_ulonglong, C.c_char_p, ci]
+        L.tinsel_hip_bake_status.argtypes = [vp, C.POINTER(C.c_uint32), C.c_char_p]
+        L.tinsel_hip_set_bounce_bake.argtypes = [vp, ci]
+        L.tinsel_hip_get_bounce_bake.argtypes = [vp]
     if hasattr(L, "tinsel_hip_queue_counts"):
         L.tinsel_hip_queue_counts.argtypes = [vp, C.POINTER(C.c_uint32), C.c_int]
     L.tinsel_hip_set_lookahead.argtypes = [vp, ci]
@@ -169,6 +178,7 @@
 
 
 EXPORTED_SYMBOLS = [
+    "tinsel_hip_bake_source", "tinsel_hip_bake_source_desc", "tinsel_hip_install_baked", "tinsel_hip_bake_status", "tinsel_hip_set_bounce_bake", "tinsel_hip_get_bounce_bake",
     "tinsel_hip_bounce_plan", "tinsel_hip_scene_features", "tinsel_hip_scene_slim", "tinsel_hip_scene_plane_pairs", "tinsel_hip_plane_table", "tinsel_hip_create", "tinsel_hip_destroy", "tinsel_hip_init", "tinsel_hip_init_external", "tinsel_hip_render",
     "tinsel_hip_render_async", "tinsel_hip_accum_device_ptr", "tinsel_hip_read_accum", "tinsel_hip_set_shard",
     "tinsel_hip_set_pipeline", "tinsel_hip_set_pass_index", "tinsel_hip_get_pass_index", "tinsel_hip_stats",
@@ -549,6 +559,22 @@
         singles = C.c_int(0)
         k = load_library().tinsel_hip_scene_plane_pairs(C.byref(self.desc), out, n, C.byref(singles))
         return [(out[2*q], out[2*q + 1]) for q in range(k)], singles.value
+
+    def bake_source(self, tuning=None):
+        L = load_library()
+        return _bake_source(lambda buf, cap, key, ok: L.tinsel_hip_bake_source_desc(C.byref(self.desc), C.byref(tuning) if tuning is not None else None, buf, cap, key, ok))
+
+
+def _bake_source(call):
+    key = C.create_string_buffer(65)
+    ok = C.c_int(0)
+    n = call(None, 0, key, C.byref(ok))
+    if n < 0:
+        raise RuntimeError("tinsel_hip_bake_source: " + load_library().tinsel_hip_last_error().decode())
+    why = "" if ok.value else load_library().tinsel_hip_last_error().decode()
+    buf = C.create_string_buffer(int(n) + 1)
+    call(buf, int(n) + 1, key, C.byref(ok))
+    return buf.value.decode(), key.value.decode(), bool(ok.value), why
 
 
 def _bytes_at(ptr, n):
@@ -627,10 +653,19 @@
         if not self._h:
             msg = L.tinsel_hip_last_error()
             raise TinselHipError("tinsel_hip_create failed: %s" % (msg.decode() if msg else "?"))
+        if tuning is not None:
+            self._apply_bake_mode(tuning)
         self.device = device
         self.num_primitives = int(scene.desc.num_primitives)
         self.width = self.height = 0
         self._accum_tensor = None
+
+    _bake_mode = -1
+    _bake_failed_key = None
+
+    def _bake_before_render(self):
+        if self._bake_mode == 1:
+            self.bake()
 
     def init(self, width, height, accum_tensor=None):
         if accum_tensor is not None:
@@ -646,6 +681,7 @@
         if output is None and readback:
             output = np.empty((options.height, options.width, 4), np.float32)
         ptr = output.ctypes.data_as(C.c_void_p) if (readback and output is not None) else None
+        self._bake_before_render()
         _check(self._L.tinsel_hip_render(self._h, C.byref(camera), C.byref(options), ptr, passes), "tinsel_hip_render")
         return output
 
@@ -653,6 +689,7 @@
     Render = render
 
     def render_async(self, camera, options, passes=1, stream=None):
+        self._bake_before_render()
         _check(self._L.tinsel_hip_render_async(self._h, C.byref(camera), C.byref(options), passes, stream), "tinsel_hip_render_async")
 
     def read_accum(self):
@@ -707,7 +744,14 @@
 
     def set_tuning(self, tuning=None, **fields):
         t = (tuning if tuning is not None else self.get_tuning()).replace(**fields)
-        _check(self._L.tinsel_hip_set_tuning(self._h, C.byref(t)), "tinsel_hip_set_tuning")
+        if not (tuning is None and fields and set(fields) <= set(abi.Tuning.BINDING_FIELDS)):
+            _check(self._L.tinsel_hip_set_tuning(self._h, C.byref(t)), "tinsel_hip_set_tuning")
+        self._apply_bake_mode(t)
+
+    def _apply_bake_mode(self, tuning):
+        if hasattr(self._L, "tinsel_hip_set_bounce_bake"):
+            _check(self._L.tinsel_hip_set_bounce_bake(self._h, int(tuning.bounce_bake)), "tinsel_hip_set_bounce_bake")
+            self._bake_mode = int(tuning.bounce_bake)
 
     def plane_table(self):
         out = (C.c_int*2)()
@@ -717,6 +761,8 @@
     def get_tuning(self):
         t = abi.Tuning()
         _check(self._L.tinsel_hip_get_tuning(self._h, C.byref(t)), "tinsel_hip_get_tuning")
+        if hasattr(self._L, "tinsel_hip_get_bounce_bake"):
+            t.bounce_bake = int(self._L.tinsel_hip_get_bounce_bake(self._h))
         return t
 
     def set_arithmetic(self, mode):
@@ -765,6 +811,35 @@
 
     def reserve(self, passes, max_depth):
         _check(self._L.tinsel_hip_reserve(self._h, int(passes), int(max_depth)), "tinsel_hip_reserve")
+        want = self.get_tuning().bounce_bake if hasattr(self._L, "tinsel_hip_bake_source") else 0
+        if want > 0 or (want < 0 and int(passes)*self.width*self.height >= abi.BAKE_AUTO_MIN_PATHS):
+            self.bake()
+
+    def bake_source(self):
+        return _bake_source(lambda buf, cap, key, ok: self._L.tinsel_hip_bake_source(self._h, buf, cap, key, ok))
+
+    def bake(self):
+        from . import build as hb
+        st = self.bake_status()
+        if st["state"] in (abi.BAKE_NONE, abi.BAKE_STALE, abi.BAKE_NO_COMPILER):
+            text, key, ok, _ = self.bake_source()
+            if key == self._bake_failed_key:
+                return st
+            image, how = hb.bake(text, key) if ok else (None, None)
+            self._bake_failed_key = key if (ok and image is None) else None
+            if image is not None:
+                _check(self._L.tinsel_hip_install_baked(self._h, image, len(image), key.encode(), abi.BAKE_FROM_CACHE if how == "cache" else abi.BAKE_COMPILED),
+                       "tinsel_hip_install_baked")
+            elif ok:
+                _check(self._L.tinsel_hip_install_baked(self._h, None, 0, None, abi.BAKE_NO_COMPILER), "tinsel_hip_install_baked")
+            st = self.bake_status()
+        return st
+
+    def bake_status(self):
+        out = (C.c_uint32*3)()
+        key = C.create_string_buffer(65)
+        _check(self._L.tinsel_hip_bake_status(self._h, out, key), "tinsel_hip_bake_status")
+        return {"state": int(out[0]), "key": key.value.decode(), "launches": int(out[1]) | (int(out[2]) << 32)}
 
     def get_pass_index(self):
         return int(self._L.tinsel_hip_get_pass_index(self._h))
```

Result: faster. 7480 Msamples/s, median of 6 (+8.4%).
